# chorowski-lab/pytorch-asr

Hardware: AMD Instinct MI355X
Metric: CTC train-step frames/sec (higher is better)
Workload: dtype bf16; 1 GPU; WSJ mono-char CTC (egs/wsj/yamls/ctc.yaml shapes), DeepSpeech2 conv+4xBiLSTM-320 encoder + FSTDecoder, fwd+bwd+GradientClipping(clip 480000, skip 4.8e+06 = recipe x global_batch/16)+PolyakDecay+Adam, synthetic 40-dim x 1-channel x 1000-frame fbank; batch_per_gpu=768, global_batch=768, frames=1000, classes=49, parallelism=dp1, batch_norm=per-replica statistics, optimizer_steps=139, step_boundary=device: att_speech.fused_step (clip / skip decision + Adam, no read-back)

## Files before the change

include/asr_amd.h:

```cpp
#ifndef ASR_AMD_H
#define ASR_AMD_H

#include <stdint.h>

#ifdef __cplusplus
extern "C" {
#endif

enum {
    ASR_OK = 0,
    ASR_EINVAL = 1,
    ASR_EUNSUPPORTED = 2,
    ASR_ELAUNCH = 3
};

int asr_abi_version(void);

const char *asr_strerror(int code);

int64_t asr_lattice_fwbw_workspace_bytes(int T, int B, int C, int N);

int asr_lattice_fwbw_f32(const float *lp, int T, int B, int C,
                         const int32_t *lens,
                         const int32_t *src_in, const int32_t *il_in,
                         const float *w_in, const float *term,
                         const int32_t *dst_out, const int32_t *il_out,
                         const float *w_out,
                         int N, int Kin, int Kout, int Bg, float neg_inf,
                         float *out_logZ, float *out_grad,
                         float *out_logZ_bwd,
                         void *workspace, int64_t workspace_bytes,
                         void *stream);

int asr_lattice_fwbw_band_supported(int T, int B, int C, int N, int Kin, int Kout, int Bg);
int asr_lattice_fwbw_band_f32(const float *lp, int T, int B, int C,
                              const int32_t *lens,
                              const int32_t *src_in, const int32_t *il_in,
                              const float *w_in, const float *term,
                              const int32_t *dst_out, const int32_t *il_out,
                              const float *w_out,
                              int N, int Kin, int Kout, int Bg, float neg_inf, float grad_sign,
                              float *out_logZ, float *out_grad,
                              float *out_logZ_bwd,
                              void *workspace, int64_t workspace_bytes,
                              uint32_t *redo_count,
                              const int32_t *ctc_labels, const int32_t *ctc_label_lens, int ctc_lmax,
                              void *stream);

int64_t asr_lattice_viterbi_workspace_bytes(int T, int B, int N);

int asr_lattice_forward_f32(const float *lp, int T, int B, int C,
                            const int32_t *lens,
                            const int32_t *src_in, const int32_t *il_in,
                            const float *w_in, const float *term,
                            int N, int K, int Bg, float neg_inf, int viterbi,
                            float *out_score, int32_t *out_best_il,
                            void *workspace, int64_t workspace_bytes,
                            void *stream);

int asr_log_softmax_fwd_f32(const float *x, int64_t rows, int group,
                            float *y, void *stream);

int asr_log_softmax_bwd_f32(const float *y, const float *dy, int64_t rows,
                            int group, float *dx, void *stream);

int asr_sub_rowmax_f32(const float *x, int T, int B, int C,
                       const int32_t *lens, float *y, float *row_max,
                       float *max_sum, void *stream);

int asr_argmax_rows_f32(const float *x, int64_t rows, int C, int32_t *out_idx,
                        void *stream);

int asr_ctc_graph_build(const int32_t *labels, const int32_t *label_lens, int B, int Lmax,
                        int num_symbols, int context_order, int allow_nonblank_selfloops,
                        int use_contextual_blanks, float nc_weight, int32_t *src_in,
                        int32_t *il_in, float *w_in, float *term, int32_t *dst_out,
                        int32_t *il_out, float *w_out, void *stream);

int64_t asr_lattice_grouped_workspace_bytes(int T, int B, int N, int G);

int asr_lattice_grouped_fwbw_f32(
    const float *lp, int T, int B, int C, const int32_t *lens, int N, int G, int Wg, int Wh,
    const int32_t *g_of, const int32_t *h_of, const int32_t *label, const int32_t *selfx,
    const int32_t *uniq, const int32_t *mem_g, const int32_t *mem_h, const float *term,
    float neg_inf, float *out_logZ, float *out_grad, float *out_logZ_bwd, void *workspace,
    int64_t workspace_bytes, void *stream);
int asr_lattice_grouped_fwbw_acc_f32(
    const float *lp, int T, int B, int C, const int32_t *lens, int N, int G, int Wg, int Wh,
    const int32_t *g_of, const int32_t *h_of, const int32_t *label, const int32_t *selfx,
    const int32_t *uniq, const int32_t *mem_g, const int32_t *mem_h, const float *term,
    float neg_inf, int accumulate, float *out_logZ, float *out_grad, float *out_logZ_bwd,
    void *workspace, int64_t workspace_bytes, void *stream);

int asr_lattice_grouped_forward_f32(
    const float *lp, int T, int B, int C, const int32_t *lens, int N, int G, int Wg, int Wh,
    const int32_t *g_of, const int32_t *h_of, const int32_t *label, const int32_t *selfx,
    const int32_t *uniq, const int32_t *mem_g, const int32_t *mem_h, const float *term,
    float neg_inf, int viterbi, float *out_score, int32_t *out_best_il, void *workspace,
    int64_t workspace_bytes, void *stream);

int64_t asr_lstm_workspace_bytes(int B, int H);

int asr_lstm_bidir_fwd_bf16(const void *gx, int gx_bf16, const void *whh_bf16,
                            const int32_t *lens, int T, int B, int H,
                            float *y, void *y_bf16, void *gates_bf16, float *csave,
                            void *workspace, int64_t workspace_bytes,
                            uint32_t *err_flag, void *stream);

int asr_lstm_wgrad_supported(int H);
int64_t asr_lstm_wgrad_workspace_bytes(int T, int B, int H, int with_input);
int asr_lstm_wgrad_bf16(const void *dgates_bf16, const void *x_bf16, const void *y_bf16,
                        int T, int B, int H, float *dw_ih, float *dw_hh,
                        void *workspace, int64_t workspace_bytes, void *stream);

int asr_lstm_dgrad_supported(int H);
int asr_lstm_dgrad_bf16(const void *dgates_bf16, const void *w_ih_bf16, int T, int B, int H,
                        float *dx, void *stream);

int asr_lstm_fused_supported(int B, int H, int F);
int asr_lstm_bidir_fwd_fused_bf16(const void *x_bf16, const void *wih_bf16,
                                  const void *whh_bf16, const int32_t *lens,
                                  int T, int B, int H, int F, float *y, void *y_bf16,
                                  void *gates_bf16, float *csave, void *workspace,
                                  int64_t workspace_bytes, uint32_t *err_flag, void *stream);

int asr_lstm_bidir_bwd_bf16(const float *dy, int dy_shared, const void *whhT_bf16,
                            const int32_t *lens, int T, int B, int H,
                            const void *gates_bf16, const float *csave,
                            void *dgates_bf16,
                            void *workspace, int64_t workspace_bytes,
                            uint32_t *err_flag, void *stream);

int64_t asr_gru_workspace_bytes(int B, int H);
int asr_gru_supported(int B, int H);

int asr_gru_bidir_fwd_bf16(const void *gx, int gx_bf16, const void *whh_bf16,
                           const int32_t *lens, int T, int B, int H,
                           float *y, void *y_bf16, void *gates_bf16,
                           void *workspace, int64_t workspace_bytes,
                           uint32_t *err_flag, void *stream);

int asr_gru_bidir_bwd_bf16(const float *dy, int dy_shared, const void *whhT_bf16,
                           const int32_t *lens, int T, int B, int H,
                           const void *gates_bf16, const float *y,
                           void *dgx_bf16, void *dhn_bf16,
                           void *workspace, int64_t workspace_bytes,
                           uint32_t *err_flag, void *stream);

int64_t asr_bn_act_workspace_bytes(int C);
int asr_bn_act_fwd_f32(const void *x, int x_bf16, const float *conv_bias, int B, int C, int H, int W,
                       const float *gamma, const float *beta,
                       float *running_mean, float *running_var,
                       int channels_last,
                       int training, float momentum, float eps, float lo, float hi,
                       void *out, int out_bf16, int out_time_major,
                       float *save_mean, float *save_invstd,
                       const double *chan_sums,
                       void *workspace, int64_t workspace_bytes, void *stream);

int asr_bn_act_bwd_f32(const void *x, int x_bf16, const float *conv_bias, int B, int C, int H, int W,
                       const float *gamma, const float *beta,
                       const float *save_mean, const float *save_invstd,
                       int channels_last,
                       int training, float lo, float hi,
                       const void *dy, int dy_bf16, int dy_time_major,
                       void *dx, float *dgamma, float *dbeta, float *dconv_bias,
                       void *workspace, int64_t workspace_bytes, void *stream);

int asr_bn_act_bwd_phase_f32(const void *x, int x_bf16, const float *conv_bias, int B, int C, int H, int W,
                             const float *gamma, const float *beta,
                             const float *save_mean, const float *save_invstd,
                             int channels_last,
                             int training, float lo, float hi,
                             const void *dy, int dy_bf16, int dy_time_major,
                             void *dx, float *dgamma, float *dbeta, float *dconv_bias,
                             void *workspace, int64_t workspace_bytes, int phase, double n_total,
                             void *stream);

int asr_log_softmax_shift_fwd_f32(const float *x, int T, int B, int C, const int32_t *lens,
                                  float *y, float *nls, float *nls_sum, void *stream);
int asr_log_softmax_shift_bwd_f32(const float *y, const float *nls, const float *dy, int64_t rows,
                                  int C, float *dx, void *stream);

int asr_log_softmax_shift_bwd_split_blocks(int64_t rows);
int asr_log_softmax_shift_bwd_split_bf16(const float *y, const float *nls, const float *dy,
                                         int64_t rows, int C, void *hi_bf16, void *lo_bf16, int ld,
                                         float *colsum_partial, void *stream);

int asr_sum_leading_f32(const float *in, int G, int64_t n, float *out, void *stream);

int asr_split_bf16_f32(const float *x, int64_t rows, int64_t cols, int64_t ldx,
                       void *hi_bf16, int64_t ldhi, void *lo_bf16, int64_t ldlo, void *stream);

int64_t asr_conv7x7c32_workspace_bytes(void);
int asr_conv7x7c32_fwd_bf16(const void *x, const float *w, int B, int H, int W, int stride_h,
                            void *y, double *chan_sums, void *workspace, int64_t workspace_bytes,
                            void *stream);
int asr_conv7x7c32_bwd_data_bf16(const void *dy, const float *w, int B, int H, int W,
                                 int stride_h, void *dx, void *workspace,
                                 int64_t workspace_bytes, void *stream);
int asr_conv7x7c32_wgrad_bf16(const void *x, const void *dy, int B, int H, int W, int stride_h,
                              float *dw, void *workspace, int64_t workspace_bytes, void *stream);

int64_t asr_conv1_7x7s2_workspace_bytes(void);
int asr_conv1_7x7s2_fwd(const float *x, const float *w, int B, int T, int F, void *y,
                        double *chan_sums, void *workspace, int64_t workspace_bytes, void *stream);
int asr_conv1_7x7s2_wgrad(const float *x, const void *dy, int B, int T, int F, float *dw,
                          void *workspace, int64_t workspace_bytes, void *stream);

int64_t asr_conv1c_7x7s2_workspace_bytes(int cin);
int asr_conv1c_7x7s2_fwd(const float *x, const float *w, int B, int T, int F, int cin, void *y,
                         double *chan_sums, void *workspace, int64_t workspace_bytes, void *stream);
int asr_conv1c_7x7s2_wgrad(const float *x, const void *dy, int B, int T, int F, int cin,
                           float *dw, void *workspace, int64_t workspace_bytes, void *stream);

int asr_tcn_attention_step_f32(const float *eproj, const float *enc, const int32_t *enc_lens,
                               const float *filt, const float *glob, const float *w_score,
                               float b_score, float temperature,
                               const float *att_prev, const int32_t *parent,
                               int T, int B, int beam, int A, int Kf, int E,
                               float *att_new, float *context, void *stream);

int asr_tcn_attention_step_win_f32(const float *eproj, const float *enc, const int32_t *enc_lens,
                                   const float *filt, const float *glob, const float *w_score,
                                   float b_score, float temperature,
                                   const float *att_prev, const int32_t *parent,
                                   int T, int B, int beam, int A, int Kf, int E,
                                   int win_lo, int win_hi,
                                   float *att_new, float *context, void *stream);

int asr_tcn_attention_scan_fwd_f32(const float *eproj, const float *filt, const float *glob,
                                   const float *a0, const float *w_score, const float *b_score,
                                   float temperature, const int32_t *enc_lens, int T, int B,
                                   int L, int A, int Kf, float *att, void *stream);
int asr_tcn_attention_scan_bwd_f32(const float *eproj, const float *filt, const float *glob,
                                   const float *a0, const float *w_score, float temperature,
                                   const int32_t *enc_lens, const float *att, const float *d_att,
                                   int T, int B, int L, int A, int Kf, float *d_eproj,
                                   float *d_filt, float *d_glob, float *d_a0, float *d_wb,
                                   void *stream);

int asr_att_gru_scan_fwd_f32(const float *eproj, const float *encoded, const int32_t *enc_lens,
                             const float *gx_emb, const float *w_ic, const float *w_hh,
                             const float *b_hh, const float *w_rec, const float *w_score,
                             const float *b_score, const float *h0, int T, int B, int beam,
                             int L, int A, int E, int H, float *att, float *states,
                             float *contexts, float *gates, float *rec, void *stream);
int asr_att_gru_scan_bwd_f32(const float *eproj, const float *encoded, const int32_t *enc_lens,
                             const float *w_icT, const float *w_hhT, const float *w_recT,
                             const float *w_score, const float *h0, const float *att,
                             const float *states, const float *gates, const float *rec,
                             const float *d_att, const float *d_states, int T, int B, int L,
                             int A, int E, int H, float *d_eproj, float *d_gates,
                             float *d_contexts, float *d_rec, float *d_w_score, float *d_h0,
                             void *stream);

int asr_beam_step_f32(const float *logits, const float *scores_in, float *scores_out,
                      const int32_t *est_in, int32_t *est_out, int step, int B, int beam, int C,
                      int Lcap, float len_div, int32_t *finished_count, float *best_score,
                      int32_t *best_len, int32_t *best_tokens, int32_t *new_input,
                      int32_t *parent, int32_t *done_and_scratch, void *stream);

#define ASR_LM_BAG_CAP 32
int asr_beam_lm_supported(int beam, int C, int bag_cap);
int asr_lm_label_costs_f64(const int32_t *ptr, const int32_t *ilabel, const double *arc_w_closed,
                           int nstates, const int32_t *bag_state, const double *bag_cost,
                           const int32_t *bag_n, int bag_cap, const int32_t *mapping,
                           const int32_t *frozen, int B, int beam, int C, double *cost, void *stream);
int asr_lm_bag_advance_f64(const int32_t *ptr, const int32_t *ptr_ne, const int32_t *dst,
                           const int32_t *ilabel, const double *weight, const int32_t *rank,
                           int nstates, int max_rank, const int32_t *mapping,
                           const int32_t *in_state, const double *in_cost, const int32_t *in_n,
                           int32_t *out_state, double *out_cost, int32_t *out_n, int bag_cap,
                           const int32_t *parent, const int32_t *new_input, const int32_t *nsteps,
                           int step, int B, int beam, int32_t *overflow, void *stream);
int asr_beam_lm_step_f32(const float *logits, const float *att, const int32_t *enc_lens,
                         const double *lm_cost, double lm_weight, const float *scores_in,
                         float *scores_out, const int32_t *est_in, int32_t *est_out,
                         const float *cov_in, float *cov_out, float *min_eos, int step, int B,
                         int beam, int C, int T, int Lcap, float len_div, double min_attention_pos,
                         float coverage_tau, float coverage_weight, int32_t *fin_count,
                         int32_t *fin_parity, float *fin_score, int32_t *fin_len, int32_t *fin_beam,
                         int32_t *fin_tokens, float *best_score, int32_t *best_len,
                         int32_t *best_tokens, float *best_elems, int32_t *new_input,
                         int32_t *parent, int32_t *frozen, int32_t *nsteps, void *stream);

int asr_graph_search_supported(int beam, int span, int T, int bag_cap);
int asr_beam_lm_step_graph_f32(const float *logits, const float *att, const int32_t *enc_lens,
                               const double *lm_cost, double lm_weight, const float *scores_in,
                               float *scores_out, const int32_t *est_in, int32_t *est_out,
                               const float *cov_in, float *cov_out, float *min_eos, int step, int B,
                               int beam, int C, int T, int Lcap, float len_div,
                               double min_attention_pos, float coverage_tau, float coverage_weight,
                               int32_t *fin_count, int32_t *fin_parity, float *fin_score,
                               int32_t *fin_len, int32_t *fin_beam, int32_t *fin_tokens,
                               float *best_score, int32_t *best_len, int32_t *best_tokens,
                               float *best_elems, int32_t *new_input, int32_t *parent,
                               int32_t *frozen, int32_t *nsteps, int32_t *fin_mask, float *tot_out,
                               void *stream);
int asr_graph_merge_f32(const float *att, const int32_t *enc_lens, float *scores, float *tot,
                        const int32_t *est_in, const int32_t *est_out, const int32_t *fin_mask,
                        const int32_t *bag_state, const int32_t *bag_n, int bag_cap,
                        const int32_t *nsteps, const float *len_pow, int step, int B, int beam, int T,
                        int Lcap, int span, float merge_threshold, int Ncap, int32_t *node_count,
                        float *node_score, int32_t *node_len, int32_t *node_tokens, float *node_att,
                        int32_t *node_bag_n, int32_t *node_bag_state, int32_t *node_fin,
                        int32_t *node_uplink, void *stream);

int asr_forced_level_f32(const float *logits, const float *att, const float *cov_in, float *cov_out,
                         const int32_t *parent, const int32_t *edge_ptr, const int32_t *edge_label,
                         const int32_t *edge_dst, const double *acoustic_in, double *acoustic_out,
                         const int32_t *enc_lens, int B, int width, int C, int T, int cov_in_rows,
                         int n_edges, int n_out, int n_sent, float coverage_tau,
                         double *sent_acoustic, int32_t *sent_covered, void *stream);

int asr_lattice_fwbw_signed_f32(const float *lp, int T, int B, int C, const int32_t *lens,
                                const int32_t *src_in, const int32_t *il_in, const float *w_in,
                                const float *term, const int32_t *dst_out, const int32_t *il_out,
                                const float *w_out, int N, int Kin, int Kout, int Bg, float neg_inf,
                                float grad_sign, float *out_logZ, float *out_grad,
                                float *out_logZ_bwd, void *workspace, int64_t workspace_bytes,
                                void *stream);
int asr_scale_rows_f32(float *x, int T, int B, int C, const float *scale, void *stream);

typedef struct AsrAdamChunk {
    void *param;
    uint32_t flat_offset;
    uint32_t count;
} AsrAdamChunk;
int asr_adam_chunk_elems(void);
int asr_grad_sumsq_partials_f32(const float *g, int64_t n, float *partials, int nparts, void *stream);
int asr_adam_clip_step_f32(const AsrAdamChunk *chunks, int nchunks, const float *g_flat,
                           float *m_flat, float *v_flat, const float *partials, int nparts,
                           const uint32_t *err_word, float lr, float beta1, float beta2, float eps,
                           float weight_decay, float clip_norm, float skip_norm,
                           const int32_t *step_in, int32_t *step_out, float *stats, void *stream);

int asr_adam_clip_step_ex_f32(const AsrAdamChunk *chunks, int nchunks, const float *g_flat,
                              float *m_flat, float *v_flat, const float *partials, int nparts,
                              const uint32_t *err_word, float lr, float beta1, float beta2, float eps,
                              float weight_decay, float clip_norm, float skip_norm,
                              const int32_t *step_in, int32_t *step_out, const uint32_t *skip_word,
                              float *stats, void *stream);

int asr_nonfinite_flag_f32(const float *x, int n, uint32_t *flag, void *stream);

typedef struct AsrNoiseSegment {
    void *data;
    uint64_t index;
    uint32_t count;
    float sigma;
} AsrNoiseSegment;
#define ASR_NOISE_APPLY 0
#define ASR_NOISE_WRITE 1
int asr_noise_chunk_elems(void);
int asr_gaussian_noise_f32(const AsrNoiseSegment *segs, int nsegs, uint64_t seed, uint32_t tag,
                           uint64_t iteration, int mode, int sign, void *stream);

int asr_edit_distance_max_len(void);
int asr_edit_distance_stats_i32(const int32_t *x, const int32_t *x_off, const int32_t *y,
                                const int32_t *y_off, int n_pairs, int max_x, int max_y,
                                int32_t *out, void *stream);

int asr_lattice_shared_supported(int N, int E, int C);
int64_t asr_lattice_shared_workspace_bytes(int T, int B, int N);
int asr_lattice_shared_fwbw_f32(
    const float *lp, int T, int B, int C, const int32_t *lens, int N, int E,
    const int32_t *in_ptr, const uint32_t *in_arc, const int32_t *out_ptr, const uint32_t *out_arc,
    const float *term, const int32_t *order_in, int n_light_in, int lanes_in,
    const int32_t *order_out, int n_light_out, int lanes_out, float neg_inf, float grad_sign,
    int accumulate, float *out_logZ, float *out_grad, float *out_logZ_bwd, void *workspace,
    int64_t workspace_bytes, void *stream);
int asr_lattice_shared_forward_f32(
    const float *lp, int T, int B, int C, const int32_t *lens, int N, int E,
    const int32_t *in_ptr, const uint32_t *in_arc, const float *term, const int32_t *order_in,
    int n_light_in, int lanes_in, float neg_inf, int viterbi, float *out_score,
    int32_t *out_best_il, void *workspace, int64_t workspace_bytes, void *stream);

int asr_ctc_align_supported(int T, int Lmax, int C);
int64_t asr_ctc_align_workspace_bytes(int T, int B, int Lmax);
int asr_ctc_align_f64(const float *lp, const int32_t *lens, const int32_t *labels,
                      const int32_t *label_lens, int B, int T, int C, int Lmax, int S,
                      int context_order, int allow_nonblank_selfloops, int eval_repeats_in_context,
                      double *out_cost, int32_t *out_frames, int32_t *out_states,
                      int32_t *out_segments, void *workspace, int64_t workspace_bytes, void *stream);

int asr_wfst_decode_supported(int64_t N, int64_t A, int C, int T);
int64_t asr_wfst_decode_workspace_bytes(int64_t N, int B, int64_t list_cap, int64_t log_cap);
int asr_wfst_decode_f32(const float *lp, int64_t frame_stride, const int32_t *lens, int T, int B, int C,
                        int64_t N, int64_t A, const uint32_t *arc_ptr, const int32_t *arc_src,
                        const int32_t *arc_dst, const int32_t *arc_ilabel, const int32_t *arc_olabel,
                        const float *arc_weight, const float *final_cost, const uint32_t *eps_ptr,
                        const uint32_t *eps_arc, int64_t E, const int32_t *eps_rank, int num_ranks,
                        int start, float beam, float acoustic_scale, int allow_partial, int64_t list_cap,
                        int64_t log_cap, int word_cap, int threads, float *out_cost,
                        int32_t *out_reached_final,
                        int32_t *out_alignment, int32_t *out_num_active, int32_t *out_words,
                        int32_t *out_num_words, int32_t *out_overflow, void *workspace,
                        int64_t workspace_bytes, void *stream);

int asr_wfst_lattice_supported(int64_t N, int64_t A, int C, int T);
int64_t asr_wfst_lattice_workspace_bytes(int64_t N, int B, int T, int64_t list_cap, int64_t log_cap);
int asr_wfst_lattice_f32(const float *lp, int64_t frame_stride, const int32_t *lens, int T, int B, int C,
                         int64_t N, int64_t A, const uint32_t *arc_ptr, const int32_t *arc_src,
                         const int32_t *arc_dst, const int32_t *arc_ilabel, const int32_t *arc_olabel,
                         const float *arc_weight, const float *final_cost, const uint32_t *eps_ptr,
                         const uint32_t *eps_arc, int64_t E, const int32_t *eps_rank, int num_ranks,
                         int start, float beam, float lattice_beam, float acoustic_scale,
                         int allow_partial, int64_t list_cap, int64_t log_cap, int64_t node_cap,
                         int64_t arc_cap, int threads, float *out_cost, int32_t *out_reached_final,
                         int32_t *out_num_nodes, int32_t *out_num_arcs, int32_t *node_time,
                         int32_t *node_state, float *node_alpha, float *node_beta,
                         int32_t *lat_src, int32_t *lat_dst, uint32_t *lat_arc, float *lat_lp,
                         int32_t *out_overflow, void *workspace, int64_t workspace_bytes,
                         void *stream);

int asr_lattice_bestpath_supported(int64_t N, int64_t A, int64_t L);
int64_t asr_lattice_bestpath_workspace_bytes(int64_t num_nodes, int num_pairs);
int asr_lattice_bestpath_f64(
    int B, int b_begin, int b_count, int num_pairs, int64_t N, int64_t A, int64_t L, const int64_t *h_node_off,
    const int64_t *h_arc_off, const int64_t *h_level_off, const int64_t *node_off, const int64_t *arc_off,
    const int64_t *level_off, const int32_t *node_time, const int32_t *node_state, const int32_t *node_level,
    const int32_t *lat_src, const int32_t *lat_dst, const int64_t *lat_arc, const float *lat_lp,
    const int32_t *level_ptr, const int32_t *level_node, const int32_t *in_ptr, const int32_t *in_arc,
    const int32_t *out_ptr, const int32_t *num_frames, const int32_t *reached_final, const double *own_scale,
    const double *acoustic_scales, const double *lm_scales, int64_t num_states, int64_t num_graph_arcs,
    const float *arc_weight, const int32_t *arc_olabel, const float *final_cost, int start, int threads,
    double *out_cost, int32_t *out_num_words, int32_t *out_words, int32_t *out_status, void *workspace,
    int64_t workspace_bytes, void *stream);
int asr_lattice_posterior_supported(int64_t N, int64_t A, int64_t L);
int64_t asr_lattice_posterior_workspace_bytes(int64_t num_nodes);
int asr_lattice_posterior_f64(
    int B, int b_begin, int b_count, int64_t N, int64_t A, int64_t L, const int64_t *h_node_off,
    const int64_t *h_arc_off, const int64_t *h_level_off, const int64_t *node_off, const int64_t *arc_off,
    const int64_t *level_off, const int32_t *node_time, const int32_t *node_state, const int32_t *node_level,
    const int32_t *lat_src, const int32_t *lat_dst, const int64_t *lat_arc, const float *lat_lp,
    const int32_t *level_ptr, const int32_t *level_node, const int32_t *in_ptr, const int32_t *in_arc,
    const int32_t *out_ptr, const int32_t *num_frames, const int32_t *reached_final, const double *own_scale,
    double acoustic_scale, double lm_scale, int64_t num_states, int64_t num_graph_arcs, const float *arc_weight,
    const int32_t *arc_olabel, const float *final_cost, int start, int threads, double *out_log_z,
    double *out_arc_log_post, double *out_node_log_post, int32_t *out_status, void *workspace,
    int64_t workspace_bytes, void *stream);

#ifdef __cplusplus
}
#endif
#endif
```

pytorch-asr_amd/att_speech/_native.py:

```python
import ctypes
import warnings
import os

import torch

_HERE = os.path.dirname(os.path.abspath(__file__))
LIB_PATH = os.environ.get(
    'ASR_AMD_LIB', os.path.join(os.path.dirname(_HERE), 'csrc', 'libasr_amd.so'))

ASR_OK, ASR_EINVAL, ASR_EUNSUPPORTED, ASR_ELAUNCH = 0, 1, 2, 3
ABI_VERSION = 24

_lib = None
EVENT_HOOK = None
_WARNED = {}

_vp, _i, _i64, _f = ctypes.c_void_p, ctypes.c_int, ctypes.c_int64, ctypes.c_float

_SIGNATURES = {
    'asr_abi_version': (ctypes.c_int, []),
    'asr_strerror': (ctypes.c_char_p, [_i]),
    'asr_lattice_fwbw_workspace_bytes': (_i64, [_i, _i, _i, _i]),
    'asr_lattice_fwbw_f32': (_i, [_vp, _i, _i, _i, _vp, _vp, _vp, _vp, _vp, _vp,
                                  _vp, _vp, _i, _i, _i, _i, _f, _vp, _vp, _vp,
                                  _vp, _i64, _vp]),
    'asr_lattice_fwbw_signed_f32': (_i, [_vp, _i, _i, _i, _vp, _vp, _vp, _vp, _vp, _vp,
                                         _vp, _vp, _i, _i, _i, _i, _f, _f, _vp, _vp, _vp,
                                         _vp, _i64, _vp]),
    'asr_scale_rows_f32': (_i, [_vp, _i, _i, _i, _vp, _vp]),
    'asr_lattice_fwbw_band_supported': (_i, [_i] * 7),
    'asr_lattice_fwbw_band_f32': (_i, [_vp, _i, _i, _i, _vp, _vp, _vp, _vp, _vp, _vp,
                                       _vp, _vp, _i, _i, _i, _i, _f, _f, _vp, _vp, _vp,
                                       _vp, _i64, _vp, _vp, _vp, _i, _vp]),
    'asr_lattice_viterbi_workspace_bytes': (_i64, [_i, _i, _i]),
    'asr_lattice_forward_f32': (_i, [_vp, _i, _i, _i, _vp, _vp, _vp, _vp, _vp,
                                     _i, _i, _i, _f, _i, _vp, _vp, _vp, _i64,
                                     _vp]),
    'asr_log_softmax_fwd_f32': (_i, [_vp, _i64, _i, _vp, _vp]),
    'asr_log_softmax_bwd_f32': (_i, [_vp, _vp, _i64, _i, _vp, _vp]),
    'asr_sub_rowmax_f32': (_i, [_vp, _i, _i, _i, _vp, _vp, _vp, _vp, _vp]),
    'asr_argmax_rows_f32': (_i, [_vp, _i64, _i, _vp, _vp]),
    'asr_conv7x7c32_workspace_bytes': (_i64, []),
    'asr_conv7x7c32_fwd_bf16': (_i, [_vp, _vp, _i, _i, _i, _i, _vp, _vp, _vp, _i64, _vp]),
    'asr_conv7x7c32_bwd_data_bf16': (_i, [_vp, _vp, _i, _i, _i, _i, _vp, _vp, _i64, _vp]),
    'asr_conv7x7c32_wgrad_bf16': (_i, [_vp, _vp, _i, _i, _i, _i, _vp, _vp, _i64, _vp]),
    'asr_conv1_7x7s2_workspace_bytes': (_i64, []),
    'asr_conv1_7x7s2_fwd': (_i, [_vp, _vp, _i, _i, _i, _vp, _vp, _vp, _i64, _vp]),
    'asr_conv1_7x7s2_wgrad': (_i, [_vp, _vp, _i, _i, _i, _vp, _vp, _i64, _vp]),
    'asr_conv1c_7x7s2_workspace_bytes': (_i64, [_i]),
    'asr_conv1c_7x7s2_fwd': (_i, [_vp, _vp, _i, _i, _i, _i, _vp, _vp, _vp, _i64, _vp]),
    'asr_conv1c_7x7s2_wgrad': (_i, [_vp, _vp, _i, _i, _i, _i, _vp, _vp, _i64, _vp]),
    'asr_log_softmax_shift_fwd_f32': (_i, [_vp, _i, _i, _i, _vp, _vp, _vp, _vp, _vp]),
    'asr_log_softmax_shift_bwd_f32': (_i, [_vp, _vp, _vp, _i64, _i, _vp, _vp]),
    'asr_sum_leading_f32': (_i, [_vp, _i, _i64, _vp, _vp]),
    'asr_adam_chunk_elems': (_i, []),
    'asr_grad_sumsq_partials_f32': (_i, [_vp, _i64, _vp, _i, _vp]),
    'asr_adam_clip_step_f32': (_i, [_vp, _i, _vp, _vp, _vp, _vp, _i, _vp, _f, _f, _f, _f, _f, _f, _f,
                                    _vp, _vp, _vp, _vp]),
    'asr_adam_clip_step_ex_f32': (_i, [_vp, _i, _vp, _vp, _vp, _vp, _i, _vp, _f, _f, _f, _f, _f, _f, _f,
                                       _vp, _vp, _vp, _vp, _vp]),
    'asr_nonfinite_flag_f32': (_i, [_vp, _i, _vp, _vp]),
    'asr_noise_chunk_elems': (_i, []),
    'asr_gaussian_noise_f32': (_i, [_vp, _i, ctypes.c_uint64, ctypes.c_uint32, ctypes.c_uint64, _i, _i, _vp]),
    'asr_edit_distance_max_len': (_i, []),
    'asr_edit_distance_stats_i32': (_i, [_vp, _vp, _vp, _vp, _i, _i, _i, _vp, _vp]),
    'asr_ctc_align_supported': (_i, [_i, _i, _i]),
    'asr_ctc_align_workspace_bytes': (_i64, [_i, _i, _i]),
    'asr_ctc_align_f64': (_i, [_vp, _vp, _vp, _vp, _i, _i, _i, _i, _i, _i, _i, _i,
                               _vp, _vp, _vp, _vp, _vp, _i64, _vp]),
    'asr_wfst_decode_supported': (_i, [_i64, _i64, _i, _i]),
    'asr_wfst_decode_workspace_bytes': (_i64, [_i64, _i, _i64, _i64]),
    'asr_wfst_decode_f32': (_i, [_vp, _i64, _vp, _i, _i, _i, _i64, _i64] + [_vp] * 9 + [_i64, _vp, _i, _i,
                                 _f, _f, _i, _i64, _i64, _i, _i] + [_vp] * 8 + [_i64, _vp]),
    'asr_wfst_lattice_supported': (_i, [_i64, _i64, _i, _i]),
    'asr_wfst_lattice_workspace_bytes': (_i64, [_i64, _i, _i, _i64, _i64]),
    'asr_wfst_lattice_f32': (_i, [_vp, _i64, _vp, _i, _i, _i, _i64, _i64] + [_vp] * 9 + [_i64, _vp, _i, _i,
                                  _f, _f, _f, _i, _i64, _i64, _i64, _i64, _i] + [_vp] * 14 + [_i64, _vp]),
    'asr_lattice_bestpath_supported': (_i, [_i64, _i64, _i64]),
    'asr_lattice_bestpath_workspace_bytes': (_i64, [_i64, _i]),
    'asr_lattice_bestpath_f64': (_i, [_i, _i, _i, _i, _i64, _i64, _i64] + [_vp] * 23 + [_i64, _i64] + [_vp] * 3 +
                                 [_i, _i] + [_vp] * 5 + [_i64, _vp]),
    'asr_lattice_posterior_supported': (_i, [_i64, _i64, _i64]),
    'asr_lattice_posterior_workspace_bytes': (_i64, [_i64]),
    'asr_lattice_posterior_f64': (_i, [_i, _i, _i, _i64, _i64, _i64] + [_vp] * 21 + [ctypes.c_double] * 2 +
                                  [_i64, _i64] + [_vp] * 3 + [_i, _i] + [_vp] * 5 + [_i64, _vp]),
    'asr_split_bf16_f32': (_i, [_vp, _i64, _i64, _i64, _vp, _i64, _vp, _i64, _vp]),
    'asr_log_softmax_shift_bwd_split_blocks': (_i, [_i64]),
    'asr_log_softmax_shift_bwd_split_bf16': (_i, [_vp, _vp, _vp, _i64, _i, _vp, _vp, _i, _vp, _vp]),
    'asr_tcn_attention_step_f32': (_i, [_vp, _vp, _vp, _vp, _vp, _vp, _f, _f, _vp, _vp,
                                        _i, _i, _i, _i, _i, _i, _vp, _vp, _vp]),
    'asr_tcn_attention_step_win_f32': (_i, [_vp, _vp, _vp, _vp, _vp, _vp, _f, _f, _vp, _vp,
                                            _i, _i, _i, _i, _i, _i, _i, _i, _vp, _vp, _vp]),
    'asr_tcn_attention_scan_fwd_f32': (_i, [_vp] * 6 + [_f, _vp, _i, _i, _i, _i, _i, _vp, _vp]),
    'asr_tcn_attention_scan_bwd_f32': (_i, [_vp] * 5 + [_f, _vp, _vp, _vp, _i, _i, _i, _i, _i] +
                                       [_vp] * 6),
    'asr_att_gru_scan_fwd_f32': (_i, [_vp] * 11 + [_i] * 7 + [_vp] * 6),
    'asr_att_gru_scan_bwd_f32': (_i, [_vp] * 14 + [_i] * 6 + [_vp] * 7),
    'asr_beam_step_f32': (_i, [_vp, _vp, _vp, _vp, _vp, _i, _i, _i, _i, _i, _f,
                               _vp, _vp, _vp, _vp, _vp, _vp, _vp, _vp]),
    'asr_beam_lm_supported': (_i, [_i, _i, _i]),
    'asr_lm_label_costs_f64': (_i, [_vp, _vp, _vp, _i, _vp, _vp, _vp, _i, _vp, _vp, _i, _i, _i, _vp, _vp]),
    'asr_lm_bag_advance_f64': (_i, [_vp] * 6 + [_i, _i] + [_vp] * 7 + [_i, _vp, _vp, _vp, _i, _i, _i, _vp, _vp]),
    'asr_beam_lm_step_f32': (_i, [_vp, _vp, _vp, _vp, ctypes.c_double] + [_vp] * 7 + [_i] * 6 +
                             [_f, ctypes.c_double, _f, _f] + [_vp] * 15),
    'asr_graph_search_supported': (_i, [_i, _i, _i, _i]),
    'asr_beam_lm_step_graph_f32': (_i, [_vp, _vp, _vp, _vp, ctypes.c_double] + [_vp] * 7 + [_i] * 6 +
                                   [_f, ctypes.c_double, _f, _f] + [_vp] * 17),
    'asr_graph_merge_f32': (_i, [_vp] * 9 + [_i, _vp, _vp] + [_i] * 6 + [_f, _i] + [_vp] * 10),
    'asr_forced_level_f32': (_i, [_vp] * 11 + [_i] * 8 + [_f, _vp, _vp, _vp]),
    'asr_ctc_graph_build': (_i, [_vp, _vp, _i, _i, _i, _i, _i, _i, _f] + [_vp] * 8),
    'asr_lattice_grouped_workspace_bytes': (_i64, [_i, _i, _i, _i]),
    'asr_lattice_grouped_fwbw_f32': (_i, [_vp, _i, _i, _i, _vp, _i, _i, _i, _i] + [_vp] * 8 +
                                     [_f, _vp, _vp, _vp, _vp, _i64, _vp]),
    'asr_lattice_grouped_fwbw_acc_f32': (_i, [_vp, _i, _i, _i, _vp, _i, _i, _i, _i] + [_vp] * 8 +
                                         [_f, _i, _vp, _vp, _vp, _vp, _i64, _vp]),
    'asr_lattice_grouped_forward_f32': (_i, [_vp, _i, _i, _i, _vp, _i, _i, _i, _i] + [_vp] * 8 +
                                        [_f, _i, _vp, _vp, _vp, _i64, _vp]),
    'asr_lattice_shared_supported': (_i, [_i, _i, _i]),
    'asr_lattice_shared_workspace_bytes': (_i64, [_i, _i, _i]),
    'asr_lattice_shared_fwbw_f32': (_i, [_vp, _i, _i, _i, _vp, _i, _i] + [_vp] * 6 + [_i, _i, _vp, _i, _i,
                                         _f, _f, _i, _vp, _vp, _vp, _vp, _i64, _vp]),
    'asr_lattice_shared_forward_f32': (_i, [_vp, _i, _i, _i, _vp, _i, _i] + [_vp] * 4 +
                                       [_i, _i, _f, _i, _vp, _vp, _vp, _i64, _vp]),
    'asr_lstm_workspace_bytes': (_i64, [_i, _i]),
    'asr_lstm_bidir_fwd_bf16': (_i, [_vp, _i, _vp, _vp, _i, _i, _i, _vp, _vp, _vp, _vp, _vp, _i64, _vp, _vp]),
    'asr_lstm_bidir_bwd_bf16': (_i, [_vp, _i, _vp, _vp, _i, _i, _i, _vp, _vp, _vp, _vp, _i64, _vp, _vp]),
    'asr_lstm_fused_supported': (_i, [_i, _i, _i]),
    'asr_lstm_wgrad_supported': (_i, [_i]),
    'asr_lstm_dgrad_supported': (_i, [_i]),
    'asr_lstm_dgrad_bf16': (_i, [_vp, _vp, _i, _i, _i, _vp, _vp]),
    'asr_lstm_wgrad_workspace_bytes': (_i64, [_i, _i, _i, _i]),
    'asr_lstm_wgrad_bf16': (_i, [_vp, _vp, _vp, _i, _i, _i, _vp, _vp, _vp, _i64, _vp]),
    'asr_lstm_bidir_fwd_fused_bf16': (_i, [_vp, _vp, _vp, _vp, _i, _i, _i, _i, _vp, _vp, _vp, _vp, _vp, _i64, _vp, _vp]),
    'asr_gru_workspace_bytes': (_i64, [_i, _i]),
    'asr_gru_supported': (_i, [_i, _i]),
    'asr_gru_bidir_fwd_bf16': (_i, [_vp, _i, _vp, _vp, _i, _i, _i, _vp, _vp, _vp, _vp, _i64, _vp, _vp]),
    'asr_gru_bidir_bwd_bf16': (_i, [_vp, _i, _vp, _vp, _i, _i, _i, _vp, _vp, _vp, _vp, _vp, _i64, _vp, _vp]),
    'asr_bn_act_workspace_bytes': (_i64, [_i]),
    'asr_bn_act_fwd_f32': (_i, [_vp, _i, _vp, _i, _i, _i, _i, _vp, _vp, _vp, _vp, _i, _i, _f, _f, _f, _f,
                                _vp, _i, _i, _vp, _vp, _vp, _vp, _i64, _vp]),
    'asr_bn_act_bwd_f32': (_i, [_vp, _i, _vp, _i, _i, _i, _i, _vp, _vp, _vp, _vp, _i, _i, _f, _f,
                                _vp, _i, _i, _vp, _vp, _vp, _vp, _vp, _i64, _vp]),
    'asr_bn_act_bwd_phase_f32': (_i, [_vp, _i, _vp, _i, _i, _i, _i, _vp, _vp, _vp, _vp, _i, _i, _f, _f,
                                      _vp, _i, _i, _vp, _vp, _vp, _vp, _vp, _i64, _i, ctypes.c_double, _vp]),
}

_EXPERIMENT_SIGNATURES = {
    'asr_lstm_bidir_bwd_fused_bf16': (_i, [_vp, _i, _vp, _vp, _vp, _i, _i, _i, _vp, _vp, _vp, _vp,
                                           _vp, _i64, _vp, _vp]),
    'asr_lstm_bidir_fwd_fused_sum_bf16': (_i, [_vp, _vp, _vp, _vp, _i, _i, _i, _i, _vp, _vp, _vp, _vp, _vp, _vp, _i64,
                                               _vp, _vp]),
}
_experiments = False


class NativeLibraryError(RuntimeError):
    pass


def lib():
    global _lib, _experiments
    if _lib is None:
        if not os.path.exists(LIB_PATH):
            raise NativeLibraryError(
                "%s is missing: build it with `make -C pytorch-asr_amd/csrc` "
                "(or __graft_entry__.build()); there is no fallback path."
                % LIB_PATH)
        handle = ctypes.CDLL(LIB_PATH)
        for name, (res, args) in _SIGNATURES.items():
            fn = getattr(handle, name)
            fn.restype = res
            fn.argtypes = args
        if handle.asr_abi_version() != ABI_VERSION:
            raise NativeLibraryError("libasr_amd.so ABI %d != expected %d" % (
                handle.asr_abi_version(), ABI_VERSION))
        _experiments = all(hasattr(handle, name) for name in _EXPERIMENT_SIGNATURES)
        if _experiments:
            for name, (res, args) in _EXPERIMENT_SIGNATURES.items():
                fn = getattr(handle, name)
                fn.restype = res
                fn.argtypes = args
        _lib = handle
    return _lib


def experiments_built():
    lib()
    return _experiments


def _need_experiments(what):
    if not experiments_built():
        raise NotImplementedError(
            '%s is an experiment (include/asr_amd_experiments.h): rebuild with '
            '`make -C pytorch-asr_amd/csrc clean all EXPERIMENTS=1`' % what)


def check(code, what):
    if code == ASR_OK:
        return
    msg = "%s: %s" % (what, lib().asr_strerror(code).decode())
    if code == ASR_EINVAL:
        raise AssertionError(msg)
    if code == ASR_EUNSUPPORTED:
        raise NotImplementedError(msg)
    raise RuntimeError(msg)


def _dev(t, dtype, name):
    if not isinstance(t, torch.Tensor) or not t.is_cuda:
        raise NativeLibraryError(
            "%s must be a GPU tensor: the MI355X path has no CPU fallback" % name)
    if t.dtype != dtype:
        raise TypeError("%s must be %s, got %s" % (name, dtype, t.dtype))
    return t if t.is_contiguous() else t.contiguous()


def _p(t):
    return ctypes.c_void_p(t.data_ptr()) if t is not None else None


def _stream():
    return ctypes.c_void_p(torch.cuda.current_stream().cuda_stream)


class Graph(object):
    __slots__ = ('src_in', 'il_in', 'w_in', 'term', 'dst_out', 'il_out',
                 'w_out', 'Bg', 'N', 'Kin', 'Kout', 'band', 'ctc_labels', 'addend')

    def __init__(self, graph_matrices, device):
        self.band = False
        self.ctc_labels = None
        self.addend = None
        if graph_matrices is None:
            return
        gm = list(graph_matrices)
        if len(gm) not in (4, 8):
            raise AssertionError("expected 4 or 8 graph matrices")
        bg = gm[0].size(0)
        if not all(m.size(0) == bg for m in gm):
            raise AssertionError("graph matrices disagree on batch size")

        def to_i(m):
            return m.to(device=device, dtype=torch.int32).contiguous()

        def to_f(m):
            return m.to(device=device, dtype=torch.float32).contiguous()
        self.src_in, self.il_in, self.w_in = to_i(gm[0]), to_i(gm[1]), to_f(gm[2])
        self.term = to_f(gm[3]).reshape(bg, -1)
        self.Bg, self.N, self.Kin = self.src_in.shape
        if len(gm) == 8:
            self.dst_out, self.il_out, self.w_out = to_i(gm[4]), to_i(gm[5]), to_f(gm[6])
            self.Kout = self.dst_out.shape[2]
            self.band = _host_band_check(gm)
        else:
            self.dst_out = self.il_out = self.w_out = None
            self.Kout = 0


def _host_band_check(gm):
    src, w = gm[0], gm[2]
    if src.is_cuda or w.is_cuda or src.dim() != 3 or src.size(1) > 256:
        return False
    valid = w > -5e19
    d = torch.arange(src.size(1)).view(1, -1, 1) - src.long()
    return bool(((d >= 0) & (d <= 2) & (w <= 0) | ~valid).all())


_BAND_STATE = {'cool': 0, 'pending': None, 'launched': 0, 'seen': (0, 0)}
_BAND_COOLDOWN = 64
_BAND_MAX_BATCH = 1 << 30
_BAND_COUNTER = {}


def _band_counter(device):
    c = _BAND_COUNTER.get(device)
    if c is None:
        c = (torch.zeros(1, dtype=torch.int32, device=device), torch.zeros(1, dtype=torch.int32).pin_memory())
        _BAND_COUNTER[device] = c
        _BAND_STATE.update(pending=None, launched=0, seen=(0, 0))
    return c


def _band_policy_allows():
    st = _BAND_STATE
    pend = st['pending']
    if pend is not None and pend[1].query():
        redone_total, launched_total = int(pend[0].item()), pend[2]
        redone, batch = redone_total - st['seen'][0], launched_total - st['seen'][1]
        st['seen'] = (redone_total, launched_total)
        st['pending'] = None
        if redone * 10 > batch:
            st['cool'] = _BAND_COOLDOWN
    if st['cool'] > 0:
        st['cool'] -= 1
        return False
    return True


def _band_policy_record(device, B):
    st = _BAND_STATE
    st['launched'] += B
    if st['pending'] is not None:
        return
    dev_cnt, host = _band_counter(device)
    host.copy_(dev_cnt, non_blocking=True)
    ev = torch.cuda.Event()
    ev.record()
    st['pending'] = (host, ev, st['launched'])


def scale_rows_(x, scale):
    x = _dev(x, torch.float32, 'x')
    scale = _dev(scale.to(torch.float32), torch.float32, 'scale')
    T, B, C = x.shape
    check(lib().asr_scale_rows_f32(_p(x), T, B, C, _p(scale), _stream()), 'asr_scale_rows_f32')
    return x


def lattice_fwbw(lp, lens, graph, neg_inf=-1e20, want_bwd_total=False, grad_sign=1.0):
    lp = _dev(lp, torch.float32, 'log_probs')
    lens = _dev(lens, torch.int32, 'act_lens')
    T, B, C = lp.shape
    if graph.Bg not in (1, B):
        raise AssertionError("graph batch %d not in (1, %d)" % (graph.Bg, B))
    L = lib()
    logZ = torch.empty(B, dtype=torch.float32, device=lp.device)
    grad = torch.empty_like(lp)
    zb = torch.empty(B, dtype=torch.float32, device=lp.device) if want_bwd_total else None
    if (T + 64) * B * C * 4 >= 2 ** 32 and graph.N <= 512 and not _WARNED.get('fits32'):
        _WARNED['fits32'] = True
        warnings.warn('lattice_fwbw: T*B*C*4 = %.2f GiB >= 4 GiB (e.g. bi-char CTC at B >= ~1100): the '
                      'meet-in-the-middle kernels address with 32-bit offsets, this call runs the '
                      'generic (much slower) kernel; split the batch' % (T * B * C * 4 / 2.0 ** 30))
    nbytes = L.asr_lattice_fwbw_workspace_bytes(T, B, C, graph.N)
    ws = torch.empty(nbytes, dtype=torch.uint8, device=lp.device)
    hook = EVENT_HOOK
    if hook is not None:
        ev0 = torch.cuda.Event(enable_timing=True)
        ev1 = torch.cuda.Event(enable_timing=True)
        ev0.record()
    band_env = os.environ.get('ASR_LATTICE_BAND', '1')
    use_band = (graph.band and band_env != '0' and
                L.asr_lattice_fwbw_band_supported(T, B, C, graph.N, graph.Kin, graph.Kout, graph.Bg))
    if use_band and band_env != '2' and (B > _BAND_MAX_BATCH or not _band_policy_allows()):
        use_band = False
    args = (_p(lp), T, B, C, _p(lens), _p(graph.src_in), _p(graph.il_in),
            _p(graph.w_in), _p(graph.term), _p(graph.dst_out), _p(graph.il_out),
            _p(graph.w_out), graph.N, graph.Kin, graph.Kout, graph.Bg,
            float(neg_inf), _p(logZ), _p(grad), _p(zb), _p(ws), nbytes)
    sargs = args[:17] + (float(grad_sign),) + args[17:]
# ... 624 lines not shown


def tcn_attention_scan_fwd(eproj, filt, glob, a0, w_score, b_score, enc_lens, temperature):
    eproj, a0 = _dev(eproj, torch.float32, 'eproj'), _dev(a0, torch.float32, 'a0')
    filt, glob = _dev(filt, torch.float32, 'filt'), _dev(glob, torch.float32, 'glob')
    w_score = _dev(w_score, torch.float32, 'w_score')
    b_score = _dev(b_score, torch.float32, 'b_score')
    enc_lens = _dev(enc_lens, torch.int32, 'enc_lens')
    T, B, A = eproj.shape
    L = glob.shape[0]
    att = torch.empty((L, B, T), dtype=torch.float32, device=eproj.device)
    check(lib().asr_tcn_attention_scan_fwd_f32(
        _p(eproj), _p(filt), _p(glob), _p(a0), _p(w_score), _p(b_score), float(temperature),
        _p(enc_lens), T, B, L, A, filt.shape[2] // A, _p(att), _stream()),
        'asr_tcn_attention_scan_fwd_f32')
    return att


def tcn_attention_scan_bwd(eproj, filt, glob, a0, w_score, enc_lens, temperature, att, d_att):
    eproj, a0 = _dev(eproj, torch.float32, 'eproj'), _dev(a0, torch.float32, 'a0')
    filt, glob = _dev(filt, torch.float32, 'filt'), _dev(glob, torch.float32, 'glob')
    w_score = _dev(w_score, torch.float32, 'w_score')
    enc_lens = _dev(enc_lens, torch.int32, 'enc_lens')
    att, d_att = _dev(att, torch.float32, 'att'), _dev(d_att, torch.float32, 'd_att')
    T, B, A = eproj.shape
    L = glob.shape[0]
    d_eproj = torch.empty_like(eproj)
    d_filt = torch.empty_like(filt)
    d_glob = torch.empty_like(glob)
    d_a0 = torch.empty_like(a0)
    d_wb = torch.empty((B, A + 1), dtype=torch.float32, device=eproj.device)
    check(lib().asr_tcn_attention_scan_bwd_f32(
        _p(eproj), _p(filt), _p(glob), _p(a0), _p(w_score), float(temperature), _p(enc_lens),
        _p(att), _p(d_att), T, B, L, A, filt.shape[2] // A, _p(d_eproj), _p(d_filt), _p(d_glob),
        _p(d_a0), _p(d_wb), _stream()), 'asr_tcn_attention_scan_bwd_f32')
    return d_eproj, d_filt, d_glob, d_a0, d_wb


ATT_GRU_MAX_FRAMES, ATT_GRU_MAX_HIDDEN, ATT_GRU_MAX_ENCODED = 4096, 320, 512


def att_gru_supported(T, A, E, H):
    return (1 <= T <= ATT_GRU_MAX_FRAMES and 1 <= A <= ATT_GRU_MAX_HIDDEN
            and 1 <= H <= ATT_GRU_MAX_HIDDEN and 1 <= E <= ATT_GRU_MAX_ENCODED
            and A % 4 == 0 and E % 4 == 0 and H % 4 == 0)


def att_gru_scan_fwd(eproj, encoded, enc_lens, gx_emb, w_ic, w_hh, b_hh, w_rec, w_score, b_score,
                     h0, beam=1, save=True):
    f32 = torch.float32
    eproj, encoded = _dev(eproj, f32, 'eproj'), _dev(encoded, f32, 'encoded')
    gx_emb, h0 = _dev(gx_emb, f32, 'gx_emb'), _dev(h0, f32, 'h0')
    w_ic, w_hh, b_hh = _dev(w_ic, f32, 'w_ic'), _dev(w_hh, f32, 'w_hh'), _dev(b_hh, f32, 'b_hh')
    w_rec, w_score = _dev(w_rec, f32, 'w_rec'), _dev(w_score, f32, 'w_score')
    b_score = _dev(b_score, f32, 'b_score')
    enc_lens = _dev(enc_lens, torch.int32, 'enc_lens')
    T, NU, A = eproj.shape
    E = encoded.shape[2]
    L, B, H3 = gx_emb.shape
    H = H3 // 3
    if (encoded.shape[:2] != (T, NU) or B != NU * beam or h0.shape != (B, H) or H3 != 3 * H
            or w_ic.shape != (H3, E) or w_hh.shape != (H3, H) or b_hh.numel() != H3
            or w_rec.shape != (A, H) or w_score.numel() != A or enc_lens.numel() != NU):
        raise AssertionError('asr_att_gru_scan_fwd_f32: inconsistent operand shapes')
    new = lambda *shape: torch.empty(shape, dtype=f32, device=eproj.device)
    att, states = new(L, B, T), new(L, B, H)
    ctxs, gates, rec = (new(L, B, E), new(L, B, 4 * H), new(L, B, A)) if save else (None,) * 3
    check(lib().asr_att_gru_scan_fwd_f32(
        _p(eproj), _p(encoded), _p(enc_lens), _p(gx_emb), _p(w_ic), _p(w_hh), _p(b_hh), _p(w_rec),
        _p(w_score), _p(b_score), _p(h0), T, B, beam, L, A, E, H, _p(att), _p(states), _p(ctxs),
        _p(gates), _p(rec), _stream()), 'asr_att_gru_scan_fwd_f32')
    return att, states, ctxs, gates, rec


def att_gru_scan_bwd(eproj, encoded, enc_lens, w_icT, w_hhT, w_recT, w_score, h0, att, states,
                     gates, rec, d_att, d_states):
    f32 = torch.float32
    eproj, encoded = _dev(eproj, f32, 'eproj'), _dev(encoded, f32, 'encoded')
    w_icT, w_hhT = _dev(w_icT, f32, 'w_icT'), _dev(w_hhT, f32, 'w_hhT')
    w_recT, w_score = _dev(w_recT, f32, 'w_recT'), _dev(w_score, f32, 'w_score')
    h0, att, states = _dev(h0, f32, 'h0'), _dev(att, f32, 'att'), _dev(states, f32, 'states')
    gates, rec = _dev(gates, f32, 'gates'), _dev(rec, f32, 'rec')
    d_att = None if d_att is None else _dev(d_att, f32, 'd_att')
    d_states = None if d_states is None else _dev(d_states, f32, 'd_states')
    enc_lens = _dev(enc_lens, torch.int32, 'enc_lens')
    T, B, A = eproj.shape
    E = encoded.shape[2]
    L, _, H = states.shape
    if (encoded.shape[:2] != (T, B) or states.shape[1] != B or att.shape != (L, B, T)
            or gates.shape != (L, B, 4 * H) or rec.shape != (L, B, A) or h0.shape != (B, H)
            or w_icT.shape != (E, 3 * H) or w_hhT.shape != (H, 3 * H) or w_recT.shape != (H, A)
            or (d_att is not None and d_att.shape != att.shape)
            or (d_states is not None and d_states.shape != states.shape)):
        raise AssertionError('asr_att_gru_scan_bwd_f32: inconsistent operand shapes')
    dev = eproj.device
    d_eproj = torch.zeros_like(eproj)
    d_gates = torch.empty_like(gates)
    d_ctx = torch.empty((L, B, E), dtype=f32, device=dev)
    d_rec = torch.empty_like(rec)
    d_v = torch.empty((B, A), dtype=f32, device=dev)
    d_h0 = torch.empty_like(h0)
    check(lib().asr_att_gru_scan_bwd_f32(
        _p(eproj), _p(encoded), _p(enc_lens), _p(w_icT), _p(w_hhT), _p(w_recT), _p(w_score),
        _p(h0), _p(att), _p(states), _p(gates), _p(rec), _p(d_att), _p(d_states), T, B, L, A, E, H,
        _p(d_eproj), _p(d_gates), _p(d_ctx), _p(d_rec), _p(d_v), _p(d_h0), _stream()),
        'asr_att_gru_scan_bwd_f32')
    return d_eproj, d_gates, d_ctx, d_rec, d_v, d_h0


LM_BAG_CAP = 32


def beam_lm_supported(beam, C, bag_cap=LM_BAG_CAP):
    return bool(lib().asr_beam_lm_supported(beam, C, bag_cap))


def lm_label_costs(lm, bag_state, bag_cost, bag_n, mapping, frozen, B, beam, C, cost, bag_cap=LM_BAG_CAP):
    check(lib().asr_lm_label_costs_f64(
        _p(lm['ptr']), _p(lm['ilabel']), _p(lm['w_closed']), lm['nstates'], _p(bag_state), _p(bag_cost),
        _p(bag_n), bag_cap, _p(mapping), _p(frozen), B, beam, C, _p(cost), _stream()),
        'asr_lm_label_costs_f64')
    return cost


def lm_bag_advance(lm, mapping, bags_in, bags_out, parent, new_input, nsteps, step, B, beam, overflow,
                   bag_cap=LM_BAG_CAP):
    check(lib().asr_lm_bag_advance_f64(
        _p(lm['ptr']), _p(lm['ptr_ne']), _p(lm['dst']), _p(lm['ilabel']), _p(lm['weight']), _p(lm['rank']),
        lm['nstates'], lm['max_rank'], _p(mapping), _p(bags_in[0]), _p(bags_in[1]), _p(bags_in[2]),
        _p(bags_out[0]), _p(bags_out[1]), _p(bags_out[2]), bag_cap, _p(parent), _p(new_input),
        _p(nsteps), step, B, beam, _p(overflow), _stream()), 'asr_lm_bag_advance_f64')


def beam_lm_step(logits, att, lens, lm_cost, lm_weight, scores_in, scores_out, est_in, est_out, cov_in,
                 cov_out, min_eos, step, B, beam, len_div, min_attention_pos, coverage_tau,
                 coverage_weight, state, fin_mask=None, tot_out=None):
    C, T = logits.shape[-1], att.shape[-1]
    graph = fin_mask is not None or tot_out is not None
    name = 'asr_beam_lm_step_graph_f32' if graph else 'asr_beam_lm_step_f32'
    extra = (_p(fin_mask), _p(tot_out)) if graph else ()
    check(getattr(lib(), name)(
        _p(logits), _p(att), _p(lens), _p(lm_cost), float(lm_weight), _p(scores_in), _p(scores_out),
        _p(est_in), _p(est_out), _p(cov_in), _p(cov_out), _p(min_eos), step, B, beam, C, T,
        est_in.shape[1], len_div, float(min_attention_pos), coverage_tau, coverage_weight,
        _p(state['fin_count']), _p(state['fin_parity']), _p(state['fin_score']), _p(state['fin_len']),
        _p(state['fin_beam']), _p(state['fin_tokens']), _p(state['best_score']), _p(state['best_len']),
        _p(state['best_tokens']), _p(state['best_elems']), _p(state['new_input']), _p(state['parent']),
        _p(state['frozen']), _p(state['nsteps']), *(extra + (_stream(),))), name)


beam_lm_step_graph = beam_lm_step


def graph_search_supported(beam, span, T, bag_cap=LM_BAG_CAP):
    return bool(lib().asr_graph_search_supported(beam, span, T, bag_cap))


NODE_KEYS = ('node_count', 'node_score', 'node_len', 'node_tokens', 'node_att', 'node_bag_n',
             'node_bag_state', 'node_fin', 'node_uplink')


def graph_merge(att, lens, scores, tot, est_in, est_out, fin_mask, bags, nsteps, len_pow, step, B, beam,
                span, merge_threshold, store, bag_cap=LM_BAG_CAP):
    T, Lcap, Ncap = att.shape[-1], est_in.shape[1], store['node_score'].shape[1]
    check(lib().asr_graph_merge_f32(
        _p(att), _p(lens), _p(scores), _p(tot), _p(est_in), _p(est_out), _p(fin_mask),
        _p(bags[0]) if bags is not None else None, _p(bags[2]) if bags is not None else None, bag_cap,
        _p(nsteps), _p(len_pow), step, B, beam, T, Lcap, int(span), float(merge_threshold), Ncap,
        *([_p(store[k]) for k in NODE_KEYS] + [_stream()])), 'asr_graph_merge_f32')


def forced_level(logits, att, cov_in, cov_out, parent, edge_ptr, edge_label, edge_dst, acoustic_in,
                 acoustic_out, lens, B, width, coverage_tau, sent_acoustic, sent_covered):
    slots = B * width
    C, T = logits.shape[-1], att.shape[-1]
    assert logits.shape[0] == slots and att.shape[0] == slots and cov_out.shape[0] >= slots
    assert cov_in.shape[-1] == T and cov_out.shape[-1] == T and parent.numel() >= slots
    assert edge_ptr.numel() >= slots + 1 and acoustic_in.numel() >= slots
    assert edge_dst.numel() == edge_label.numel() and sent_covered.numel() == sent_acoustic.numel()
    check(lib().asr_forced_level_f32(
        _p(_dev(logits, torch.float32, 'logits')), _p(_dev(att, torch.float32, 'att')),
        _p(_dev(cov_in, torch.float32, 'cov_in')), _p(_dev(cov_out, torch.float32, 'cov_out')),
        _p(_dev(parent, torch.int32, 'parent')), _p(_dev(edge_ptr, torch.int32, 'edge_ptr')),
        _p(_dev(edge_label, torch.int32, 'edge_label')), _p(_dev(edge_dst, torch.int32, 'edge_dst')),
        _p(_dev(acoustic_in, torch.float64, 'acoustic_in')),
        _p(_dev(acoustic_out, torch.float64, 'acoustic_out')), _p(_dev(lens, torch.int32, 'lens')),
        B, width, C, T, cov_in.shape[0], edge_label.numel(), acoustic_out.numel(),
        sent_acoustic.numel(), float(coverage_tau), _p(_dev(sent_acoustic, torch.float64, 'sent_acoustic')),
        _p(_dev(sent_covered, torch.int32, 'sent_covered')), _stream()), 'asr_forced_level_f32')


def beam_step(logits, scores_in, scores_out, est_in, est_out, step, B, beam, len_div, state):
    C = logits.shape[-1]
    check(lib().asr_beam_step_f32(
        _p(logits), _p(scores_in), _p(scores_out), _p(est_in), _p(est_out), int(step), B, beam, C,
        est_in.shape[1], float(len_div), _p(state['finished_count']), _p(state['best_score']),
        _p(state['best_len']), _p(state['best_tokens']), _p(state['new_input']),
        _p(state['parent']), _p(state['done']), _stream()), 'asr_beam_step_f32')


def _nhwc_bf16(t, what):
    if not t.is_cuda:
        raise NativeLibraryError("%s must live on the MI355X" % what)
    if t.dtype != torch.bfloat16:
        t = t.to(torch.bfloat16)
    t = t.contiguous(memory_format=torch.channels_last)
    return (t,) + tuple(t.shape)


def conv7x7c32_fwd(x, weight, stride_h, want_sums=False):
    x, B, C, H, W = _nhwc_bf16(x, 'x')
    weight = _dev(weight, torch.float32, 'weight')
    Ho, Wo = (H - 7) // stride_h + 1, W - 6
    y = torch.empty((B, 32, Ho, Wo), dtype=torch.bfloat16, device=x.device,
                    memory_format=torch.channels_last)
    L = lib()
    nbytes = L.asr_conv7x7c32_workspace_bytes()
    ws = torch.empty(nbytes, dtype=torch.uint8, device=x.device)
    sums = torch.empty((2, 32), dtype=torch.float64, device=x.device) if want_sums else None
    check(L.asr_conv7x7c32_fwd_bf16(_p(x), _p(weight), B, H, W, int(stride_h), _p(y), _p(sums),
                                    _p(ws), nbytes, _stream()), 'asr_conv7x7c32_fwd_bf16')
    return (y, sums) if want_sums else y


def conv7x7c32_bwd_data(dy, weight, H, W, stride_h):
    dy, B, C, Ho, Wo = _nhwc_bf16(dy, 'dy')
    weight = _dev(weight, torch.float32, 'weight')
    assert Ho == (H - 7) // stride_h + 1 and Wo == W - 6
    dx = torch.empty((B, 32, H, W), dtype=torch.bfloat16, device=dy.device,
                     memory_format=torch.channels_last)
    L = lib()
    nbytes = L.asr_conv7x7c32_workspace_bytes()
    ws = torch.empty(nbytes, dtype=torch.uint8, device=dy.device)
    check(L.asr_conv7x7c32_bwd_data_bf16(_p(dy), _p(weight), B, H, W, int(stride_h), _p(dx),
                                         _p(ws), nbytes, _stream()), 'asr_conv7x7c32_bwd_data_bf16')
    return dx


def conv7x7c32_wgrad(x, dy, stride_h):
    x, B, C, H, W = _nhwc_bf16(x, 'x')
    dy = _nhwc_bf16(dy, 'dy')[0]
    dw = torch.empty((32, 32, 7, 7), dtype=torch.float32, device=x.device)
    L = lib()
    nbytes = L.asr_conv7x7c32_workspace_bytes()
    ws = torch.empty(nbytes, dtype=torch.uint8, device=x.device)
    check(L.asr_conv7x7c32_wgrad_bf16(_p(x), _p(dy), B, H, W, int(stride_h), _p(dw), _p(ws),
                                      nbytes, _stream()), 'asr_conv7x7c32_wgrad_bf16')
    return dw


def conv1_supported(F, cin):
    Fo = (F - 7) // 2 + 1
    return F >= 7 and ((cin == 1 and Fo <= 64) or (cin == 3 and Fo <= 48 and Fo % 2 == 0))


def conv1_fwd(x, weight, want_sums=False):
    x = _dev(x, torch.float32, 'x')
    weight = _dev(weight, torch.float32, 'weight')
    cin = x.shape[3] if x.dim() == 4 else 1
    B, T, F = x.shape[:3]
    if tuple(weight.shape) != (32, cin, 7, 7):
        raise ValueError('conv1_fwd: weight must be [32, %d, 7, 7]' % cin)
    y = torch.empty((B, 32, T + 6, (F - 7) // 2 + 1), dtype=torch.bfloat16, device=x.device,
                    memory_format=torch.channels_last)
    L = lib()
    sums = torch.empty((2, 32), dtype=torch.float64, device=x.device) if want_sums else None
    if cin == 1:
        nbytes = L.asr_conv1_7x7s2_workspace_bytes()
        ws = torch.empty(nbytes, dtype=torch.uint8, device=x.device)
        check(L.asr_conv1_7x7s2_fwd(_p(x), _p(weight), B, T, F, _p(y), _p(sums), _p(ws), nbytes,
                                    _stream()), 'asr_conv1_7x7s2_fwd')
    else:
        nbytes = L.asr_conv1c_7x7s2_workspace_bytes(cin)
        if nbytes < 0:
            raise NotImplementedError('conv1_fwd: %d input channels' % cin)
        ws = torch.empty(nbytes, dtype=torch.uint8, device=x.device)
        check(L.asr_conv1c_7x7s2_fwd(_p(x), _p(weight), B, T, F, cin, _p(y), _p(sums), _p(ws), nbytes,
                                     _stream()), 'asr_conv1c_7x7s2_fwd')
    return (y, sums) if want_sums else y


def conv1_wgrad(x, dy):
    x = _dev(x, torch.float32, 'x')
    dy = _nhwc_bf16(dy, 'dy')[0]
    cin = x.shape[3] if x.dim() == 4 else 1
    B, T, F = x.shape[:3]
    dw = torch.empty((32, cin, 7, 7), dtype=torch.float32, device=x.device)
    L = lib()
    if cin == 1:
        nbytes = L.asr_conv1_7x7s2_workspace_bytes()
        ws = torch.empty(nbytes, dtype=torch.uint8, device=x.device)
        check(L.asr_conv1_7x7s2_wgrad(_p(x), _p(dy), B, T, F, _p(dw), _p(ws), nbytes, _stream()),
              'asr_conv1_7x7s2_wgrad')
    else:
        nbytes = L.asr_conv1c_7x7s2_workspace_bytes(cin)
        if nbytes < 0:
            raise NotImplementedError('conv1_wgrad: %d input channels' % cin)
        ws = torch.empty(nbytes, dtype=torch.uint8, device=x.device)
        check(L.asr_conv1c_7x7s2_wgrad(_p(x), _p(dy), B, T, F, cin, _p(dw), _p(ws), nbytes, _stream()),
              'asr_conv1c_7x7s2_wgrad')
    return dw


def split_bf16(x, hi=None, lo=None):
    x = _dev(x, torch.float32, 'x')
    if hi is None:
        hi = torch.empty(x.shape, dtype=torch.bfloat16, device=x.device)
        lo = torch.empty(x.shape, dtype=torch.bfloat16, device=x.device)
        rows, cols, ldx, ldh, ldl = 1, x.numel(), x.numel(), x.numel(), x.numel()
    else:
        if x.dim() != 2 or hi.shape != x.shape or lo.shape != x.shape or x.stride(1) != 1 \
                or hi.stride(1) != 1 or lo.stride(1) != 1 or hi.dtype != torch.bfloat16 or lo.dtype != torch.bfloat16:
            raise ValueError('split_bf16: x, hi, lo must be [rows, cols] with a dense last dimension')
        rows, cols = x.shape
        ldx, ldh, ldl = x.stride(0), hi.stride(0), lo.stride(0)
    check(lib().asr_split_bf16_f32(_p(x), rows, cols, ldx, _p(hi), ldh, _p(lo), ldl, _stream()),
          'asr_split_bf16_f32')
    return hi, lo


def sum_leading(t):
    if not t.is_cuda or t.dtype != torch.float32 or (t[0].numel() & 3):
        return t.sum(0)
    t = t.contiguous()
    if t.data_ptr() & 15:
        return t.sum(0)
    out = torch.empty(t.shape[1:], dtype=torch.float32, device=t.device)
    check(lib().asr_sum_leading_f32(_p(t), t.shape[0], t[0].numel(), _p(out), _stream()),
          'asr_sum_leading_f32')
    return out


def log_softmax_shift_fwd(x, lens):
    x = _dev(x, torch.float32, 'logits')
    lens = _dev(lens, torch.int32, 'lens')
    T, B, C = x.shape
    y = torch.empty_like(x)
    nls = torch.empty((T, B), dtype=torch.float32, device=x.device)
    nls_sum = torch.empty(B, dtype=torch.float32, device=x.device)
    check(lib().asr_log_softmax_shift_fwd_f32(_p(x), T, B, C, _p(lens), _p(y), _p(nls), _p(nls_sum),
                                              _stream()), 'asr_log_softmax_shift_fwd_f32')
    return y, nls, nls_sum


def log_softmax_shift_bwd_split(y, nls, dy, ld):
    y, dy = _dev(y, torch.float32, 'y'), _dev(dy, torch.float32, 'dy')
    C = y.shape[-1]
    rows = y.numel() // C
    L = lib()
    hi = torch.empty((rows, ld), dtype=torch.bfloat16, device=y.device)
    lo = torch.empty((rows, ld), dtype=torch.bfloat16, device=y.device)
    part = torch.empty((L.asr_log_softmax_shift_bwd_split_blocks(rows), ld), dtype=torch.float32, device=y.device)
    check(L.asr_log_softmax_shift_bwd_split_bf16(_p(y), _p(nls), _p(dy), rows, C, _p(hi), _p(lo), int(ld),
                                                 _p(part), _stream()), 'asr_log_softmax_shift_bwd_split_bf16')
    nb = part.shape[0]
    if nb % 32 == 0 and nb > 32:
        part = sum_leading(part.view(32, (nb // 32) * ld)).view(nb // 32, ld)
    return hi, lo, sum_leading(part)[:C]


def log_softmax_shift_bwd(y, nls, dy):
    y, dy = _dev(y, torch.float32, 'y'), _dev(dy, torch.float32, 'dy')
    C = y.shape[-1]
    dx = torch.empty_like(y)
    check(lib().asr_log_softmax_shift_bwd_f32(_p(y), _p(nls), _p(dy), y.numel() // C, C, _p(dx),
                                              _stream()), 'asr_log_softmax_shift_bwd_f32')
    return dx


def edit_distance_max_len():
    return int(lib().asr_edit_distance_max_len())


def edit_distance_stats(x, x_off, y, y_off, max_x, max_y):
    x, x_off = _dev(x, torch.int32, 'x'), _dev(x_off, torch.int32, 'x_off')
    y, y_off = _dev(y, torch.int32, 'y'), _dev(y_off, torch.int32, 'y_off')
    n = x_off.numel() - 1
    if n < 0 or y_off.numel() != n + 1:
        raise AssertionError('edit_distance_stats: x_off and y_off must both hold n + 1 offsets')
    out = torch.empty((n, 4), dtype=torch.int32, device=x.device)
    check(lib().asr_edit_distance_stats_i32(_p(x), _p(x_off), _p(y), _p(y_off), n, int(max_x),
                                            int(max_y), _p(out), _stream()),
          'asr_edit_distance_stats_i32')
    return out


def ctc_align_supported(T, Lmax, C):
    return bool(lib().asr_ctc_align_supported(int(T), int(Lmax), int(C)))


def ctc_align(lp, lens, labels, label_lens, num_symbols, context_order=1,
              allow_nonblank_selfloops=True, eval_repeats_in_context=False):
    lp = _dev(lp, torch.float32, 'log_probs')
    lens, label_lens = _dev(lens, torch.int32, 'lens'), _dev(label_lens, torch.int32, 'label_lens')
    labels = _dev(labels, torch.int32, 'labels')
    T, B, C = lp.shape
    Lmax = labels.shape[1] if labels.dim() == 2 else -1
    if Lmax < 0 or labels.shape[0] != B or lens.numel() != B or label_lens.numel() != B:
        raise AssertionError('ctc_align: lens [B], labels [B, Lmax] and label_lens [B] must match lp [T, B, C]')
    L = lib()
    dev = lp.device
    cost = torch.empty(B, dtype=torch.float64, device=dev)
    frames = torch.empty((B, T), dtype=torch.int32, device=dev)
    states = torch.empty((B, T), dtype=torch.int32, device=dev)
    segments = torch.empty((B, Lmax, 2), dtype=torch.int32, device=dev)
    nbytes = int(L.asr_ctc_align_workspace_bytes(T, B, Lmax))
    ws = torch.empty(nbytes, dtype=torch.uint8, device=dev) if nbytes else None
    check(L.asr_ctc_align_f64(_p(lp), _p(lens), _p(labels), _p(label_lens), B, T, C, Lmax,
                              int(num_symbols), int(context_order), int(bool(allow_nonblank_selfloops)),
                              int(bool(eval_repeats_in_context)), _p(cost), _p(frames), _p(states),
                              _p(segments), _p(ws), nbytes, _stream()), 'asr_ctc_align_f64')
    return cost, frames, states, segments
```

pytorch-asr_amd/att_speech/modules/encoders/deep_speech_2.py:

```python
import warnings
from collections import OrderedDict

import torch
from torch import nn

from att_speech.modules.encoders.base_encoder import BaseEncoder
from att_speech.modules.encoders.encoder_utils import (
    BatchRNN, Normalization, SequentialWithOptionalAttributes)


class DeepSpeech2(BaseEncoder):
    def __init__(self, sample_batch, conv_normalization='batch_norm',
                 conv_strides=[[2, 2], [2, 1]],
                 conv_kernel_sizes=[[41, 11], [21, 11]],
                 conv_num_features=[32, 32],
                 rnn_hidden_size=768, rnn_nb_layers=5, rnn_projection_size=0,
                 rnn_type=nn.LSTM, rnn_dropout=0.0, rnn_residual=False,
                 rnn_normalization='batch_norm', rnn_subsample=None, **kwargs):
        super(DeepSpeech2, self).__init__(**kwargs)
        import os
        self.conv_bf16 = os.environ.get('ASR_CONV_BF16', '1') != '0'
        self.fused_bn = os.environ.get('ASR_FUSED_BN', '1') != '0'
        self.native_conv = os.environ.get('ASR_NATIVE_CONV', '1') != '0'
        if isinstance(rnn_type, str):
            rnn_type = {'LSTM': nn.LSTM, 'GRU': nn.GRU}[rnn_type.split('.')[-1]]
        self.makeConv(sample_batch, conv_strides, conv_kernel_sizes,
                      conv_num_features, conv_normalization)
        features = sample_batch['features']
        features = features.permute(0, 3, 1, 2)
        with torch.no_grad():
            was_training = self.conv.training
            self.conv.eval()
            after_conv_size = self.conv.forward(features).size()
            self.conv.train(was_training)
        self.rnn_input_size = after_conv_size[1] * after_conv_size[3]
        self.makeRnn(rnn_hidden_size, rnn_nb_layers, rnn_projection_size,
                     rnn_type, rnn_dropout, rnn_residual, rnn_normalization,
                     rnn_subsample)

    def makeConv(self, sample_batch, conv_strides, conv_kernel_sizes,
                 conv_num_features, normalization):
        num_channels = sample_batch['features'].size()[3]
        conv_padding = int(0.5 * (
            conv_kernel_sizes[1][0] - 1 +
            conv_strides[0][0] * (conv_kernel_sizes[0][0] - 1)))
        self.conv_cumative_stride = conv_strides[0][0] * conv_strides[1][0]
        self.conv = nn.Sequential(
            nn.Conv2d(num_channels, conv_num_features[0],
                      kernel_size=tuple(conv_kernel_sizes[0]),
                      stride=tuple(conv_strides[0]), padding=(conv_padding, 0)),
            Normalization(normalization, 2, conv_num_features[0]),
            nn.Hardtanh(0, 20, inplace=True),
            nn.Conv2d(conv_num_features[0], conv_num_features[1],
                      kernel_size=tuple(conv_kernel_sizes[1]),
                      stride=tuple(conv_strides[1])),
            Normalization(normalization, 2, conv_num_features[1]),
            nn.Hardtanh(0, 20, inplace=True))

    def makeRnn(self, rnn_hidden_size, rnn_nb_layers, rnn_projection_size,
                rnn_type, rnn_dropout, rnn_residual, normalization,
                rnn_subsample):
        if rnn_subsample is None:
            rnn_subsample = []
        rnn_dropout = nn.Dropout(p=rnn_dropout) if rnn_dropout > 0.0 else None
        rnns = [('0', BatchRNN(input_size=self.rnn_input_size,
                               hidden_size=rnn_hidden_size, rnn_type=rnn_type,
                               bidirectional=True, packed_data=True,
                               normalization=None,
                               projection_size=rnn_projection_size,
                               subsample=(0 in rnn_subsample)))]
        for i in range(rnn_nb_layers - 1):
            rnn = BatchRNN(input_size=(rnn_hidden_size if rnn_projection_size == 0
                                       else rnn_projection_size),
                           projection_size=rnn_projection_size,
                           hidden_size=rnn_hidden_size, rnn_type=rnn_type,
                           bidirectional=True, packed_data=True,
                           normalization=normalization, residual=rnn_residual,
                           subsample=(i + 1 in rnn_subsample))
            if rnn_dropout:
                rnns.append(('{}_dropout'.format(i + 1), rnn_dropout))
            rnns.append(('{}'.format(i + 1), rnn))
        self.rnns = SequentialWithOptionalAttributes(OrderedDict(rnns))

    def _conv_forward(self, features):
        conv = self.conv
        fused = (features.is_cuda and self.fused_bn and len(conv) == 6
                 and isinstance(conv[0], nn.Conv2d) and isinstance(conv[3], nn.Conv2d)
                 and all(isinstance(conv[i], Normalization)
                         and isinstance(conv[i].batch_norm, nn.BatchNorm2d)
                         and conv[i].batch_norm.affine for i in (1, 4))
                 and all(isinstance(conv[i], nn.Hardtanh) for i in (2, 5)))
        bf16 = features.is_cuda and self.conv_bf16 and len(conv) == 6 \
            and isinstance(conv[3], nn.Conv2d)
        c2 = conv[3] if len(conv) == 6 else None

        def run_conv(c, x, with_bias=True, keep_bf16=False):
            bias = c.bias if with_bias else None
            if not bf16:
                return nn.functional.conv2d(x.float() if x.dtype != torch.float32 else x,
                                            c.weight, bias, c.stride, c.padding,
                                            c.dilation, c.groups)
            y = nn.functional.conv2d(
                x.to(torch.bfloat16), c.weight.to(torch.bfloat16),
                None if bias is None else bias.to(torch.bfloat16),
                c.stride, c.padding, c.dilation, c.groups)
            return y if keep_bf16 else y.float()

        def second_conv(x, with_bias=True):
            return run_conv(c2, x, with_bias)

        if fused:
            from att_speech.modules.encoders.native_bn import bn_hardtanh
            from att_speech.modules.encoders import native_conv
            c1 = conv[0]
            sums1 = sums2 = None
            if bf16 and self.native_conv and native_conv.first_supported(c1, features):
                x, sums1 = native_conv.conv1(features, c1)
            else:
                if bf16 and self.native_conv and not getattr(self, '_warned_conv1', False):
                    self._warned_conv1 = True
                    warnings.warn('DeepSpeech2: the first convolution is not a (1 or 3)->32 7x7 stride-(1,2) '
                                  'shape on gradient-free features csrc/conv.hip is built for; using '
                                  'torch / MIOpen for it')
                x = run_conv(c1, features, with_bias=False, keep_bf16=True)
            x = bn_hardtanh(x, conv[1].batch_norm, conv[2], out_bf16=bf16, conv_bias=c1.bias,
                            chan_sums=sums1)
            if bf16 and self.native_conv and native_conv.supported(c2, x):
                y2, sums2 = native_conv.conv7x7c32(x, c2)
            else:
                if bf16 and self.native_conv and not getattr(self, '_warned_conv', False):
                    self._warned_conv = True
                    warnings.warn('DeepSpeech2: the second convolution is not the 32->32 7x7 '
                                  'stride-(3,1) shape csrc/conv.hip is built for; using torch / MIOpen')
                y2 = run_conv(c2, x, with_bias=False, keep_bf16=True)
            x = bn_hardtanh(y2, conv[4].batch_norm, conv[5], time_major=True, conv_bias=c2.bias,
                            chan_sums=sums2, out_bf16=bf16 and self._rnn_takes_bf16(y2))
            return x.view(x.size(0), x.size(1), -1)
        if bf16:
            x = conv[5](conv[4](second_conv(conv[2](conv[1](conv[0](features))))))
        else:
            x = conv(features)
        x = x.permute(2, 0, 1, 3).contiguous()
        return x.view(x.size(0), x.size(1), -1)

    def _rnn_takes_bf16(self, x):
        import os
        if os.environ.get('ASR_LSTM_BF16_INPUT', '1') == '0':
            return False
        first = next(iter(self.rnns._modules.values()), None)
        return (isinstance(first, BatchRNN) and first._use_native(x) and not first.residual
                and type(first.batch_norm.batch_norm).__name__ == 'Identity')

    def forward(self, features, features_lengths, spkids, ivectors=None,
                characteristic_vectors=None, **kwargs):
        features = features.permute(0, 3, 1, 2)
        features_lengths = torch.as_tensor(features_lengths)
        features_lengths = ((features_lengths + self.conv_cumative_stride - 1)
                            // self.conv_cumative_stride).int()
        if features.is_cuda:
            from att_speech import _native
            _native.attach_device_lens(features_lengths, features.device)
        features = self._conv_forward(features)
        assert features_lengths[0] == features.size()[0]
        return self.rnns(features, features_lengths, spkids)
```

pytorch-asr_amd/att_speech/modules/encoders/native_conv.py:

```python
import torch

from att_speech import _native


def supported(conv, x):
    return (x.is_cuda and isinstance(conv, torch.nn.Conv2d) and conv.in_channels == 32
            and conv.out_channels == 32 and tuple(conv.kernel_size) == (7, 7)
            and tuple(conv.stride) == (3, 1) and tuple(conv.padding) == (0, 0)
            and tuple(conv.dilation) == (1, 1) and conv.groups == 1
            and x.dim() == 4 and x.size(2) >= 7 and 7 <= x.size(3) <= 48)


class Conv7x7C32Function(torch.autograd.Function):
    @staticmethod
    def forward(ctx, x, weight):
        x = x.to(torch.bfloat16).contiguous(memory_format=torch.channels_last)
        ctx.save_for_backward(x, weight)
        y, sums = _native.conv7x7c32_fwd(x, weight.detach(), 3, want_sums=True)
        ctx.mark_non_differentiable(sums)
        return y, sums

    @staticmethod
    def backward(ctx, dy, _dsums):
        x, weight = ctx.saved_tensors
        dx = dw = None
        if ctx.needs_input_grad[0]:
            dx = _native.conv7x7c32_bwd_data(dy, weight.detach(), x.size(2), x.size(3), 3)
        if ctx.needs_input_grad[1]:
            dw = _native.conv7x7c32_wgrad(x, dy, 3)
        return dx, dw


def first_supported(conv, x):
    return (x.is_cuda and isinstance(conv, torch.nn.Conv2d) and conv.in_channels in (1, 3)
            and conv.out_channels == 32 and tuple(conv.kernel_size) == (7, 7)
            and tuple(conv.stride) == (1, 2) and tuple(conv.padding) == (6, 0)
            and tuple(conv.dilation) == (1, 1) and conv.groups == 1
            and x.dim() == 4 and x.size(1) == conv.in_channels
            and _native.conv1_supported(x.size(3), conv.in_channels)
            and not x.requires_grad)


class Conv1Function(torch.autograd.Function):

    @staticmethod
    def forward(ctx, x, weight):
        x = x.float().contiguous()
        ctx.save_for_backward(x, weight)
        y, sums = _native.conv1_fwd(x, weight.detach(), want_sums=True)
        ctx.mark_non_differentiable(sums)
        return y, sums

    @staticmethod
    def backward(ctx, dy, _dsums):
        x, weight = ctx.saved_tensors
        return None, (_native.conv1_wgrad(x, dy) if ctx.needs_input_grad[1] else None)


def conv1(features, conv):
    if features.size(1) == 1:
        return Conv1Function.apply(features[:, 0], conv.weight)
    return Conv1Function.apply(features.permute(0, 2, 3, 1), conv.weight)


def conv7x7c32(x, conv):
    return Conv7x7C32Function.apply(x, conv.weight)
```

pytorch-asr_amd/csrc/bnact.hip:

```cpp
#include "common.h"
#include "../../include/asr_amd.h"

namespace {

using namespace asr;

struct BnParams {
    const float *x;
    int B, C, HW, Wd;
    const float *gamma, *beta;
    const float *mean, *invstd;
    const float *shift;
    float lo, hi;
};

__global__ __launch_bounds__(256) void bn_stats_kernel(const float *x, const float *shift, int C, int HW, double *sums) {
    __shared__ float red[64];
    const int c = blockIdx.x, b = blockIdx.y;
    const float *p = x + ((size_t)b * C + c) * HW;
    const float sh0 = shift ? shift[c] : 0.f;
    float s = 0.f, q = 0.f;
    for (int i = threadIdx.x; i < HW; i += 256) {
        const float v = p[i] + sh0;
        s += v;
// ... 241 lines not shown

template <typename DyT, int TM>
__device__ __forceinline__ F4 load_dy4(const BnParamsN &p, const DyT *dy, int64_t pix, int c0) {
    if (TM) {
        const size_t o = tm_index(p, pix, c0);
        F4 d;
#pragma unroll
        for (int i = 0; i < 4; ++i) d.v[i] = (float)dy[o + (size_t)i * p.W];
        return d;
    }
    return load4(dy + pix * p.C + c0);
}

template <typename XT, typename DyT, int TM>
__global__ __launch_bounds__(256) void bn_act_bwd_reduce_nhwc_kernel(BnParamsN p, const DyT *dy, double *sums) {
    const XT *px = (const XT *)p.x;
    const int C = p.C;
    NHWC_THREAD_SETUP(p.P);
    float m[4], is[4], g[4], be[4], s[4] = {0.f, 0.f, 0.f, 0.f}, q[4] = {0.f, 0.f, 0.f, 0.f};
#pragma unroll
    for (int i = 0; i < 4; ++i) {
        m[i] = p.mean[c0 + i] - (p.shift ? p.shift[c0 + i] : 0.f);
        is[i] = p.invstd[c0 + i]; g[i] = p.gamma[c0 + i]; be[i] = p.beta[c0 + i];
    }
    auto acc = [&](const F4 &v, const F4 &dv) {
#pragma unroll
        for (int i = 0; i < 4; ++i) {
            const float xh = (v.v[i] - m[i]) * is[i];
            const float y = fmaf(xh, g[i], be[i]);
            const float d = (y > p.lo && y < p.hi) ? dv.v[i] : 0.f;
            s[i] += d;
            q[i] += d * xh;
        }
    };
    int64_t pix = p0 + pl;
    for (; pix + PL < p1; pix += 2 * PL) {
        const F4 v0 = load4(px + pix * C + c0), v1 = load4(px + (pix + PL) * C + c0);
        const F4 d0 = load_dy4<DyT, TM>(p, dy, pix, c0), d1 = load_dy4<DyT, TM>(p, dy, pix + PL, c0);
        acc(v0, d0);
        acc(v1, d1);
    }
    for (; pix < p1; pix += PL) acc(load4(px + pix * C + c0), load_dy4<DyT, TM>(p, dy, pix, c0));
    nhwc_block_atomics(s, q, C, sums);
}

template <typename XT, typename DyT, int TM>
__global__ __launch_bounds__(256) void bn_act_bwd_apply_nhwc_kernel(BnParamsN p, const DyT *dy, const double *sums,
                                                                    double n, int training, XT *dx) {
    const XT *px = (const XT *)p.x;
    const int C = p.C;
    NHWC_THREAD_SETUP(p.P);
    float m[4], is[4], g[4], be[4], k1[4], k2[4];
#pragma unroll
    for (int i = 0; i < 4; ++i) {
        m[i] = p.mean[c0 + i] - (p.shift ? p.shift[c0 + i] : 0.f);
        is[i] = p.invstd[c0 + i]; g[i] = p.gamma[c0 + i]; be[i] = p.beta[c0 + i];
        k1[i] = training ? (float)(sums[2 * (c0 + i)] / n) : 0.f;
        k2[i] = training ? (float)(sums[2 * (c0 + i) + 1] / n) : 0.f;
    }
    for (int64_t pix = p0 + pl; pix < p1; pix += PL) {
        const F4 v = load4(px + pix * C + c0);
        const F4 dv = load_dy4<DyT, TM>(p, dy, pix, c0);
        F4 o;
#pragma unroll
        for (int i = 0; i < 4; ++i) {
            const float xh = (v.v[i] - m[i]) * is[i];
            const float y = fmaf(xh, g[i], be[i]);
            const float d = (y > p.lo && y < p.hi) ? dv.v[i] : 0.f;
            o.v[i] = g[i] * is[i] * (d - k1[i] - xh * k2[i]);
        }
        store4(dx + pix * C + c0, o);
    }
}

struct F8 { float v[8]; };
typedef __attribute__((ext_vector_type(8))) __bf16 bf16x8v;
__device__ __forceinline__ F8 load8(const __bf16 *p) {
    const bf16x8v t = *reinterpret_cast<const bf16x8v *>(p);
    F8 r;
#pragma unroll
    for (int i = 0; i < 8; ++i) r.v[i] = (float)t[i];
    return r;
}
__device__ __forceinline__ F8 load8(const float *p) {
    const float4 a = reinterpret_cast<const float4 *>(p)[0], b = reinterpret_cast<const float4 *>(p)[1];
    return F8{{a.x, a.y, a.z, a.w, b.x, b.y, b.z, b.w}};
}
__device__ __forceinline__ void store8(__bf16 *p, const F8 &a) {
    bf16x8v t;
#pragma unroll
    for (int i = 0; i < 8; ++i) t[i] = (__bf16)a.v[i];
    *reinterpret_cast<bf16x8v *>(p) = t;
}
__device__ __forceinline__ void store8(float *p, const F8 &a) {
    reinterpret_cast<float4 *>(p)[0] = make_float4(a.v[0], a.v[1], a.v[2], a.v[3]);
    reinterpret_cast<float4 *>(p)[1] = make_float4(a.v[4], a.v[5], a.v[6], a.v[7]);
}
__device__ __forceinline__ void nhwc_block_atomics8(const float (&s)[8], const float (&q)[8], int C,
                                                    double *sums) {
    __shared__ float rs8[256][9], rq8[256][9];
#pragma unroll
    for (int i = 0; i < 8; ++i) { rs8[threadIdx.x][i] = s[i]; rq8[threadIdx.x][i] = q[i]; }
    __syncthreads();
    const int CG = C / 8;
    if ((int)threadIdx.x < C) {
        const int cg = threadIdx.x >> 3, i = threadIdx.x & 7;
        float a = 0.f, b = 0.f;
        for (int t = cg; t < 256; t += CG) { a += rs8[t][i]; b += rq8[t][i]; }
        atomicAdd(&sums[2 * threadIdx.x], (double)a);
        atomicAdd(&sums[2 * threadIdx.x + 1], (double)b);
    }
}
#define NHWC8_THREAD_SETUP(P_)                                                         \
    const int CG = C / 8, PL = 256 / CG, c0 = 8 * ((int)threadIdx.x % CG),             \
              pl = (int)threadIdx.x / CG;                                              \
    const int64_t pend = (P_), cstep = (int64_t)gridDim.x * 2 * PL

template <typename XT, typename OutT>
__global__ __launch_bounds__(256) void bn_act_fwd_nhwc8_kernel(BnParamsN p, OutT *out) {
    const XT *px = (const XT *)p.x;
    const int C = p.C;
    NHWC8_THREAD_SETUP(p.P);
    float sc[8], sh[8];
#pragma unroll
    for (int i = 0; i < 8; ++i) {
        sc[i] = p.gamma[c0 + i] * p.invstd[c0 + i];
        sh[i] = p.beta[c0 + i] - (p.mean[c0 + i] - (p.shift ? p.shift[c0 + i] : 0.f)) * sc[i];
    }
    auto one = [&](int64_t pix, const F8 &v) {
        F8 y;
#pragma unroll
        for (int i = 0; i < 8; ++i) y.v[i] = fminf(fmaxf(fmaf(v.v[i], sc[i], sh[i]), p.lo), p.hi);
        store8(out + pix * C + c0, y);
    };
    for (int64_t pix = (int64_t)blockIdx.x * 2 * PL + pl; pix < pend; pix += cstep) {
        if (pix + PL < pend) {
            const F8 v0 = load8(px + pix * C + c0), v1 = load8(px + (pix + PL) * C + c0);
            one(pix, v0);
            one(pix + PL, v1);
        } else {
            one(pix, load8(px + pix * C + c0));
        }
    }
}

template <typename XT, typename DyT, int MODE>
__global__ __launch_bounds__(256) void bn_act_bwd_nhwc8_kernel(BnParamsN p, const DyT *dy, double *sums,
                                                               double n, int training, XT *dx) {
    const XT *px = (const XT *)p.x;
    const int C = p.C;
    NHWC8_THREAD_SETUP(p.P);
    float m[8], is[8], g[8], be[8], k1[8], k2[8], s[8], q[8];
#pragma unroll
    for (int i = 0; i < 8; ++i) {
        m[i] = p.mean[c0 + i] - (p.shift ? p.shift[c0 + i] : 0.f);
        is[i] = p.invstd[c0 + i]; g[i] = p.gamma[c0 + i]; be[i] = p.beta[c0 + i];
        k1[i] = MODE == 1 && training ? (float)(sums[2 * (c0 + i)] / n) : 0.f;
        k2[i] = MODE == 1 && training ? (float)(sums[2 * (c0 + i) + 1] / n) : 0.f;
        s[i] = q[i] = 0.f;
    }
    auto one = [&](int64_t pix, const F8 &v, const F8 &dv) {
        F8 o;
#pragma unroll
        for (int i = 0; i < 8; ++i) {
            const float xh = (v.v[i] - m[i]) * is[i];
            const float y = fmaf(xh, g[i], be[i]);
            const float d = (y > p.lo && y < p.hi) ? dv.v[i] : 0.f;
            if (MODE == 0) { s[i] += d; q[i] += d * xh; }
            else o.v[i] = g[i] * is[i] * (d - k1[i] - xh * k2[i]);
        }
        if (MODE == 1) store8(dx + pix * C + c0, o);
    };
    for (int64_t pix = (int64_t)blockIdx.x * 2 * PL + pl; pix < pend; pix += cstep) {
        if (pix + PL < pend) {
            const F8 v0 = load8(px + pix * C + c0), v1 = load8(px + (pix + PL) * C + c0);
            const F8 d0 = load8(dy + pix * C + c0), d1 = load8(dy + (pix + PL) * C + c0);
            one(pix, v0, d0);
            one(pix + PL, v1, d1);
        } else {
            one(pix, load8(px + pix * C + c0), load8(dy + pix * C + c0));
        }
    }
    if (MODE == 0) nhwc_block_atomics8(s, q, C, sums);
}

struct FastDiv {
    unsigned m, d;
    __device__ __forceinline__ explicit FastDiv(int dd) : m((unsigned)((1ull << 32) / (unsigned)dd) + 1u), d((unsigned)dd) {}
    __device__ __forceinline__ int operator()(int x) const { return d == 1u ? x : (int)__umulhi((unsigned)x, m); }
};

template <typename T>
__device__ __forceinline__ void tm_row_to_lds(const T *row, float *tile, int CW, int it) {
    const F4 v = load4(row + 4 * it);
    *reinterpret_cast<float4 *>(tile + 4 * it) = make_float4(v.v[0], v.v[1], v.v[2], v.v[3]);
}

template <typename XT, typename OutT>
__global__ __launch_bounds__(256) void bn_act_fwd_nhwc_tm_kernel(BnParamsN p, OutT *out, int TMR) {
    extern __shared__ __attribute__((aligned(16))) float tile[];
    const XT *px = (const XT *)p.x;
    const int C = p.C, W = p.W, CW = C * W, CG = C / 4, Q = CW / 4;
    const int c0 = 4 * ((int)threadIdx.x % CG);
    float sc[4], sh[4];
#pragma unroll
    for (int i = 0; i < 4; ++i) {
        sc[i] = p.gamma[c0 + i] * p.invstd[c0 + i];
        sh[i] = p.beta[c0 + i] - (p.mean[c0 + i] - (p.shift ? p.shift[c0 + i] : 0.f)) * sc[i];
    }
    const int64_t nrows = p.P / W;
    const FastDiv dCG(CG), dW(W), dQ(Q);
    for (int64_t r0 = (int64_t)blockIdx.x * TMR; r0 < nrows; r0 += (int64_t)gridDim.x * TMR) {
        const int nr = nrows - r0 < TMR ? (int)(nrows - r0) : TMR;
        const int b0 = (int)(r0 / p.H), h0 = (int)(r0 - (int64_t)b0 * p.H);
        for (int it = threadIdx.x; it < nr * W * CG; it += 256) {
            const int j = dCG(it), row = dW(j), w = j - row * W;
            const F4 v = load4(px + (r0 * W + j) * C + c0);
#pragma unroll
            for (int i = 0; i < 4; ++i)
                tile[row * CW + (c0 + i) * W + w] = fminf(fmaxf(fmaf(v.v[i], sc[i], sh[i]), p.lo), p.hi);
        }
        __syncthreads();
        for (int it = threadIdx.x; it < nr * Q; it += 256) {
            const int row = dQ(it), k = it - row * Q;
            int h = h0 + row, b = b0;
            while (h >= p.H) { h -= p.H; ++b; }
            const float4 t = *reinterpret_cast<const float4 *>(tile + row * CW + 4 * k);
            store4(out + ((size_t)h * p.B + b) * CW + 4 * k, F4{{t.x, t.y, t.z, t.w}});
        }
        __syncthreads();
    }
}

template <typename XT, typename DyT, int MODE>
__global__ __launch_bounds__(256) void bn_act_bwd_nhwc_tm_kernel(BnParamsN p, const DyT *dy, double *sums,
                                                                 double n, int training, XT *dx, int TMR) {
    extern __shared__ __attribute__((aligned(16))) float tile[];
    const XT *px = (const XT *)p.x;
    const int C = p.C, W = p.W, CW = C * W, CG = C / 4, Q = CW / 4;
    const int c0 = 4 * ((int)threadIdx.x % CG);
    float m[4], is[4], g[4], be[4], k1[4], k2[4], s[4] = {0.f, 0.f, 0.f, 0.f}, q[4] = {0.f, 0.f, 0.f, 0.f};
#pragma unroll
    for (int i = 0; i < 4; ++i) {
        m[i] = p.mean[c0 + i] - (p.shift ? p.shift[c0 + i] : 0.f);
        is[i] = p.invstd[c0 + i]; g[i] = p.gamma[c0 + i]; be[i] = p.beta[c0 + i];
        k1[i] = MODE == 1 && training ? (float)(sums[2 * (c0 + i)] / n) : 0.f;
        k2[i] = MODE == 1 && training ? (float)(sums[2 * (c0 + i) + 1] / n) : 0.f;
    }
    const int64_t nrows = p.P / W;
    const FastDiv dCG(CG), dW(W), dQ(Q);
    for (int64_t r0 = (int64_t)blockIdx.x * TMR; r0 < nrows; r0 += (int64_t)gridDim.x * TMR) {
        const int nr = nrows - r0 < TMR ? (int)(nrows - r0) : TMR;
        const int b0 = (int)(r0 / p.H), h0 = (int)(r0 - (int64_t)b0 * p.H);
        for (int it = threadIdx.x; it < nr * Q; it += 256) {
            const int row = dQ(it), k = it - row * Q;
            int h = h0 + row, b = b0;
            while (h >= p.H) { h -= p.H; ++b; }
            tm_row_to_lds(dy + ((size_t)h * p.B + b) * CW, tile + row * CW, CW, k);
        }
        __syncthreads();
        for (int it = threadIdx.x; it < nr * W * CG; it += 256) {
            const int j = dCG(it), row = dW(j), w = j - row * W;
            const F4 v = load4(px + (r0 * W + j) * C + c0);
            F4 o;
#pragma unroll
            for (int i = 0; i < 4; ++i) {
                const float xh = (v.v[i] - m[i]) * is[i];
                const float y = fmaf(xh, g[i], be[i]);
                const float d = (y > p.lo && y < p.hi) ? tile[row * CW + (c0 + i) * W + w] : 0.f;
                if (MODE == 0) { s[i] += d; q[i] += d * xh; }
                else o.v[i] = g[i] * is[i] * (d - k1[i] - xh * k2[i]);
            }
            if (MODE == 1) store4(dx + (r0 * W + j) * C + c0, o);
        }
        __syncthreads();
    }
    if (MODE == 0) nhwc_block_atomics(s, q, C, sums);
}

__global__ void bn_param_grads_kernel(const double *sums, int C, const float *gamma,
                                      const float *invstd, int training, float *dgamma,
                                      float *dbeta, float *dshift) {
    const int c = blockIdx.x * blockDim.x + threadIdx.x;
    if (c >= C) return;
    dbeta[c] = (float)sums[2 * c];
    dgamma[c] = (float)sums[2 * c + 1];
    if (dshift) dshift[c] = training ? 0.f : gamma[c] * invstd[c] * (float)sums[2 * c];
}

__global__ void zero_doubles_kernel(double *p, int n) {
    const int i = blockIdx.x * blockDim.x + threadIdx.x;
    if (i < n) p[i] = 0.0;
}

inline int tm_rows(int cw) {
    if (cw <= 0) return 0;
    const int fit = 48 * 1024 / (cw * 4);
    return fit < 8 ? fit : 8;
}

inline bool bad_shape(int B, int C, int H, int W) {
    return B <= 0 || C <= 0 || H <= 0 || W <= 0 || C > 65535 || B > 65535 ||
           (int64_t)H * W > 0x7fffffff;
}

}

extern "C" int64_t asr_bn_act_workspace_bytes(int C) { return C < 0 ? -1 : (int64_t)C * 2 * 8 + 64; }

extern "C" int asr_bn_act_fwd_f32(const void *x, int x_bf16, const float *conv_bias, int B, int C, int H, int W,
                                  const float *gamma, const float *beta,
                                  float *running_mean, float *running_var,
                                  int channels_last,
                                  int training, float momentum, float eps, float lo, float hi,
                                  void *out, int out_bf16, int out_time_major,
                                  float *save_mean, float *save_invstd,
                                  const double *chan_sums,
                                  void *workspace, int64_t workspace_bytes, void *stream) {
    if (bad_shape(B, C, H, W) || !x || !gamma || !beta || !out || !save_mean || !save_invstd)
        return ASR_EINVAL;
    if (!training && (!running_mean || !running_var)) return ASR_EINVAL;
    if (!workspace || workspace_bytes < asr_bn_act_workspace_bytes(C)) return ASR_EINVAL;
    hipStream_t s = (hipStream_t)stream;
    double *sums = (double *)workspace;
    const int HW = H * W;
    const dim3 grid(C, B);
    if (channels_last && (C % 4 != 0 || C > 1024 || 256 % (C / 4) != 0)) return ASR_EUNSUPPORTED;
    if (x_bf16 && !channels_last) return ASR_EUNSUPPORTED;
    const int64_t P = (int64_t)B * HW;
    const int nwg = (int)(P / 64 < 4096 ? (P / 64 > 0 ? P / 64 : 1) : 4096);
    if (training && chan_sums) {
        hipLaunchKernelGGL(bn_finalize_from_sums_kernel, dim3((C + 63) / 64), dim3(64), 0, s, chan_sums,
                           conv_bias, C, (double)B * HW, eps, momentum, save_mean, save_invstd,
                           running_mean, running_var);
    } else if (training) {
        hipLaunchKernelGGL(zero_doubles_kernel, dim3((2 * C + 255) / 256), dim3(256), 0, s, sums, 2 * C);
        if (channels_last)
            if (x_bf16) hipLaunchKernelGGL(bn_stats_nhwc_kernel<__bf16>, dim3(nwg), dim3(256), 0, s, (const __bf16 *)x, conv_bias, P, C, sums);
            else hipLaunchKernelGGL(bn_stats_nhwc_kernel<float>, dim3(nwg), dim3(256), 0, s, (const float *)x, conv_bias, P, C, sums);
        else
            hipLaunchKernelGGL(bn_stats_kernel, grid, dim3(256), 0, s, (const float *)x, conv_bias, C, HW, sums);
        hipLaunchKernelGGL(bn_finalize_kernel, dim3((C + 63) / 64), dim3(64), 0, s, sums, C,
                           (double)B * HW, eps, momentum, save_mean, save_invstd, running_mean,
                           running_var);
    } else {
        hipLaunchKernelGGL(bn_eval_stats_kernel, dim3((C + 63) / 64), dim3(64), 0, s, running_mean,
                           running_var, C, eps, save_mean, save_invstd);
    }
    BnParams p;
    p.x = (const float *)x; p.B = B; p.C = C; p.HW = HW; p.Wd = W; p.gamma = gamma; p.beta = beta;
    p.mean = save_mean; p.invstd = save_invstd; p.shift = conv_bias; p.lo = lo; p.hi = hi;
    if (channels_last) {
        BnParamsN q;
        q.x = x; q.P = P; q.B = B; q.C = C; q.H = H; q.W = W; q.gamma = gamma; q.beta = beta;
        q.mean = save_mean; q.invstd = save_invstd; q.shift = conv_bias; q.lo = lo; q.hi = hi;
        const int cw = C * W, tmr = tm_rows(cw);
        if (out_time_major && cw % 8 == 0 && tmr >= 1) {
            const int64_t rows = (int64_t)B * H;
            const int g2 = (int)((rows + tmr - 1) / tmr < 2048 ? (rows + tmr - 1) / tmr : 2048);
            const size_t lds = (size_t)tmr * cw * 4;
#define ASR_BN_FWDT(XT, OT) \
            hipLaunchKernelGGL((bn_act_fwd_nhwc_tm_kernel<XT, OT>), dim3(g2), dim3(256), lds, s, q, (OT *)out, tmr)
            if (x_bf16) { if (out_bf16) ASR_BN_FWDT(__bf16, __bf16); else ASR_BN_FWDT(__bf16, float); }
            else { if (out_bf16) ASR_BN_FWDT(float, __bf16); else ASR_BN_FWDT(float, float); }
#undef ASR_BN_FWDT
            return hipGetLastError() == hipSuccess ? ASR_OK : ASR_ELAUNCH;
        }
        if (!out_time_major && x_bf16 && C % 8 == 0 && 256 % (C / 8) == 0) {
            if (out_bf16) hipLaunchKernelGGL((bn_act_fwd_nhwc8_kernel<__bf16, __bf16>), dim3(nwg), dim3(256), 0, s, q, (__bf16 *)out);
            else hipLaunchKernelGGL((bn_act_fwd_nhwc8_kernel<__bf16, float>), dim3(nwg), dim3(256), 0, s, q, (float *)out);
            return hipGetLastError() == hipSuccess ? ASR_OK : ASR_ELAUNCH;
        }
#define ASR_BN_FWDN(XT, OT, TMV) \
        hipLaunchKernelGGL((bn_act_fwd_nhwc_kernel<XT, OT, TMV>), dim3(nwg), dim3(256), 0, s, q, (OT *)out)
        if (x_bf16) {
            if (out_bf16) { if (out_time_major) ASR_BN_FWDN(__bf16, __bf16, 1); else ASR_BN_FWDN(__bf16, __bf16, 0); }
            else { if (out_time_major) ASR_BN_FWDN(__bf16, float, 1); else ASR_BN_FWDN(__bf16, float, 0); }
        } else {
            if (out_bf16) { if (out_time_major) ASR_BN_FWDN(float, __bf16, 1); else ASR_BN_FWDN(float, __bf16, 0); }
            else { if (out_time_major) ASR_BN_FWDN(float, float, 1); else ASR_BN_FWDN(float, float, 0); }
        }
#undef ASR_BN_FWDN
        return hipGetLastError() == hipSuccess ? ASR_OK : ASR_ELAUNCH;
    }
    if (out_bf16) {
        if (out_time_major) hipLaunchKernelGGL((bn_act_fwd_kernel<__bf16, 1>), grid, dim3(256), 0, s, p, (__bf16 *)out);
        else hipLaunchKernelGGL((bn_act_fwd_kernel<__bf16, 0>), grid, dim3(256), 0, s, p, (__bf16 *)out);
    } else {
        if (out_time_major) hipLaunchKernelGGL((bn_act_fwd_kernel<float, 1>), grid, dim3(256), 0, s, p, (float *)out);
        else hipLaunchKernelGGL((bn_act_fwd_kernel<float, 0>), grid, dim3(256), 0, s, p, (float *)out);
    }
    return hipGetLastError() == hipSuccess ? ASR_OK : ASR_ELAUNCH;
}

extern "C" int asr_bn_act_bwd_phase_f32(const void *x, int x_bf16, const float *conv_bias, int B, int C, int H, int W,
                                  const float *gamma, const float *beta,
                                  const float *save_mean, const float *save_invstd,
                                  int channels_last,
                                  int training, float lo, float hi,
                                  const void *dy, int dy_bf16, int dy_time_major,
                                  void *dx, float *dgamma, float *dbeta, float *dconv_bias,
                                  void *workspace, int64_t workspace_bytes, int phase,
                                  double n_total, void *stream) {
    if (phase < 0 || phase > 2 || (phase == 2 && !(n_total >= 1.0))) return ASR_EINVAL;
    const bool do_reduce = phase != 2, do_apply = phase != 1;
    if (bad_shape(B, C, H, W) || !x || !gamma || !beta || !save_mean || !save_invstd || !dy ||
        !dx || !dgamma || !dbeta)
        return ASR_EINVAL;
    if (!workspace || workspace_bytes < asr_bn_act_workspace_bytes(C)) return ASR_EINVAL;
    hipStream_t s = (hipStream_t)stream;
    double *sums = (double *)workspace;
    const int HW = H * W;
    const dim3 grid(C, B);
    BnParams p;
    p.x = (const float *)x; p.B = B; p.C = C; p.HW = HW; p.Wd = W; p.gamma = gamma; p.beta = beta;
    p.mean = save_mean; p.invstd = save_invstd; p.shift = conv_bias; p.lo = lo; p.hi = hi;
    const double n = phase == 2 ? n_total : (double)B * HW;
    if (do_reduce)
        hipLaunchKernelGGL(zero_doubles_kernel, dim3((2 * C + 255) / 256), dim3(256), 0, s, sums, 2 * C);
    if (x_bf16 && !channels_last) return ASR_EUNSUPPORTED;
    if (channels_last) {
        if (C % 4 != 0 || C > 1024 || 256 % (C / 4) != 0) return ASR_EUNSUPPORTED;
        BnParamsN q;
        q.x = x; q.P = (int64_t)B * HW; q.B = B; q.C = C; q.H = H; q.W = W; q.gamma = gamma;
        q.beta = beta; q.mean = save_mean; q.invstd = save_invstd; q.shift = conv_bias; q.lo = lo; q.hi = hi;
        const int nwg = (int)(q.P / 64 < 4096 ? (q.P / 64 > 0 ? q.P / 64 : 1) : 4096);
        const int cw = C * W, tmr = tm_rows(cw);
        if (dy_time_major && cw % 8 == 0 && tmr >= 1) {
            const int64_t rows = (int64_t)B * H;
            const int g2 = (int)((rows + tmr - 1) / tmr < 2048 ? (rows + tmr - 1) / tmr : 2048);
            const size_t lds = (size_t)tmr * cw * 4;
#define ASR_BN_BWDT(XT, DT)                                                                          \
            do {                                                                                     \
                if (do_reduce)                                                                       \
                hipLaunchKernelGGL((bn_act_bwd_nhwc_tm_kernel<XT, DT, 0>), dim3(g2), dim3(256), lds, \
                                   s, q, (const DT *)dy, sums, n, training, (XT *)dx, tmr);          \
                if (do_apply)                                                                        \
                hipLaunchKernelGGL((bn_act_bwd_nhwc_tm_kernel<XT, DT, 1>), dim3(g2), dim3(256), lds, \
                                   s, q, (const DT *)dy, sums, n, training, (XT *)dx, tmr);          \
            } while (0)
            if (x_bf16) { if (dy_bf16) ASR_BN_BWDT(__bf16, __bf16); else ASR_BN_BWDT(__bf16, float); }
            else { if (dy_bf16) ASR_BN_BWDT(float, __bf16); else ASR_BN_BWDT(float, float); }
#undef ASR_BN_BWDT
            if (do_reduce) hipLaunchKernelGGL(bn_param_grads_kernel, dim3((C + 63) / 64), dim3(64), 0, s, sums, C, gamma, save_invstd, training, dgamma, dbeta, dconv_bias);
            return hipGetLastError() == hipSuccess ? ASR_OK : ASR_ELAUNCH;
        }
        if (!dy_time_major && x_bf16 && C % 8 == 0 && 256 % (C / 8) == 0) {
#define ASR_BN_BWD8(DT)                                                                            \
            do {                                                                                   \
                if (do_reduce)                                                                     \
                hipLaunchKernelGGL((bn_act_bwd_nhwc8_kernel<__bf16, DT, 0>), dim3(nwg), dim3(256), 0, s, \
                                   q, (const DT *)dy, sums, n, training, (__bf16 *)dx);            \
                if (do_apply)                                                                      \
                hipLaunchKernelGGL((bn_act_bwd_nhwc8_kernel<__bf16, DT, 1>), dim3(nwg), dim3(256), 0, s, \
                                   q, (const DT *)dy, sums, n, training, (__bf16 *)dx);            \
            } while (0)
            if (dy_bf16) ASR_BN_BWD8(__bf16); else ASR_BN_BWD8(float);
#undef ASR_BN_BWD8
            if (do_reduce) hipLaunchKernelGGL(bn_param_grads_kernel, dim3((C + 63) / 64), dim3(64), 0, s, sums, C, gamma, save_invstd, training, dgamma, dbeta, dconv_bias);
            return hipGetLastError() == hipSuccess ? ASR_OK : ASR_ELAUNCH;
        }
#define ASR_BN_BWDN(XT, DT, TMV)                                                                  \
        do {                                                                                      \
            if (do_reduce)                                                                        \
            hipLaunchKernelGGL((bn_act_bwd_reduce_nhwc_kernel<XT, DT, TMV>), dim3(nwg), dim3(256), \
                               0, s, q, (const DT *)dy, sums);                                    \
            if (do_apply)                                                                         \
            hipLaunchKernelGGL((bn_act_bwd_apply_nhwc_kernel<XT, DT, TMV>), dim3(nwg), dim3(256),  \
                               0, s, q, (const DT *)dy, sums, n, training, (XT *)dx);             \
        } while (0)
        if (x_bf16) {
            if (dy_bf16) { if (dy_time_major) ASR_BN_BWDN(__bf16, __bf16, 1); else ASR_BN_BWDN(__bf16, __bf16, 0); }
            else { if (dy_time_major) ASR_BN_BWDN(__bf16, float, 1); else ASR_BN_BWDN(__bf16, float, 0); }
        } else {
            if (dy_bf16) { if (dy_time_major) ASR_BN_BWDN(float, __bf16, 1); else ASR_BN_BWDN(float, __bf16, 0); }
            else { if (dy_time_major) ASR_BN_BWDN(float, float, 1); else ASR_BN_BWDN(float, float, 0); }
        }
#undef ASR_BN_BWDN
        if (do_reduce) hipLaunchKernelGGL(bn_param_grads_kernel, dim3((C + 63) / 64), dim3(64), 0, s, sums, C, gamma, save_invstd, training, dgamma, dbeta, dconv_bias);
        return hipGetLastError() == hipSuccess ? ASR_OK : ASR_ELAUNCH;
    }
#define ASR_BN_BWD(DT, LAY)                                                                       \
    do {                                                                                          \
        if (do_reduce)                                                                            \
        hipLaunchKernelGGL((bn_act_bwd_reduce_kernel<DT, LAY>), grid, dim3(256), 0, s, p,         \
                           (const DT *)dy, sums);                                                 \
        if (do_apply)                                                                             \
        hipLaunchKernelGGL((bn_act_bwd_apply_kernel<DT, LAY>), grid, dim3(256), 0, s, p,          \
                           (const DT *)dy, sums, n, training, (float *)dx);                       \
    } while (0)
    if (dy_bf16) {
        if (dy_time_major) ASR_BN_BWD(__bf16, 1); else ASR_BN_BWD(__bf16, 0);
    } else {
        if (dy_time_major) ASR_BN_BWD(float, 1); else ASR_BN_BWD(float, 0);
    }
#undef ASR_BN_BWD
    if (do_reduce) hipLaunchKernelGGL(bn_param_grads_kernel, dim3((C + 63) / 64), dim3(64), 0, s, sums, C, gamma, save_invstd, training, dgamma, dbeta, dconv_bias);
    return hipGetLastError() == hipSuccess ? ASR_OK : ASR_ELAUNCH;
}

extern "C" int asr_bn_act_bwd_f32(const void *x, int x_bf16, const float *conv_bias, int B, int C, int H, int W,
                                  const float *gamma, const float *beta,
                                  const float *save_mean, const float *save_invstd,
                                  int channels_last,
                                  int training, float lo, float hi,
                                  const void *dy, int dy_bf16, int dy_time_major,
                                  void *dx, float *dgamma, float *dbeta, float *dconv_bias,
                                  void *workspace, int64_t workspace_bytes, void *stream) {
    return asr_bn_act_bwd_phase_f32(x, x_bf16, conv_bias, B, C, H, W, gamma, beta, save_mean, save_invstd,
                                    channels_last, training, lo, hi, dy, dy_bf16, dy_time_major, dx, dgamma,
                                    dbeta, dconv_bias, workspace, workspace_bytes, 0, 0.0, stream);
}
```

pytorch-asr_amd/csrc/common.h:

```cpp
#pragma once
#include <hip/hip_runtime.h>
#include <stdint.h>

#define ASR_WAVE 64

namespace asr {

__device__ __forceinline__ float wave_max(float v) {
#pragma unroll
    for (int o = 32; o > 0; o >>= 1) v = fmaxf(v, __shfl_xor(v, o, ASR_WAVE));
    return v;
}

__device__ __forceinline__ float wave_sum(float v) {
#pragma unroll
    for (int o = 32; o > 0; o >>= 1) v += __shfl_xor(v, o, ASR_WAVE);
    return v;
}

__device__ __forceinline__ float block_max(float v, float *scratch) {
    const int lane = threadIdx.x & 63, w = threadIdx.x >> 6;
    const int nw = (blockDim.x + 63) >> 6;
    v = wave_max(v);
    __syncthreads();
    if (lane == 0) scratch[w] = v;
    __syncthreads();
    float r = scratch[0];
    for (int i = 1; i < nw; ++i) r = fmaxf(r, scratch[i]);
    return r;
}

__device__ __forceinline__ float block_sum(float v, float *scratch) {
    const int lane = threadIdx.x & 63, w = threadIdx.x >> 6;
    const int nw = (blockDim.x + 63) >> 6;
    v = wave_sum(v);
    __syncthreads();
    if (lane == 0) scratch[w] = v;
    __syncthreads();
    float r = scratch[0];
    for (int i = 1; i < nw; ++i) r += scratch[i];
    return r;
}

struct Lse {
    float m, s;
    __device__ __forceinline__ void init() { m = -INFINITY; s = 0.f; }
    __device__ __forceinline__ void add(float v) {
        if (v > m) {
            s = s * __expf(m - v) + 1.f;
            m = v;
        } else {
            s += __expf(v - m);
        }
    }
    __device__ __forceinline__ float value() const { return m + __logf(s); }
};

}
```

pytorch-asr_amd/csrc/conv.hip:

```cpp
#include <type_traits>
#include "common.h"
#include "../../include/asr_amd.h"

namespace {

typedef __attribute__((ext_vector_type(8))) __bf16 bf16x8;
typedef __attribute__((ext_vector_type(16))) float f32x16;
typedef __attribute__((ext_vector_type(4))) unsigned int u32x4;
typedef __attribute__((ext_vector_type(4))) float f32x4;
typedef __attribute__((ext_vector_type(4))) __bf16 bf16x4;

constexpr int CH = 32;
constexpr int KS = 7;
constexpr int PIX = 80;
constexpr int KSTEPS = KS * KS * CH / 16;

typedef __attribute__((ext_vector_type(4))) int rsrc_words;
__device__ __forceinline__ rsrc_words conv_raw_rsrc(const void *base, unsigned bytes) {
    const unsigned long long a = (unsigned long long)base;
    rsrc_words r;
    r.x = __builtin_amdgcn_readfirstlane((int)(unsigned)a);
    r.y = __builtin_amdgcn_readfirstlane((int)((unsigned)(a >> 32) & 0xffffu));
    r.z = __builtin_amdgcn_readfirstlane((int)bytes);
    r.w = 0x00020000;
// ... 361 lines not shown
        if (idx + DG_AD < N) __builtin_amdgcn_sched_group_barrier(0x100, 1, 0);
    }
}

template <int ROLE>
__device__ __forceinline__ void conv_dgrad_wave(const ConvDgradParams &p, char *smem, int lane, int wave) {
    constexpr int NS = ROLE < 2 ? 21 : 28;
    constexpr int FIRST = ROLE == 0 ? 0 : (ROLE == 1 ? 21 : (ROLE == 2 ? 42 : 70));
    constexpr int R = ROLE < 2 ? 0 : ROLE - 1;
    constexpr int HT = DG_NT / 2;
    constexpr int NT = ROLE < 2 ? HT : DG_NT, T0 = ROLE == 1 ? HT : 0;
    constexpr int GIVE0 = ROLE == 0 ? HT : 0;
    constexpr int SLOTS = 14;
    const int W = p.W, Wo = p.Wo, Rq = p.Rq;
    const unsigned img_bytes = (unsigned)(Rq + 2) * (unsigned)p.pitch;
    bf16x8 bf[28];
    {
        const bf16x8 *src = reinterpret_cast<const bf16x8 *>(p.wpack) + (size_t)FIRST * 64 + lane;
#pragma unroll
        for (int s = 0; s < NS; ++s) bf[s] = src[(size_t)s * 64];
    }
    unsigned tab[SLOTS];
    if (ROLE < 2) {
#pragma unroll
        for (int kk = 0; kk < SLOTS; ++kk) {
            const unsigned beta = (unsigned)(SLOTS * ROLE + kk) * 1024u + (unsigned)lane * 16u;
            const unsigned row = beta / (unsigned)p.pitch, rem = beta - row * (unsigned)p.pitch;
            const unsigned col = (rem * 52429u) >> 22, within = rem - col * 80u;
            const int wo = (int)col - 6;
            const bool ok = beta < img_bytes && within < 64u && wo >= 0 && wo < Wo;
            tab[kk] = ok ? (row * (unsigned)Wo + (unsigned)wo) * 64u + within : 0xC0000000u;
        }
    }
    unsigned pixbase[DG_NT];
    const int npix = Rq * W;
#pragma unroll
    for (int i = 0; i < DG_NT; ++i) {
        int m = 32 * i + (lane & 31);
        if (m >= npix) m = npix - 1;
        const int q = m / W, w = m - q * W;
        pixbase[i] = (unsigned)(q * p.pitch + w * PIX + (lane >> 5) * 16);
    }
    const int nq = (p.H + 2) / 3;
    const int tiles = (nq + Rq - 1) / Rq, nitems = tiles * p.B;
    const int nslots = (int)((img_bytes + 1023u) / 1024u);
    constexpr int HALF = HT * 4 * 64 * 16;
    char *epi = smem + nslots * 1024;
    char *part_out = epi + (ROLE == 0 ? 0 : HALF);
    char *part_in = epi + (ROLE == 0 ? HALF : 0);
    char *ocls = ROLE == 0 ? epi + HALF : ROLE == 1 ? epi - T0 * 2048 : epi + 2 * HALF + (R - 1) * DG_PIX * 64;
    const unsigned img_lds = conv_lds_addr(smem);
    const unsigned item_bytes = (unsigned)(p.Ho * Wo * 64);
    auto stage = [&](int it) {
        const int b = it / tiles, q0 = (it - b * tiles) * Rq;
        const rsrc_words yR = conv_raw_rsrc(reinterpret_cast<const char *>(p.dy) + (size_t)b * item_bytes, item_bytes);
        const unsigned base = (unsigned)((q0 - 2) * Wo * 64);
#pragma unroll
        for (int kk = 0; kk < SLOTS; ++kk)
            if (SLOTS * ROLE + kk < nslots)
                conv_dma16(yR, (unsigned)__builtin_amdgcn_readfirstlane((int)(img_lds + (SLOTS * ROLE + kk) * 1024u)),
                           tab[kk] + base, 0u);
    };
    if (ROLE < 2 && (int)blockIdx.x < nitems) stage(blockIdx.x);
    const unsigned wr_base = (unsigned)((lane & 31) * 64 + ((lane >> 5) << 3));
    const unsigned wr_swz = (unsigned)((lane >> 2) & 3);
    const unsigned qmagic = 65536u / (unsigned)W + 1u;
    const int cls_chunks = Rq * W * 4;
    int nst = 0;
    for (int item = blockIdx.x; item < nitems; item += gridDim.x, ++nst) {
        const int b = item / tiles, q0 = (item - b * tiles) * Rq;
        STAMP(0);
        if (ROLE < 2) asm volatile("s_waitcnt vmcnt(0)" ::: "memory");
        __syncthreads();
        f32x16 acc[DG_NT];
        STAMP(1);
        conv_dgrad_part<NS, ROLE == 1 ? 21 : 0>(smem, pixbase, p.pitch, bf, acc);
        STAMP(2);
        if (ROLE < 2) {
#pragma unroll
            for (int i = 0; i < HT; ++i)
#pragma unroll
                for (int g = 0; g < 4; ++g) {
                    const f32x16 &c = acc[GIVE0 + i];
                    *reinterpret_cast<f32x4 *>(part_out + ((i * 4 + g) * 64 + lane) * 16) =
                        f32x4{c[4 * g], c[4 * g + 1], c[4 * g + 2], c[4 * g + 3]};
                }
        }
        STAMP(3);
        __syncthreads();
        STAMP(4);
        if (ROLE < 2 && item + (int)gridDim.x < nitems) stage(item + gridDim.x);
        {
            constexpr int E = NT * 4, RD = ROLE < 2 ? E / 2 : E;
#pragma unroll
            for (int e0 = 0; e0 < E; e0 += RD) {
                f32x4 o[ROLE < 2 ? RD : 1];
                if (ROLE < 2) {
#pragma unroll
                    for (int k = 0; k < RD; ++k)
                        o[k] = *reinterpret_cast<const f32x4 *>(part_in + ((e0 + k) * 64 + lane) * 16);
                    asm volatile("s_waitcnt lgkmcnt(0)" ::: "memory");
                }
#pragma unroll
                for (int k = 0; k < RD; ++k) {
                    const int i = (e0 + k) / 4, g = (e0 + k) % 4;
                    const f32x16 &c = acc[T0 + i];
                    f32x4 v = {c[4 * g], c[4 * g + 1], c[4 * g + 2], c[4 * g + 3]};
                    if (ROLE < 2) v += o[k];
                    bf16x4 o4 = {(__bf16)v[0], (__bf16)v[1], (__bf16)v[2], (__bf16)v[3]};
                    *reinterpret_cast<bf16x4 *>(ocls + (T0 + i) * 2048 + wr_base + (((unsigned)g ^ wr_swz) << 4)) = o4;
                }
            }
        }
        STAMP(5);
        {
            char *xb = reinterpret_cast<char *>(p.dx) + ((size_t)b * p.H + 3 * q0 + R) * W * 64;
            const int qlim = (p.H - R + 2) / 3 - q0;
            int e0 = T0 * 128 + lane;
            asm volatile("" : "+v"(e0));
#pragma unroll
            for (int rd = 0; rd < NT * 2; rd += 6) {
                u32x4 v[6];
#pragma unroll
                for (int it = 0; it < 6; ++it) {
                    const unsigned e = (unsigned)(e0 + 64 * (rd + it)), m = e >> 2;
                    v[it] = *reinterpret_cast<const u32x4 *>(ocls + ((e ^ ((m >> 2) & 3u)) << 4));
                }
#pragma unroll
                for (int it = 0; it < 6; ++it) {
                    const unsigned e = (unsigned)(e0 + 64 * (rd + it)), m = e >> 2, q = (m * qmagic) >> 16;
                    if ((int)e < cls_chunks && (int)q < qlim)
                        *reinterpret_cast<u32x4 *>(xb + (size_t)(e * 16u + q * (unsigned)(2 * W * 64))) = v[it];
                }
            }
        }
        STAMP(6); STAMP(7);
    }
}

__global__ __launch_bounds__(256, 2) void conv7x7c32_dgrad_s3_kernel(ConvDgradParams p) {
    extern __shared__ char smem[];
    const int lane = threadIdx.x & 63;
    const int wave = __builtin_amdgcn_readfirstlane(threadIdx.x >> 6);
    const int role = __builtin_amdgcn_readfirstlane(p.flip && blockIdx.x >= (gridDim.x >> 1) ? 3 - wave : wave);
    if (role == 0) conv_dgrad_wave<0>(p, smem, lane, wave);
    else if (role == 1) conv_dgrad_wave<1>(p, smem, lane, wave);
    else if (role == 2) conv_dgrad_wave<2>(p, smem, lane, wave);
    else conv_dgrad_wave<3>(p, smem, lane, wave);
}


typedef __attribute__((ext_vector_type(4))) short s16x4;
typedef __attribute__((ext_vector_type(8))) short s16x8;
typedef __attribute__((address_space(3))) s16x4 lds_s16x4;

__device__ __forceinline__ bf16x8 tr_frag(const char *addr) {
    const s16x4 lo = __builtin_amdgcn_ds_read_tr16_b64_v4i16((lds_s16x4 *)(addr));
    const s16x4 hi = __builtin_amdgcn_ds_read_tr16_b64_v4i16((lds_s16x4 *)(addr + 4 * PIX));
    s16x8 v;
    v.s0 = lo.x; v.s1 = lo.y; v.s2 = lo.z; v.s3 = lo.w;
    v.s4 = hi.x; v.s5 = hi.y; v.s6 = hi.z; v.s7 = hi.w;
    return __builtin_bit_cast(bf16x8, v);
}

constexpr int WGRAD_WGS = 256;
constexpr int WGRAD_NT = 448;
constexpr int NX_MAX = 8, ND_MAX = 3;

struct ConvWgradParams {
    const __bf16 *x, *dy;
    float *partial;
    int B, H, W, Ho, Wo, KW;
    int rows;
};

__global__ __launch_bounds__(WGRAD_NT) void conv7x7c32_wgrad_s3_kernel(ConvWgradParams p) {
    extern __shared__ char smem[];
    const int tid = threadIdx.x, lane = tid & 63;
    const int wave = __builtin_amdgcn_readfirstlane(tid >> 6);
    const int W = p.W, Wo = p.Wo, KW = p.KW, Wd = 16 * KW, rows = p.rows;
    const int xrows = 3 * (rows - 1) + KS;
    char *ximg = smem;
    char *dimg = smem + (size_t)(xrows * W + 24) * PIX;
    const int kt = wave;
    f32x16 acc[KS];
#pragma unroll
    for (int f = 0; f < KS; ++f)
#pragma unroll
        for (int j = 0; j < 16; ++j) acc[f][j] = 0.f;
    const unsigned lane_off = (unsigned)((8 * (lane >> 5) + ((lane & 15) >> 2)) * PIX +
                                         (16 * ((lane >> 4) & 1) + 4 * (lane & 3)) * 2);
    for (int i = tid; i < 24 * PIX / 4; i += WGRAD_NT)
        reinterpret_cast<unsigned *>(ximg + (size_t)xrows * W * PIX)[i] = 0u;
    const int chunks_per_utt = (p.Ho + rows - 1) / rows;
    const int nchunks = p.B * chunks_per_utt;
    const int nx = xrows * W * 4, nd = rows * Wd * 4;
    u32x4 sx[NX_MAX], sd[ND_MAX];
    const unsigned wmagic = (1u << 20) / (unsigned)W + 1u, dmagic = (1u << 20) / (unsigned)Wd + 1u;
    auto fetch = [&](int c) {
        const int b = c / chunks_per_utt, ho0 = (c - b * chunks_per_utt) * rows;
        const char *xb = reinterpret_cast<const char *>(p.x) + (size_t)b * p.H * W * 64;
        const char *yb = reinterpret_cast<const char *>(p.dy) + (size_t)b * p.Ho * Wo * 64;
#pragma unroll
        for (int k = 0; k < NX_MAX; ++k) {
            const int i = tid + k * WGRAD_NT;
            const int pix = i >> 2, part = i & 3, row = (int)(((unsigned)pix * wmagic) >> 20);
            u32x4 v = {0u, 0u, 0u, 0u};
            if (i < nx && 3 * ho0 + row < p.H)
                v = *reinterpret_cast<const u32x4 *>(xb + ((size_t)(3 * ho0) * W + pix) * 64 + part * 16);
            sx[k] = v;
        }
#pragma unroll
        for (int k = 0; k < ND_MAX; ++k) {
            const int i = tid + k * WGRAD_NT;
            const int pix = i >> 2, part = i & 3, row = (int)(((unsigned)pix * dmagic) >> 20), wo = pix - row * Wd;
            u32x4 v = {0u, 0u, 0u, 0u};
            if (i < nd && ho0 + row < p.Ho && wo < Wo)
                v = *reinterpret_cast<const u32x4 *>(yb + ((size_t)(ho0 + row) * Wo + wo) * 64 + part * 16);
            sd[k] = v;
        }
    };
    auto stage = [&]() {
#pragma unroll
        for (int k = 0; k < NX_MAX; ++k) {
            const int i = tid + k * WGRAD_NT;
            if (i < nx) *reinterpret_cast<u32x4 *>(ximg + (i >> 2) * PIX + (i & 3) * 16) = sx[k];
        }
#pragma unroll
        for (int k = 0; k < ND_MAX; ++k) {
            const int i = tid + k * WGRAD_NT;
            if (i < nd) *reinterpret_cast<u32x4 *>(dimg + (i >> 2) * PIX + (i & 3) * 16) = sd[k];
        }
    };
    int c = blockIdx.x;
    if (c < nchunks) fetch(c);
    __syncthreads();
    if (c < nchunks) stage();
    __syncthreads();
    for (; c < nchunks; c += gridDim.x) {
        const int next = c + gridDim.x;
        if (next < nchunks) fetch(next);
        for (int r = 0; r < rows; ++r) {
            for (int ks = 0; ks < KW; ++ks) {
                const bf16x8 a = tr_frag(dimg + (size_t)(r * Wd + 16 * ks) * PIX + lane_off);
                const char *xr = ximg + (size_t)((3 * r + kt) * W + 16 * ks) * PIX + lane_off;
#pragma unroll
                for (int f = 0; f < KS; ++f) {
                    const bf16x8 bb = tr_frag(xr + f * PIX);
                    acc[f] = __builtin_amdgcn_mfma_f32_32x32x16_bf16(a, bb, acc[f], 0, 0, 0);
                }
            }
        }
        __syncthreads();
        if (next < nchunks) stage();
        __syncthreads();
    }
    float *out = p.partial + (size_t)blockIdx.x * 49 * 1024;
#pragma unroll
    for (int f = 0; f < KS; ++f)
#pragma unroll
        for (int j = 0; j < 16; ++j) out[((kt * KS + f) * 16 + j) * 64 + lane] = acc[f][j];
}

__device__ __forceinline__ float partial_sum(const float *partial, int nparts, int n, float *lds) {
    const int el = threadIdx.x & 63, part = threadIdx.x >> 6, ways = blockDim.x >> 6;
    const int e = blockIdx.x * 64 + el;
    float s = 0.f;
    if (e < n)
        for (int g = part; g < nparts; g += ways) s += partial[(size_t)g * n + e];
    lds[part * 64 + el] = s;
    __syncthreads();
    float t = 0.f;
    for (int w = 0; w < ways; ++w) t += lds[w * 64 + el];
    return t;
}

__global__ __launch_bounds__(1024) void conv_wgrad_reduce_kernel(const float *partial, int nwg, float *dw) {
    __shared__ float lds4[1024];
    const float s = partial_sum(partial, nwg, 49 * 1024, lds4);
    const int e = blockIdx.x * 64 + (threadIdx.x & 63);
    if (threadIdx.x >= 64 || e >= 49 * 1024) return;
    const int tap = e >> 10, j = (e >> 6) & 15, l = e & 63;
    const int co = (j & 3) + 8 * (j >> 2) + 4 * (l >> 5), ci = l & 31;
    dw[(co * CH + ci) * 49 + tap] = s;
}


constexpr int C1_ROWS = 16;

__global__ void conv1_pack_kernel(const float *w, __bf16 *out) {
    const int i = blockIdx.x * blockDim.x + threadIdx.x;
    if (i >= 4 * 64 * 8) return;
    const int j = i & 7, l = (i >> 3) & 63, s = i >> 9;
    const int kt = 2 * s + (l >> 5), kf = j, co = l & 31;
    out[i] = (kt < KS && kf < KS) ? (__bf16)w[(co * KS + kt) * KS + kf] : (__bf16)0.f;
}

struct Conv1Params {
    const float *x;
    const __bf16 *wpack;
    __bf16 *y;
    float *partial;
    int B, T, F, To, Fo;
};

__device__ __forceinline__ void conv1_stage_windows(const Conv1Params &p, int b, int t0, int nrows,
                                                    char *wimg, int tid, int nt) {
    const float *xb = p.x + (size_t)b * p.T * p.F;
    const unsigned fmagic = (1u << 20) / (unsigned)p.Fo + 1u;
    for (int i = tid; i < nrows * p.Fo; i += nt) {
        const unsigned row = ((unsigned)i * fmagic) >> 20, fo = (unsigned)i - row * (unsigned)p.Fo;
        const int t = t0 - 6 + (int)row;
        bf16x8 v = {};
        if (t >= 0 && t < p.T) {
            const float2 *src = reinterpret_cast<const float2 *>(xb + (size_t)t * p.F + 2 * fo);
#pragma unroll
            for (int j = 0; j < 4; ++j) {
                const float2 f2 = src[j];
                v[2 * j] = (__bf16)f2.x;
                v[2 * j + 1] = (__bf16)f2.y;
            }
        }
        *reinterpret_cast<bf16x8 *>(wimg + (size_t)i * 16) = v;
    }
}

__global__ __launch_bounds__(256) void conv1_fwd_kernel(Conv1Params p) {
    extern __shared__ char smem[];
    const int tid = threadIdx.x, lane = tid & 63;
    const int wave = __builtin_amdgcn_readfirstlane(tid >> 6);
    const int b = blockIdx.y, t0 = blockIdx.x * C1_ROWS, Fo = p.Fo;
    const int npix = C1_ROWS * Fo, ntiles = (npix + 31) >> 5;
    char *wimg = smem;
    __bf16 *oimg = reinterpret_cast<__bf16 *>(smem + (size_t)(C1_ROWS + 8) * Fo * 16);
    bf16x8 bf[4];
#pragma unroll
    for (int s = 0; s < 4; ++s) bf[s] = reinterpret_cast<const bf16x8 *>(p.wpack)[s * 64 + lane];
    conv1_stage_windows(p, b, t0, C1_ROWS + 8, wimg, tid, 256);
    __syncthreads();
    const unsigned fmagic = (1u << 20) / (unsigned)Fo + 1u;
    for (int tile = wave; tile < ntiles; tile += 4) {
        int m = 32 * tile + (lane & 31);
        if (m >= npix) m = npix - 1;
        const unsigned r = ((unsigned)m * fmagic) >> 20, fo = (unsigned)m - r * (unsigned)Fo;
        const char *base = wimg + (size_t)((r + (unsigned)(lane >> 5)) * (unsigned)Fo + fo) * 16;
        bf16x8 a[4];
#pragma unroll
        for (int s = 0; s < 4; ++s) a[s] = *reinterpret_cast<const bf16x8 *>(base + (size_t)(2 * s * Fo) * 16);
        f32x16 acc = {};
#pragma unroll
        for (int s = 0; s < 4; ++s) acc = __builtin_amdgcn_mfma_f32_32x32x16_bf16(bf[s], a[s], acc, 0, 0, 0);
#pragma unroll
        for (int g = 0; g < 4; ++g) {
            bf16x4 o4 = {(__bf16)acc[4 * g], (__bf16)acc[4 * g + 1], (__bf16)acc[4 * g + 2], (__bf16)acc[4 * g + 3]};
            *reinterpret_cast<bf16x4 *>(reinterpret_cast<char *>(oimg) + (size_t)(32 * tile + (lane & 31)) * 64 +
                                        16 * g + 8 * (lane >> 5)) = o4;
        }
    }
    __syncthreads();
    const int rows_here = (p.To - t0) < C1_ROWS ? (p.To - t0) : C1_ROWS;
    char *yb = reinterpret_cast<char *>(p.y) + ((size_t)b * p.To + t0) * Fo * 64;
    for (int c = tid; c < rows_here * Fo * 4; c += 256)
        *reinterpret_cast<u32x4 *>(yb + (size_t)c * 16) =
            *reinterpret_cast<const u32x4 *>(reinterpret_cast<const char *>(oimg) + (size_t)c * 16);
    if (p.partial)
        chan_partial_sums(oimg, rows_here * Fo, reinterpret_cast<float *>(oimg + (size_t)ntiles * 32 * CH),
                          p.partial + ((size_t)blockIdx.y * gridDim.x + blockIdx.x) * 64);
}

constexpr int C1_WGS = 1024;
template <int DI, int WPT>
__global__ __launch_bounds__(256) void conv1_wgrad_kernel(Conv1Params p) {
    extern __shared__ char smem[];
    const int tid = threadIdx.x, lane = tid & 63;
    const int wave = __builtin_amdgcn_readfirstlane(tid >> 6);
    const int Fo = p.Fo, npix = C1_ROWS * Fo, nks = npix >> 4;
    const int nwin = (C1_ROWS + 8) * Fo;
    char *wimg = smem;
    char *dimg = smem + (size_t)nwin * 16;
    f32x16 acc[2];
#pragma unroll
    for (int t = 0; t < 2; ++t)
#pragma unroll
        for (int j = 0; j < 16; ++j) acc[t][j] = 0.f;
    const int h = lane >> 5, q = (lane & 15) >> 2, pp = lane & 3, chalf = (lane >> 4) & 1;
    const unsigned a_off = (unsigned)((8 * h + q) * PIX + (16 * chalf + 4 * pp) * 2);
    const int ktl = 2 * chalf + (pp >> 1);
    const unsigned b_lane = (unsigned)(8 * (pp & 1));
    const int chunks_per_utt = (p.To + C1_ROWS - 1) / C1_ROWS;
    const int nchunks = p.B * chunks_per_utt;
    const unsigned fmagic = (1u << 20) / (unsigned)Fo + 1u;
    u32x4 dreg[DI];
    float2 wreg[WPT][4];
    auto fetch = [&](int c) {
        const int b = c / chunks_per_utt, t0 = (c - b * chunks_per_utt) * C1_ROWS;
        const char *yb = reinterpret_cast<const char *>(p.y) + ((size_t)b * p.To + t0) * Fo * 64;
        const int rows_here = (p.To - t0) < C1_ROWS ? (p.To - t0) : C1_ROWS;
#pragma unroll
        for (int k = 0; k < DI; ++k) {
            const int i = tid + 256 * k, pix = i >> 2;
            dreg[k] = pix < rows_here * Fo ? *reinterpret_cast<const u32x4 *>(yb + (size_t)i * 16) : u32x4{0u, 0u, 0u, 0u};
        }
        const float *xb = p.x + (size_t)b * p.T * p.F;
#pragma unroll
        for (int u = 0; u < WPT; ++u) {
            const unsigned i = (unsigned)(tid + 256 * u);
            const unsigned row = (i * fmagic) >> 20, fo = i - row * (unsigned)Fo;
            const int t = t0 - 6 + (int)row;
            const bool ok = (int)i < nwin && t >= 0 && t < p.T;
            const float2 *src = reinterpret_cast<const float2 *>(xb + (size_t)(ok ? t : 0) * p.F + 2 * fo);
#pragma unroll
            for (int j = 0; j < 4; ++j) wreg[u][j] = ok ? src[j] : float2{0.f, 0.f};
        }
    };
    auto stash = [&]() {
#pragma unroll
        for (int k = 0; k < DI; ++k) {
            const int i = tid + 256 * k, pix = i >> 2, part = i & 3;
            if (pix < npix) *reinterpret_cast<u32x4 *>(dimg + pix * PIX + part * 16) = dreg[k];
        }
#pragma unroll
        for (int u = 0; u < WPT; ++u) {
            const int i = tid + 256 * u;
            bf16x8 v;
#pragma unroll
            for (int j = 0; j < 4; ++j) { v[2 * j] = (__bf16)wreg[u][j].x; v[2 * j + 1] = (__bf16)wreg[u][j].y; }
            if (i < nwin) *reinterpret_cast<bf16x8 *>(wimg + (size_t)i * 16) = v;
        }
    };
    if ((int)blockIdx.x < nchunks) fetch(blockIdx.x);
    for (int c = blockIdx.x; c < nchunks; c += gridDim.x) {
        __syncthreads();
        stash();
        __syncthreads();
        if (c + (int)gridDim.x < nchunks) fetch(c + gridDim.x);
        for (int ks = wave; ks < nks; ks += 4) {
            const bf16x8 a = tr_frag(dimg + (size_t)(16 * ks) * PIX + a_off);
            const unsigned p0 = (unsigned)(16 * ks + 8 * h + q), p1 = p0 + 4;
            const unsigned r0 = (p0 * fmagic) >> 20, f0 = p0 - r0 * (unsigned)Fo;
            const unsigned r1 = (p1 * fmagic) >> 20, f1 = p1 - r1 * (unsigned)Fo;
#pragma unroll
            for (int nt = 0; nt < 2; ++nt) {
                const int kt = 4 * nt + ktl;
                const s16x4 lo = __builtin_amdgcn_ds_read_tr16_b64_v4i16(
                    (lds_s16x4 *)(wimg + (size_t)((r0 + kt) * Fo + f0) * 16 + b_lane));
                const s16x4 hi = __builtin_amdgcn_ds_read_tr16_b64_v4i16(
                    (lds_s16x4 *)(wimg + (size_t)((r1 + kt) * Fo + f1) * 16 + b_lane));
                s16x8 v;
                v.s0 = lo.x; v.s1 = lo.y; v.s2 = lo.z; v.s3 = lo.w;
                v.s4 = hi.x; v.s5 = hi.y; v.s6 = hi.z; v.s7 = hi.w;
                acc[nt] = __builtin_amdgcn_mfma_f32_32x32x16_bf16(a, __builtin_bit_cast(bf16x8, v), acc[nt], 0, 0, 0);
            }
        }
    }
    __syncthreads();
    float *red = reinterpret_cast<float *>(smem);
#pragma unroll
    for (int nt = 0; nt < 2; ++nt)
#pragma unroll
        for (int j = 0; j < 16; ++j) red[((wave * 2 + nt) * 16 + j) * 64 + lane] = acc[nt][j];
    __syncthreads();
    float *out = p.partial + (size_t)blockIdx.x * 2 * 1024;
    for (int e = tid; e < 2 * 1024; e += 256)
        out[e] = red[e] + red[2048 + e] + red[4096 + e] + red[6144 + e];
}

__global__ __launch_bounds__(1024) void conv1_wgrad_reduce_kernel(const float *partial, int nparts, float *dw) {
    __shared__ float lds4[1024];
    const float s = partial_sum(partial, nparts, 2 * 1024, lds4);
    const int e = blockIdx.x * 64 + (threadIdx.x & 63);
    if (threadIdx.x >= 64) return;
    const int nt = e >> 10, j = (e >> 6) & 15, l = e & 63;
    const int co = (j & 3) + 8 * (j >> 2) + 4 * (l >> 5), tap = 32 * nt + (l & 31);
    const int kt = tap >> 3, kf = tap & 7;
    if (kt < KS && kf < KS) dw[(co * KS + kt) * KS + kf] = s;
}


template <int CIN>
__global__ void conv1c_pack_kernel(const float *w, __bf16 *out) {
    const int i = blockIdx.x * blockDim.x + threadIdx.x;
    if (i >= CIN * 4 * 64 * 8) return;
    const int j = i & 7, l = (i >> 3) & 63, s = (i >> 9) & 3, ci = i >> 11;
    const int kt = 2 * s + (l >> 5), kf = j, co = l & 31;
    out[i] = (kt < KS && kf < KS) ? (__bf16)w[((co * CIN + ci) * KS + kt) * KS + kf] : (__bf16)0.f;
}

template <int CIN, int RPT>
__device__ __forceinline__ void conv1c_raw_load(const Conv1Params &p, const float *xb, int t0, int nrows,
                                                int tid, float (&r)[RPT]) {
    const int FC = p.F * CIN;
    const unsigned mg = ((1u << 24) + (unsigned)FC - 1u) / (unsigned)FC;
    const float *base = xb + (ptrdiff_t)(t0 - 6) * FC;
#pragma unroll
    for (int k = 0; k < RPT; ++k) {
        const int e = tid + 256 * k;
        const int t = t0 - 6 + (int)(((unsigned)e * mg) >> 24);
        r[k] = (e < nrows * FC && t >= 0 && t < p.T) ? base[e] : 0.f;
    }
}
template <int CIN, int RPT>
__device__ __forceinline__ void conv1c_raw_stash(const Conv1Params &p, int nrows, int FP, int tid,
                                                 const float (&r)[RPT], __bf16 *planes) {
    const int FC = p.F * CIN;
    const unsigned mg = ((1u << 24) + (unsigned)FC - 1u) / (unsigned)FC;
#pragma unroll
    for (int k = 0; k < RPT; ++k) {
        const int e = tid + 256 * k;
        if (e < nrows * FC) {
            const int row = (int)(((unsigned)e * mg) >> 24), rem = e - row * FC, f = rem / CIN, ci = rem - f * CIN;
            planes[(ci * nrows + row) * FP + f] = (__bf16)r[k];
        }
    }
    for (int i = tid; i < CIN * nrows * (FP - p.F); i += 256) {
        const int rp = i / (FP - p.F), f = p.F + (i - rp * (FP - p.F));
        planes[rp * FP + f] = (__bf16)0.f;
    }
}
template <int CIN>
__device__ __forceinline__ void conv1c_build_windows(int nrows, int Fo, int FP, int tid,
                                                     const __bf16 *planes, char *wimg) {
    const unsigned fmagic = (1u << 20) / (unsigned)Fo + 1u;
    for (int i = tid; i < CIN * nrows * Fo; i += 256) {
        const unsigned rp = ((unsigned)i * fmagic) >> 20, fo = (unsigned)i - rp * (unsigned)Fo;
        const unsigned *src = reinterpret_cast<const unsigned *>(planes + (size_t)rp * FP + 2 * fo);
        u32x4 v;
        v.x = src[0]; v.y = src[1]; v.z = src[2]; v.w = src[3];
        *reinterpret_cast<u32x4 *>(wimg + (size_t)i * 16) = v;
    }
}

template <int CIN, int ROWS, int RPT>
__global__ __launch_bounds__(256) void conv1c_fwd_kernel(Conv1Params p) {
    extern __shared__ char smem[];
    const int tid = threadIdx.x, lane = tid & 63;
    const int wave = __builtin_amdgcn_readfirstlane(tid >> 6);
    const int Fo = p.Fo;
    const int npix = ROWS * Fo, ntiles = (npix + 31) >> 5, nwin1 = (ROWS + 8) * Fo;
    const int FP = (2 * (Fo - 1) + 8 + 3) & ~3;
    char *wimg = smem;
    __bf16 *oimg = reinterpret_cast<__bf16 *>(smem + (size_t)CIN * nwin1 * 16);
    __bf16 *planes = oimg;
    const unsigned fmagic = (1u << 20) / (unsigned)Fo + 1u;
    bf16x8 bw[CIN * 4];
#pragma unroll
    for (int k = 0; k < CIN * 4; ++k) bw[k] = reinterpret_cast<const bf16x8 *>(p.wpack)[k * 64 + lane];
    const int chunks_per_utt = (p.To + ROWS - 1) / ROWS;
    const int nchunks = p.B * chunks_per_utt;
    float rreg[RPT];
    auto fetch = [&](int c) {
        const int b = c / chunks_per_utt, t0 = (c - b * chunks_per_utt) * ROWS;
        conv1c_raw_load<CIN, RPT>(p, p.x + (size_t)b * p.T * p.F * CIN, t0, ROWS + 8, tid, rreg);
    };
    if ((int)blockIdx.x < nchunks) fetch(blockIdx.x);
    for (int c = blockIdx.x; c < nchunks; c += gridDim.x) {
        const int b = c / chunks_per_utt, t0 = (c - b * chunks_per_utt) * ROWS;
        __syncthreads();
        conv1c_raw_stash<CIN, RPT>(p, ROWS + 8, FP, tid, rreg, planes);
        __syncthreads();
        if (c + (int)gridDim.x < nchunks) fetch(c + gridDim.x);
        conv1c_build_windows<CIN>(ROWS + 8, Fo, FP, tid, planes, wimg);
        __syncthreads();
        for (int tile = wave; tile < ntiles; tile += 4) {
            int m = 32 * tile + (lane & 31);
            if (m >= npix) m = npix - 1;
            const unsigned r = ((unsigned)m * fmagic) >> 20, fo = (unsigned)m - r * (unsigned)Fo;
            const char *base = wimg + (size_t)((r + (unsigned)(lane >> 5)) * (unsigned)Fo + fo) * 16;
            f32x16 acc = {};
#pragma unroll
            for (int ci = 0; ci < CIN; ++ci)
#pragma unroll
                for (int s4 = 0; s4 < 4; ++s4) {
                    const bf16x8 a = *reinterpret_cast<const bf16x8 *>(base + (size_t)(ci * nwin1 + 2 * s4 * Fo) * 16);
                    acc = __builtin_amdgcn_mfma_f32_32x32x16_bf16(bw[ci * 4 + s4], a, acc, 0, 0, 0);
                }
#pragma unroll
            for (int g = 0; g < 4; ++g) {
                bf16x4 o4 = {(__bf16)acc[4 * g], (__bf16)acc[4 * g + 1], (__bf16)acc[4 * g + 2], (__bf16)acc[4 * g + 3]};
                *reinterpret_cast<bf16x4 *>(reinterpret_cast<char *>(oimg) + (size_t)(32 * tile + (lane & 31)) * 64 +
                                            16 * g + 8 * (lane >> 5)) = o4;
            }
        }
        __syncthreads();
        const int rows_here = (p.To - t0) < ROWS ? (p.To - t0) : ROWS;
        char *yb = reinterpret_cast<char *>(p.y) + ((size_t)b * p.To + t0) * Fo * 64;
        for (int cc = tid; cc < rows_here * Fo * 4; cc += 256)
            *reinterpret_cast<u32x4 *>(yb + (size_t)cc * 16) =
                *reinterpret_cast<const u32x4 *>(reinterpret_cast<const char *>(oimg) + (size_t)cc * 16);
        if (p.partial)
            chan_partial_sums(oimg, rows_here * Fo, reinterpret_cast<float *>(oimg + (size_t)ntiles * 32 * CH),
                              p.partial + (size_t)c * 64);
    }
}

template <int CIN, int ROWS, int DI, int RPT>
__global__ __launch_bounds__(256) void conv1c_wgrad_kernel(Conv1Params p) {
    extern __shared__ char smem[];
    const int tid = threadIdx.x, lane = tid & 63;
    const int wave = __builtin_amdgcn_readfirstlane(tid >> 6);
    const int Fo = p.Fo, npix = ROWS * Fo, nks = npix >> 4;
    const int nwin1 = (ROWS + 8) * Fo;
    const int FP = (2 * (Fo - 1) + 8 + 3) & ~3;
    char *wimg = smem;
    char *dimg = smem + (size_t)CIN * nwin1 * 16;
    __bf16 *planes = reinterpret_cast<__bf16 *>(dimg + (size_t)npix * PIX);
    f32x16 acc[2 * CIN];
#pragma unroll
    for (int t = 0; t < 2 * CIN; ++t)
#pragma unroll
        for (int j = 0; j < 16; ++j) acc[t][j] = 0.f;
    const int h = lane >> 5, q = (lane & 15) >> 2, pp = lane & 3, chalf = (lane >> 4) & 1;
    const unsigned a_off = (unsigned)((8 * h + q) * PIX + (16 * chalf + 4 * pp) * 2);
    const int ktl = 2 * chalf + (pp >> 1);
    const unsigned b_lane = (unsigned)(8 * (pp & 1));
    const int chunks_per_utt = (p.To + ROWS - 1) / ROWS;
    const int nchunks = p.B * chunks_per_utt;
    const unsigned fmagic = (1u << 20) / (unsigned)Fo + 1u;
    u32x4 dreg[DI];
    float rreg[RPT];
    auto fetch = [&](int c) {
        const int b = c / chunks_per_utt, t0 = (c - b * chunks_per_utt) * ROWS;
        const char *yb = reinterpret_cast<const char *>(p.y) + ((size_t)b * p.To + t0) * Fo * 64;
        const int rows_here = (p.To - t0) < ROWS ? (p.To - t0) : ROWS;
#pragma unroll
        for (int k = 0; k < DI; ++k) {
            const int i = tid + 256 * k, pix = i >> 2;
            dreg[k] = pix < rows_here * Fo ? *reinterpret_cast<const u32x4 *>(yb + (size_t)i * 16) : u32x4{0u, 0u, 0u, 0u};
        }
        conv1c_raw_load<CIN, RPT>(p, p.x + (size_t)b * p.T * p.F * CIN, t0, ROWS + 8, tid, rreg);
    };
    auto stash = [&]() {
#pragma unroll
        for (int k = 0; k < DI; ++k) {
            const int i = tid + 256 * k, pix = i >> 2, part = i & 3;
            if (pix < npix) *reinterpret_cast<u32x4 *>(dimg + pix * PIX + part * 16) = dreg[k];
        }
        conv1c_raw_stash<CIN, RPT>(p, ROWS + 8, FP, tid, rreg, planes);
    };
    if ((int)blockIdx.x < nchunks) fetch(blockIdx.x);
    for (int c = blockIdx.x; c < nchunks; c += gridDim.x) {
        __syncthreads();
        stash();
        __syncthreads();
        if (c + (int)gridDim.x < nchunks) fetch(c + gridDim.x);
        conv1c_build_windows<CIN>(ROWS + 8, Fo, FP, tid, planes, wimg);
        __syncthreads();
        for (int ks = wave; ks < nks; ks += 4) {
            const bf16x8 a = tr_frag(dimg + (size_t)(16 * ks) * PIX + a_off);
            const unsigned p0 = (unsigned)(16 * ks + 8 * h + q), p1 = p0 + 4;
            const unsigned r0 = (p0 * fmagic) >> 20, f0 = p0 - r0 * (unsigned)Fo;
            const unsigned r1 = (p1 * fmagic) >> 20, f1 = p1 - r1 * (unsigned)Fo;
#pragma unroll
            for (int nt = 0; nt < 2 * CIN; ++nt) {
                const int kt = 4 * (nt & 1) + ktl;
                const char *plane = wimg + (size_t)(nt >> 1) * nwin1 * 16;
                const s16x4 lo = __builtin_amdgcn_ds_read_tr16_b64_v4i16(
                    (lds_s16x4 *)(plane + (size_t)((r0 + kt) * Fo + f0) * 16 + b_lane));
                const s16x4 hi = __builtin_amdgcn_ds_read_tr16_b64_v4i16(
                    (lds_s16x4 *)(plane + (size_t)((r1 + kt) * Fo + f1) * 16 + b_lane));
                s16x8 v;
                v.s0 = lo.x; v.s1 = lo.y; v.s2 = lo.z; v.s3 = lo.w;
                v.s4 = hi.x; v.s5 = hi.y; v.s6 = hi.z; v.s7 = hi.w;
                acc[nt] = __builtin_amdgcn_mfma_f32_32x32x16_bf16(a, __builtin_bit_cast(bf16x8, v), acc[nt], 0, 0, 0);
            }
        }
    }
    float *red = reinterpret_cast<float *>(smem);
    float *out = p.partial + (size_t)blockIdx.x * 2 * CIN * 1024;
#pragma unroll
    for (int nt = 0; nt < 2 * CIN; ++nt) {
        __syncthreads();
#pragma unroll
        for (int j = 0; j < 16; ++j) red[(wave * 16 + j) * 64 + lane] = acc[nt][j];
        __syncthreads();
        for (int e = tid; e < 1024; e += 256)
            out[nt * 1024 + e] = (red[e] + red[1024 + e]) + (red[2048 + e] + red[3072 + e]);
    }
}

template <int CIN>
__global__ __launch_bounds__(1024) void conv1c_wgrad_reduce_kernel(const float *partial, int nparts, float *dw) {
    __shared__ float lds4[1024];
    const float s = partial_sum(partial, nparts, 2 * CIN * 1024, lds4);
    const int e = blockIdx.x * 64 + (threadIdx.x & 63);
    if (threadIdx.x >= 64) return;
    const int nt = e >> 10, j = (e >> 6) & 15, l = e & 63;
    const int ci = nt >> 1;
    const int co = (j & 3) + 8 * (j >> 2) + 4 * (l >> 5), tap = 32 * (nt & 1) + (l & 31);
    const int kt = tap >> 3, kf = tap & 7;
    if (kt < KS && kf < KS) dw[((co * CIN + ci) * KS + kt) * KS + kf] = s;
}

}


#ifdef CONV_STAMPS
static long long *stamp_buf() {
    static long long *d = nullptr;
    if (!d && getenv("ASR_CONV_STAMPS")) { hipMalloc(&d, 4 * 64 * 8 * 8); }
    if (d) hipMemset(d, 0, 4 * 64 * 8 * 8);
    return d;
}
static hipEvent_t stamp_ev[2];
static void stamp_begin(hipStream_t s) {
    if (!stamp_ev[0]) { hipEventCreate(&stamp_ev[0]); hipEventCreate(&stamp_ev[1]); }
    hipEventRecord(stamp_ev[0], s);
}
static void stamp_dump(const char *name, long long *d, hipStream_t s) {
    if (!d) return;
    hipEventRecord(stamp_ev[1], s);
    hipDeviceSynchronize();
    float ms = 0;
    hipEventElapsedTime(&ms, stamp_ev[0], stamp_ev[1]);
    static long long h[4 * 64 * 8];
    hipMemcpy(h, d, sizeof(h), hipMemcpyDeviceToHost);
    for (int w = 0; w < 4; ++w)
        for (int lo = 2; lo < 30; lo += 14) {
            double avg[9] = {0};
            for (int it = lo; it < lo + 12; ++it) {
                for (int k = 1; k < 8; ++k) avg[k] += (double)(h[(w * 64 + it) * 8 + k] - h[(w * 64 + it) * 8 + k - 1]) / 12;
                avg[8] += (double)(h[(w * 64 + it + 1) * 8] - h[(w * 64 + it) * 8]) / 12;
            }
            fprintf(stderr, "%s wave %d items %d..%d avg:", name, w, lo, lo + 11);
            for (int k = 1; k < 8; ++k) fprintf(stderr, " %6.0f", avg[k]);
            fprintf(stderr, "  | total %.0f\n", avg[8]);
        }
    fprintf(stderr, "%s kernel %.1f us; items 0..30 of block 7 took %lld ticks\n", name, ms * 1e3, h[30 * 8] - h[0]);
}
#endif

extern "C" int64_t asr_conv7x7c32_workspace_bytes(void) {
    return (int64_t)KSTEPS * 64 * 8 * 2 * 2 + (int64_t)WGRAD_WGS * 49 * 1024 * 4 + 256;
}

extern "C" int asr_conv7x7c32_fwd_bf16(const void *x, const float *w, int B, int H, int W,
                                       int stride_h, void *y, double *chan_sums, void *workspace,
                                       int64_t workspace_bytes, void *stream) {
    if (B <= 0 || H < KS || W < KS) return ASR_EINVAL;
    if (!x || !w || !y || !workspace || workspace_bytes < asr_conv7x7c32_workspace_bytes())
        return ASR_EINVAL;
    if (stride_h != 1 && stride_h != 3) return ASR_EUNSUPPORTED;
    const int Ho = (H - KS) / stride_h + 1, Wo = W - KS + 1;
    if (Wo > 48) return ASR_EUNSUPPORTED;
    int R = FWD_PIX / Wo;
    if (R > 16) R = 16;
    const int pitch = pick_row_pitch(W * PIX, Wo, stride_h, R * Wo, 2 * FWD_NT);
    const size_t img = ((size_t)(stride_h * (R - 1) + KS) * pitch + 1023) / 1024 * 1024;
    if ((int64_t)H * W * 64 >= (1ll << 31)) return ASR_EUNSUPPORTED;
    if (img > (size_t)4 * FWD_MAXQ * 1024) return ASR_EUNSUPPORTED;
    const size_t lds = img + img / 8 + 4 * 4096 + 2048;
    if (lds > 80 * 1024) return ASR_EUNSUPPORTED;
    hipStream_t s = (hipStream_t)stream;
    __bf16 *wpack = (__bf16 *)workspace;
    hipLaunchKernelGGL(conv_pack_fwd_kernel, dim3((KSTEPS * 64 * 8 + 255) / 256), dim3(256), 0, s, w, wpack);
    ConvFwdParams p;
    p.x = (const __bf16 *)x; p.wpack = wpack; p.y = (__bf16 *)y;
    p.B = B; p.H = H; p.W = W; p.Ho = Ho; p.Wo = Wo; p.R = R; p.pitch = pitch;
    const int nitems = ((Ho + R - 1) / R) * B;
    int wgs = 2 * conv_cu_count();
    if (wgs <= 0) wgs = 512;
    if (wgs > nitems) wgs = nitems;
    const dim3 grid(wgs);
    p.stats = chan_sums ? (float *)((char *)workspace + (size_t)KSTEPS * 64 * 8 * 2 * 2) : nullptr;
    if (chan_sums && (int64_t)wgs * 4 * 64 * 4 > (int64_t)WGRAD_WGS * 49 * 1024 * 4) return ASR_EUNSUPPORTED;
    void (*kern)(ConvFwdParams) = stride_h == 3 ? conv7x7c32_fwd_kernel<3> : conv7x7c32_fwd_kernel<1>;
    if (lds > 64 * 1024 &&
        hipFuncSetAttribute((const void *)kern, hipFuncAttributeMaxDynamicSharedMemorySize, (int)lds) != hipSuccess)
        return ASR_EUNSUPPORTED;
#ifdef CONV_STAMPS
    p.stamps = stamp_buf();
    stamp_begin(s);
#else
    p.stamps = nullptr;
#endif
    hipLaunchKernelGGL(kern, grid, dim3(256), lds, s, p);
#ifdef CONV_STAMPS
    stamp_dump("fwd", p.stamps, s);
#endif
    if (chan_sums) {
        hipLaunchKernelGGL(zero_chan_sums_kernel, dim3(1), dim3(64), 0, s, chan_sums);
        hipLaunchKernelGGL(chan_sums_reduce_kernel, dim3(64), dim3(1024), 0, s, p.stats, wgs * 4, chan_sums);
    }
    return hipGetLastError() == hipSuccess ? ASR_OK : ASR_ELAUNCH;
}

extern "C" int asr_conv7x7c32_bwd_data_bf16(const void *dy, const float *w, int B, int H, int W,
                                            int stride_h, void *dx, void *workspace,
                                            int64_t workspace_bytes, void *stream) {
    if (B <= 0 || H < KS || W < KS) return ASR_EINVAL;
    if (!dy || !w || !dx || !workspace || workspace_bytes < asr_conv7x7c32_workspace_bytes())
        return ASR_EINVAL;
    if (stride_h != 3) return ASR_EUNSUPPORTED;
    const int Ho = (H - KS) / stride_h + 1, Wo = W - KS + 1;
    if (W > 48) return ASR_EUNSUPPORTED;
    int Rq = DG_PIX / W;
    if (Rq > 16) Rq = 16;
    const int pitch = pick_row_pitch((Wo + 12) * PIX, W, 1, Rq * W, DG_NT);
    const size_t img = ((size_t)(Rq + 2) * pitch + 1023) / 1024 * 1024;
    if ((int64_t)B * Ho * Wo * 64 >= (1ll << 31)) return ASR_EUNSUPPORTED;
    const size_t epi = (size_t)DG_NT * 4 * 64 * 16 + (size_t)2 * DG_PIX * CH * 2;
    const size_t lds = img + epi;
    if (lds > 80 * 1024 || img > 28 * 1024) return ASR_EUNSUPPORTED;
    hipStream_t s = (hipStream_t)stream;
    __bf16 *wpack = (__bf16 *)workspace + (size_t)KSTEPS * 64 * 8;
    hipLaunchKernelGGL(conv_pack_dgrad_kernel, dim3((KSTEPS * 64 * 8 + 255) / 256), dim3(256), 0, s, w, wpack);
    ConvDgradParams p;
    p.dy = (const __bf16 *)dy; p.wpack = wpack; p.dx = (__bf16 *)dx;
    p.B = B; p.H = H; p.W = W; p.Ho = Ho; p.Wo = Wo; p.Rq = Rq; p.pitch = pitch;
    const int nq = (H + 2) / 3;
    const int nitems = ((nq + Rq - 1) / Rq) * B;
    int wgs = 2 * conv_cu_count();
    if (wgs <= 0) wgs = 512;
    p.flip = wgs <= nitems;
    if (wgs > nitems) wgs = nitems;
    const dim3 grid(wgs);
    if (lds > 64 * 1024 &&
        hipFuncSetAttribute((const void *)conv7x7c32_dgrad_s3_kernel,
                            hipFuncAttributeMaxDynamicSharedMemorySize, (int)lds) != hipSuccess)
        return ASR_EUNSUPPORTED;
#ifdef CONV_STAMPS
    p.stamps = stamp_buf();
    stamp_begin(s);
#else
    p.stamps = nullptr;
#endif
    hipLaunchKernelGGL(conv7x7c32_dgrad_s3_kernel, grid, dim3(256), lds, s, p);
#ifdef CONV_STAMPS
    stamp_dump("dgrad", p.stamps, s);
#endif
    return hipGetLastError() == hipSuccess ? ASR_OK : ASR_ELAUNCH;
}

extern "C" int asr_conv7x7c32_wgrad_bf16(const void *x, const void *dy, int B, int H, int W,
                                         int stride_h, float *dw, void *workspace,
                                         int64_t workspace_bytes, void *stream) {
    if (B <= 0 || H < KS || W < KS) return ASR_EINVAL;
    if (!x || !dy || !dw || !workspace || workspace_bytes < asr_conv7x7c32_workspace_bytes())
        return ASR_EINVAL;
    if (stride_h != 3) return ASR_EUNSUPPORTED;
    const int Ho = (H - KS) / stride_h + 1, Wo = W - KS + 1;
    if (Wo > 48) return ASR_EUNSUPPORTED;
    const int KW = (Wo + 15) / 16;
    int rows = 8;
    size_t lds = 0;
    for (; rows >= 1; rows >>= 1) {
        const int xrows = 3 * (rows - 1) + KS;
        lds = (size_t)(xrows * W + 24) * PIX + (size_t)rows * 16 * KW * PIX;
        if (lds <= 72 * 1024 && xrows * W * 4 <= NX_MAX * WGRAD_NT && rows * 16 * KW * 4 <= ND_MAX * WGRAD_NT)
            break;
    }
    if (rows < 1) return ASR_EUNSUPPORTED;
    hipStream_t s = (hipStream_t)stream;
    ConvWgradParams p;
    p.x = (const __bf16 *)x; p.dy = (const __bf16 *)dy;
    p.partial = (float *)((char *)workspace + (size_t)KSTEPS * 64 * 8 * 2 * 2);
    p.B = B; p.H = H; p.W = W; p.Ho = Ho; p.Wo = Wo; p.KW = KW; p.rows = rows;
    const int chunks = B * ((Ho + rows - 1) / rows);
    const int nwg = chunks < WGRAD_WGS ? chunks : WGRAD_WGS;
    if (lds > 64 * 1024 &&
        hipFuncSetAttribute((const void *)conv7x7c32_wgrad_s3_kernel,
                            hipFuncAttributeMaxDynamicSharedMemorySize, (int)lds) != hipSuccess)
        return ASR_EUNSUPPORTED;
    hipLaunchKernelGGL(conv7x7c32_wgrad_s3_kernel, dim3(nwg), dim3(WGRAD_NT), lds, s, p);
    hipLaunchKernelGGL(conv_wgrad_reduce_kernel, dim3(49 * 1024 / 64), dim3(256), 0, s,
                       p.partial, nwg, dw);
    return hipGetLastError() == hipSuccess ? ASR_OK : ASR_ELAUNCH;
}

extern "C" int64_t asr_conv1_7x7s2_workspace_bytes(void) {
    return 4 * 64 * 8 * 2 + (int64_t)(1 << 17) * 64 * 4 + 256;
}

static int conv1_shapes(int B, int T, int F, int *To, int *Fo) {
    if (B <= 0 || T <= 0 || F < KS) return ASR_EINVAL;
    *To = T + 2 * 6 - KS + 1;
    *Fo = (F - KS) / 2 + 1;
    if (*Fo > 64) return ASR_EUNSUPPORTED;
    return ASR_OK;
}

extern "C" int asr_conv1_7x7s2_fwd(const float *x, const float *w, int B, int T, int F, void *y,
                                   double *chan_sums, void *workspace, int64_t workspace_bytes,
                                   void *stream) {
    int To, Fo;
    const int rc = conv1_shapes(B, T, F, &To, &Fo);
    if (rc != ASR_OK) return rc;
    if (!x || !w || !y || !workspace || workspace_bytes < asr_conv1_7x7s2_workspace_bytes())
        return ASR_EINVAL;
    hipStream_t s = (hipStream_t)stream;
    __bf16 *wpack = (__bf16 *)workspace;
    hipLaunchKernelGGL(conv1_pack_kernel, dim3(8), dim3(256), 0, s, w, wpack);
    Conv1Params p;
    p.x = x; p.wpack = wpack; p.y = (__bf16 *)y;
    p.B = B; p.T = T; p.F = F; p.To = To; p.Fo = Fo;
    const dim3 grid((To + C1_ROWS - 1) / C1_ROWS, B);
    p.partial = chan_sums ? (float *)((char *)workspace + 4 * 64 * 8 * 2) : nullptr;
    if (chan_sums && (int64_t)grid.x * grid.y * 64 * 4 > asr_conv1_7x7s2_workspace_bytes() - 4 * 64 * 8 * 2 - 256)
        return ASR_EUNSUPPORTED;
    const int ntiles = (C1_ROWS * Fo + 31) / 32;
    const size_t lds = (size_t)(C1_ROWS + 8) * Fo * 16 + (size_t)ntiles * 32 * CH * 2 + 512 * 4;
    if (lds > 64 * 1024) return ASR_EUNSUPPORTED;
    hipLaunchKernelGGL(conv1_fwd_kernel, grid, dim3(256), lds, s, p);
    if (chan_sums) {
        hipLaunchKernelGGL(zero_chan_sums_kernel, dim3(1), dim3(64), 0, s, chan_sums);
        hipLaunchKernelGGL(chan_sums_reduce_kernel, dim3(64), dim3(1024), 0, s, p.partial, (int)(grid.x * grid.y), chan_sums);
    }
    return hipGetLastError() == hipSuccess ? ASR_OK : ASR_ELAUNCH;
}

extern "C" int asr_conv1_7x7s2_wgrad(const float *x, const void *dy, int B, int T, int F,
                                     float *dw, void *workspace, int64_t workspace_bytes,
                                     void *stream) {
    int To, Fo;
    const int rc = conv1_shapes(B, T, F, &To, &Fo);
    if (rc != ASR_OK) return rc;
    if (!x || !dy || !dw || !workspace || workspace_bytes < asr_conv1_7x7s2_workspace_bytes())
        return ASR_EINVAL;
    hipStream_t s = (hipStream_t)stream;
    Conv1Params p;
    p.x = x; p.wpack = nullptr; p.y = (__bf16 *)const_cast<void *>(dy);
    p.partial = (float *)((char *)workspace + 4 * 64 * 8 * 2);
    p.B = B; p.T = T; p.F = F; p.To = To; p.Fo = Fo;
    size_t lds = (size_t)(C1_ROWS + 8) * Fo * 16 + (size_t)C1_ROWS * Fo * PIX;
    if (lds < 4 * 2 * 1024 * 4) lds = 4 * 2 * 1024 * 4;
    if (lds > 64 * 1024) return ASR_EUNSUPPORTED;
    const int chunks = B * ((To + C1_ROWS - 1) / C1_ROWS);
    const int nwg = chunks < C1_WGS ? chunks : C1_WGS;
    const int di = (C1_ROWS * Fo * 4 + 255) / 256, wpt = ((C1_ROWS + 8) * Fo + 255) / 256;
    void (*kern)(Conv1Params) = di <= 5 && wpt <= 2 ? conv1_wgrad_kernel<5, 2>
                              : (di <= 8 && wpt <= 3 ? conv1_wgrad_kernel<8, 3> : conv1_wgrad_kernel<16, 6>);
    hipLaunchKernelGGL(kern, dim3(nwg), dim3(256), lds, s, p);
    hipLaunchKernelGGL(conv1_wgrad_reduce_kernel, dim3(2 * 1024 / 64), dim3(1024), 0, s, p.partial, nwg, dw);
    return hipGetLastError() == hipSuccess ? ASR_OK : ASR_ELAUNCH;
}


extern "C" int64_t asr_conv1c_7x7s2_workspace_bytes(int cin) {
    if (cin != 3) return -1;
    const int64_t wg = (int64_t)C1_WGS * 2 * cin * 1024 * 4, cs = (int64_t)(1 << 17) * 64 * 4;
    return (int64_t)cin * 4 * 64 * 8 * 2 + (wg > cs ? wg : cs) + 256;
}

extern "C" int asr_conv1c_7x7s2_fwd(const float *x, const float *w, int B, int T, int F, int cin, void *y,
                                    double *chan_sums, void *workspace, int64_t workspace_bytes,
                                    void *stream) {
    int To, Fo;
    const int rc = conv1_shapes(B, T, F, &To, &Fo);
    if (rc != ASR_OK) return rc;
    if (cin != 3 || (Fo & 1)) return ASR_EUNSUPPORTED;
    if (!x || !w || !y || !workspace || workspace_bytes < asr_conv1c_7x7s2_workspace_bytes(cin))
        return ASR_EINVAL;
    if ((int64_t)T * F * cin * 4 * B >= (1ll << 40)) return ASR_EUNSUPPORTED;
    hipStream_t s = (hipStream_t)stream;
    __bf16 *wpack = (__bf16 *)workspace;
    hipLaunchKernelGGL(conv1c_pack_kernel<3>, dim3(3 * 8), dim3(256), 0, s, w, wpack);
    Conv1Params p;
    p.x = x; p.wpack = wpack; p.y = (__bf16 *)y;
    p.B = B; p.T = T; p.F = F; p.To = To; p.Fo = Fo;
    constexpr int ROWS = 8;
    const int64_t nchunks = (int64_t)B * ((To + ROWS - 1) / ROWS);
    if (nchunks >= (1ll << 31)) return ASR_EUNSUPPORTED;
    const dim3 grid((unsigned)(nchunks < 768 ? nchunks : 768));
    p.partial = chan_sums ? (float *)((char *)workspace + 3 * 4 * 64 * 8 * 2) : nullptr;
    if (chan_sums && nchunks * 64 * 4 > (int64_t)(1 << 17) * 64 * 4) return ASR_EUNSUPPORTED;
    const int ntiles = (ROWS * Fo + 31) / 32;
    const int FP = (2 * (Fo - 1) + 8 + 3) & ~3;
    size_t otail = (size_t)ntiles * 32 * CH * 2 + 512 * 4;
    if (otail < (size_t)3 * (ROWS + 8) * FP * 2) otail = (size_t)3 * (ROWS + 8) * FP * 2;
    const size_t lds = (size_t)3 * (ROWS + 8) * Fo * 16 + otail;
    const int rpt = ((ROWS + 8) * F * 3 + 255) / 256;
    if (lds > 64 * 1024 || rpt > 24) return ASR_EUNSUPPORTED;
    if (rpt <= 16) hipLaunchKernelGGL((conv1c_fwd_kernel<3, ROWS, 16>), grid, dim3(256), lds, s, p);
    else hipLaunchKernelGGL((conv1c_fwd_kernel<3, ROWS, 24>), grid, dim3(256), lds, s, p);
    if (chan_sums) {
        hipLaunchKernelGGL(zero_chan_sums_kernel, dim3(1), dim3(64), 0, s, chan_sums);
        hipLaunchKernelGGL(chan_sums_reduce_kernel, dim3(64), dim3(1024), 0, s, p.partial, (int)nchunks, chan_sums);
    }
    return hipGetLastError() == hipSuccess ? ASR_OK : ASR_ELAUNCH;
}

extern "C" int asr_conv1c_7x7s2_wgrad(const float *x, const void *dy, int B, int T, int F, int cin,
                                      float *dw, void *workspace, int64_t workspace_bytes,
                                      void *stream) {
    int To, Fo;
    const int rc = conv1_shapes(B, T, F, &To, &Fo);
    if (rc != ASR_OK) return rc;
    if (cin != 3 || (Fo & 1)) return ASR_EUNSUPPORTED;
    if (!x || !dy || !dw || !workspace || workspace_bytes < asr_conv1c_7x7s2_workspace_bytes(cin))
        return ASR_EINVAL;
    hipStream_t s = (hipStream_t)stream;
    constexpr int ROWS = 8;
    Conv1Params p;
    p.x = x; p.wpack = nullptr; p.y = (__bf16 *)const_cast<void *>(dy);
    p.partial = (float *)((char *)workspace + 3 * 4 * 64 * 8 * 2);
    p.B = B; p.T = T; p.F = F; p.To = To; p.Fo = Fo;
    const int FP = (2 * (Fo - 1) + 8 + 3) & ~3;
    size_t lds = (size_t)3 * (ROWS + 8) * Fo * 16 + (size_t)ROWS * Fo * PIX + (size_t)3 * (ROWS + 8) * FP * 2;
    if (lds < 4 * 1024 * 4) lds = 4 * 1024 * 4;
    if (lds > 64 * 1024) return ASR_EUNSUPPORTED;
    const int chunks = B * ((To + ROWS - 1) / ROWS);
    const int nwg = chunks < C1_WGS ? chunks : C1_WGS;
    const int di = (ROWS * Fo * 4 + 255) / 256, rpt = ((ROWS + 8) * F * 3 + 255) / 256;
    if (di > 8 || rpt > 24) return ASR_EUNSUPPORTED;
    void (*kern)(Conv1Params) = di <= 5 && rpt <= 16 ? conv1c_wgrad_kernel<3, ROWS, 5, 16>
                                                      : conv1c_wgrad_kernel<3, ROWS, 8, 24>;
    hipLaunchKernelGGL(kern, dim3(nwg), dim3(256), lds, s, p);
    hipLaunchKernelGGL(conv1c_wgrad_reduce_kernel<3>, dim3(2 * 3 * 1024 / 64), dim3(1024), 0, s, p.partial, nwg, dw);
    return hipGetLastError() == hipSuccess ? ASR_OK : ASR_ELAUNCH;
}
```

Baseline: 37.32 million frames/s.

## Fuse first conv with batch-norm and hardtanh, recomputing conv output in backward

Adds a fused conv1+BN+hardtanh path. Forward runs the conv twice: first to accumulate channel statistics, then again to apply BN and the activation in the epilogue, so the raw conv output never goes to memory. Backward recomputes the conv to form the BN reduction sums and applies the BN/activation backward inside the wgrad kernel. This removes the separate BN kernels and the memory traffic for the intermediate tensor, at the cost of extra conv recomputation and more kernel launches.

After: 37.41 million frames/s, median of 2. Within noise of the previous version (+0.2%).

```diff
diff --git a/include/asr_amd.h b/include/asr_amd.h
--- a/include/asr_amd.h
+++ b/include/asr_amd.h
@@ -207,6 +207,19 @@
                         double *chan_sums, void *workspace, int64_t workspace_bytes, void *stream);
 int asr_conv1_7x7s2_wgrad(const float *x, const void *dy, int B, int T, int F, float *dw,
                           void *workspace, int64_t workspace_bytes, void *stream);
+
+int asr_conv1_bn_act_fwd(const float *x, const float *w, const float *conv_bias, int B, int T,
+                         int F, const float *gamma, const float *beta, float *running_mean,
+                         float *running_var, int training, float momentum, float eps, float lo,
+                         float hi, void *out, float *save_mean, float *save_invstd,
+                         double *chan_sums, void *workspace, int64_t workspace_bytes, int phase,
+                         void *stream);
+int asr_conv1_bn_act_bwd(const float *x, const float *w, const float *conv_bias, int B, int T,
+                         int F, const float *gamma, const float *beta, const float *save_mean,
+                         const float *save_invstd, int training, float lo, float hi,
+                         const void *dy, float *dw, float *dgamma, float *dbeta,
+                         float *dconv_bias, double *sums, void *workspace,
+                         int64_t workspace_bytes, int phase, double n_total, void *stream);
 
 int64_t asr_conv1c_7x7s2_workspace_bytes(int cin);
 int asr_conv1c_7x7s2_fwd(const float *x, const float *w, int B, int T, int F, int cin, void *y,
diff --git a/pytorch-asr_amd/att_speech/_native.py b/pytorch-asr_amd/att_speech/_native.py
--- a/pytorch-asr_amd/att_speech/_native.py
+++ b/pytorch-asr_amd/att_speech/_native.py
@@ -47,6 +47,10 @@
     'asr_conv1_7x7s2_workspace_bytes': (_i64, []),
     'asr_conv1_7x7s2_fwd': (_i, [_vp, _vp, _i, _i, _i, _vp, _vp, _vp, _i64, _vp]),
     'asr_conv1_7x7s2_wgrad': (_i, [_vp, _vp, _i, _i, _i, _vp, _vp, _i64, _vp]),
+    'asr_conv1_bn_act_fwd': (_i, [_vp, _vp, _vp, _i, _i, _i, _vp, _vp, _vp, _vp, _i, _f, _f, _f, _f, _vp,
+                                  _vp, _vp, _vp, _vp, _i64, _i, _vp]),
+    'asr_conv1_bn_act_bwd': (_i, [_vp, _vp, _vp, _i, _i, _i, _vp, _vp, _vp, _vp, _i, _f, _f, _vp, _vp,
+                                  _vp, _vp, _vp, _vp, _vp, _i64, _i, ctypes.c_double, _vp]),
     'asr_conv1c_7x7s2_workspace_bytes': (_i64, [_i]),
     'asr_conv1c_7x7s2_fwd': (_i, [_vp, _vp, _i, _i, _i, _i, _vp, _vp, _vp, _i64, _vp]),
     'asr_conv1c_7x7s2_wgrad': (_i, [_vp, _vp, _i, _i, _i, _i, _vp, _vp, _i64, _vp]),
@@ -1277,6 +1281,83 @@
     return dw
 
 
+def conv1_bn_supported(F):
+    return F >= 7 and (F - 7) // 2 + 1 <= 36
+
+
+def conv1_bn_act_fwd(x, weight, conv_bias, gamma, beta, running_mean, running_var, training,
+                     momentum, eps, lo, hi, sync=None):
+    x = _dev(x, torch.float32, 'x')
+    weight = _dev(weight, torch.float32, 'weight')
+    gamma = _dev(gamma, torch.float32, 'gamma')
+    beta = _dev(beta, torch.float32, 'beta')
+    if conv_bias is not None:
+        conv_bias = _dev(conv_bias, torch.float32, 'conv_bias')
+    B, T, F = x.shape
+    if tuple(weight.shape) != (32, 1, 7, 7):
+        raise ValueError('conv1_bn_act_fwd: weight must be [32, 1, 7, 7]')
+    To, Fo = T + 6, (F - 7) // 2 + 1
+    out = torch.empty((B, 32, To, Fo), dtype=torch.bfloat16, device=x.device,
+                      memory_format=torch.channels_last)
+    mean = torch.empty(32, dtype=torch.float32, device=x.device)
+    invstd = torch.empty(32, dtype=torch.float32, device=x.device)
+    sums = torch.empty((2, 32), dtype=torch.float64, device=x.device) if training else None
+    L = lib()
+    nbytes = L.asr_conv1_7x7s2_workspace_bytes()
+    ws = torch.empty(nbytes, dtype=torch.uint8, device=x.device)
+
+    def phase(k):
+        check(L.asr_conv1_bn_act_fwd(
+            _p(x), _p(weight), _p(conv_bias), B, T, F, _p(gamma), _p(beta), _p(running_mean),
+            _p(running_var), int(bool(training)), float(momentum), float(eps), float(lo), float(hi),
+            _p(out), _p(mean), _p(invstd), _p(sums), _p(ws), nbytes, k, _stream()),
+            'asr_conv1_bn_act_fwd')
+    if sync is not None and training:
+        phase(1)
+        sync(sums, float(B) * To * Fo)
+        phase(2)
+    else:
+        phase(0)
+    return out, mean, invstd
+
+
+def conv1_bn_act_bwd(x, weight, conv_bias, gamma, beta, mean, invstd, training, lo, hi, dy,
+                     sync=None):
+    x = _dev(x, torch.float32, 'x')
+    weight = _dev(weight, torch.float32, 'weight')
+    gamma = _dev(gamma, torch.float32, 'gamma')
+    beta = _dev(beta, torch.float32, 'beta')
+    dy = _nhwc_bf16(dy, 'dy')[0]
+    B, T, F = x.shape
+    To, Fo = T + 6, (F - 7) // 2 + 1
+    if tuple(dy.shape) != (B, 32, To, Fo):
+        raise ValueError('conv1_bn_act_bwd: dy must be [%d, 32, %d, %d]' % (B, To, Fo))
+    dev = x.device
+    dw = torch.empty((32, 1, 7, 7), dtype=torch.float32, device=dev)
+    dgamma = torch.empty(32, dtype=torch.float32, device=dev)
+    dbeta = torch.empty(32, dtype=torch.float32, device=dev)
+    dcb = None
+    if conv_bias is not None:
+        conv_bias = _dev(conv_bias, torch.float32, 'conv_bias')
+        dcb = torch.empty(32, dtype=torch.float32, device=dev)
+    sums = torch.empty(64, dtype=torch.float64, device=dev)
+    L = lib()
+    nbytes = L.asr_conv1_7x7s2_workspace_bytes()
+    ws = torch.empty(nbytes, dtype=torch.uint8, device=dev)
+
+    def phase(k, n_total):
+        check(L.asr_conv1_bn_act_bwd(
+            _p(x), _p(weight), _p(conv_bias), B, T, F, _p(gamma), _p(beta), _p(mean), _p(invstd),
+            int(bool(training)), float(lo), float(hi), _p(dy), _p(dw), _p(dgamma), _p(dbeta), _p(dcb),
+            _p(sums), _p(ws), nbytes, k, float(n_total), _stream()), 'asr_conv1_bn_act_bwd')
+    if sync is not None and training:
+        phase(1, 0.0)
+        phase(2, sync(sums, float(B) * To * Fo))
+    else:
+        phase(0, 0.0)
+    return dw, dgamma, dbeta, dcb
+
+
 def split_bf16(x, hi=None, lo=None):
     x = _dev(x, torch.float32, 'x')
     if hi is None:
diff --git a/pytorch-asr_amd/att_speech/modules/encoders/deep_speech_2.py b/pytorch-asr_amd/att_speech/modules/encoders/deep_speech_2.py
--- a/pytorch-asr_amd/att_speech/modules/encoders/deep_speech_2.py
+++ b/pytorch-asr_amd/att_speech/modules/encoders/deep_speech_2.py
@@ -114,8 +114,12 @@
             from att_speech.modules.encoders import native_conv
             c1 = conv[0]
             sums1 = sums2 = None
-            if bf16 and self.native_conv and native_conv.first_supported(c1, features):
+            if bf16 and self.native_conv and native_conv.conv1_bn_fused(c1, features):
+                x = native_conv.conv1_bn_hardtanh(features, c1, conv[1].batch_norm, conv[2])
+            elif bf16 and self.native_conv and native_conv.first_supported(c1, features):
                 x, sums1 = native_conv.conv1(features, c1)
+                x = bn_hardtanh(x, conv[1].batch_norm, conv[2], out_bf16=bf16, conv_bias=c1.bias,
+                                chan_sums=sums1)
             else:
                 if bf16 and self.native_conv and not getattr(self, '_warned_conv1', False):
                     self._warned_conv1 = True
@@ -123,8 +127,7 @@
                                   'shape on gradient-free features csrc/conv.hip is built for; using '
                                   'torch / MIOpen for it')
                 x = run_conv(c1, features, with_bias=False, keep_bf16=True)
-            x = bn_hardtanh(x, conv[1].batch_norm, conv[2], out_bf16=bf16, conv_bias=c1.bias,
-                            chan_sums=sums1)
+                x = bn_hardtanh(x, conv[1].batch_norm, conv[2], out_bf16=bf16, conv_bias=c1.bias)
             if bf16 and self.native_conv and native_conv.supported(c2, x):
                 y2, sums2 = native_conv.conv7x7c32(x, c2)
             else:
diff --git a/pytorch-asr_amd/att_speech/modules/encoders/native_conv.py b/pytorch-asr_amd/att_speech/modules/encoders/native_conv.py
--- a/pytorch-asr_amd/att_speech/modules/encoders/native_conv.py
+++ b/pytorch-asr_amd/att_speech/modules/encoders/native_conv.py
@@ -1,3 +1,5 @@
+import os
+
 import torch
 
 from att_speech import _native
@@ -63,5 +65,68 @@
     return Conv1Function.apply(features.permute(0, 2, 3, 1), conv.weight)
 
 
+def conv1_bn_fused(conv, features):
+    return (os.environ.get('ASR_CONV1_FUSED', '1') != '0' and conv.in_channels == 1
+            and first_supported(conv, features) and _native.conv1_bn_supported(features.size(3)))
+
+
+class Conv1BNActFunction(torch.autograd.Function):
+
+    @staticmethod
+    def forward(ctx, x, weight, conv_bias, gamma, beta, running_mean, running_var, training,
+                momentum, eps, lo, hi, sync_fwd):
+        from att_speech.modules.encoders import native_bn
+        x = x.float().contiguous()
+        ctx.sync = bool(training) and native_bn._sync_active()
+        counts = []
+
+        def sync_sums(sums, n_local):
+            n_total = native_bn._allreduce_sums(sums, n_local)
+            sums.mul_(n_local / n_total)
+            counts.append((n_local, n_total))
+
+        out, mean, invstd = _native.conv1_bn_act_fwd(
+            x, weight.detach(), None if conv_bias is None else conv_bias.detach(), gamma.detach(),
+            beta.detach(), running_mean, running_var, training, momentum, eps, lo, hi,
+            sync=sync_sums if sync_fwd else None)
+        if counts and running_var is not None and momentum:
+            nl, nt = counts[0]
+            var = invstd.double().pow(-2) - eps
+            running_var.add_((momentum * var * (nt / (nt - 1.0) - nl / (nl - 1.0))).float())
+        ctx.has_cb = conv_bias is not None
+        ctx.save_for_backward(x, weight, gamma, beta, mean, invstd,
+                              conv_bias if conv_bias is not None else gamma)
+        ctx.cfg = (training, lo, hi)
+        return out
+
+    @staticmethod
+    def backward(ctx, dy):
+        from att_speech.modules.encoders import native_bn
+        x, weight, gamma, beta, mean, invstd, cb = ctx.saved_tensors
+        training, lo, hi = ctx.cfg
+        dw, dgamma, dbeta, dcb = _native.conv1_bn_act_bwd(
+            x, weight.detach(), cb.detach() if ctx.has_cb else None, gamma.detach(), beta.detach(),
+            mean, invstd, training, lo, hi, dy,
+            sync=native_bn._allreduce_sums if ctx.sync else None)
+        return (None, dw, dcb, dgamma, dbeta) + (None,) * 8
+
+
+def conv1_bn_hardtanh(features, conv, bn, act):
+    use_batch_stats = bn.training or bn.running_mean is None
+    momentum = 0.0
+    rm = rv = None
+    if use_batch_stats and bn.training and bn.track_running_stats and bn.running_mean is not None:
+        bn.num_batches_tracked.add_(1)
+        momentum = bn.momentum if bn.momentum is not None else 1.0 / float(bn.num_batches_tracked)
+        rm, rv = bn.running_mean, bn.running_var
+    elif not use_batch_stats:
+        rm, rv = bn.running_mean, bn.running_var
+    from att_speech.modules.encoders import native_bn
+    sync_fwd = use_batch_stats and bn.training and native_bn._sync_active()
+    return Conv1BNActFunction.apply(features[:, 0], conv.weight, conv.bias, bn.weight, bn.bias, rm, rv,
+                                    use_batch_stats, momentum, bn.eps, float(act.min_val),
+                                    float(act.max_val), sync_fwd)
+
+
 def conv7x7c32(x, conv):
     return Conv7x7C32Function.apply(x, conv.weight)
diff --git a/pytorch-asr_amd/csrc/bnact.hip b/pytorch-asr_amd/csrc/bnact.hip
--- a/pytorch-asr_amd/csrc/bnact.hip
+++ b/pytorch-asr_amd/csrc/bnact.hip
@@ -567,6 +567,30 @@
 inline bool bad_shape(int B, int C, int H, int W) {
     return B <= 0 || C <= 0 || H <= 0 || W <= 0 || C > 65535 || B > 65535 ||
            (int64_t)H * W > 0x7fffffff;
+}
+
+}
+
+namespace asr {
+
+void bn_launch_finalize_from_sums(const double *chan_sums, const float *conv_bias, int C, double n,
+                                  float eps, float momentum, float *mean, float *invstd,
+                                  float *running_mean, float *running_var, hipStream_t s) {
+    hipLaunchKernelGGL(bn_finalize_from_sums_kernel, dim3((C + 63) / 64), dim3(64), 0, s, chan_sums,
+                       conv_bias, C, n, eps, momentum, mean, invstd, running_mean, running_var);
+}
+
+void bn_launch_eval_stats(const float *running_mean, const float *running_var, int C, float eps,
+                          float *mean, float *invstd, hipStream_t s) {
+    hipLaunchKernelGGL(bn_eval_stats_kernel, dim3((C + 63) / 64), dim3(64), 0, s, running_mean,
+                       running_var, C, eps, mean, invstd);
+}
+
+void bn_launch_param_grads(const double *sums, int C, const float *gamma, const float *invstd,
+                           int training, float *dgamma, float *dbeta, float *dconv_bias,
+                           hipStream_t s) {
+    hipLaunchKernelGGL(bn_param_grads_kernel, dim3((C + 63) / 64), dim3(64), 0, s, sums, C, gamma,
+                       invstd, training, dgamma, dbeta, dconv_bias);
 }
 
 }
diff --git a/pytorch-asr_amd/csrc/common.h b/pytorch-asr_amd/csrc/common.h
--- a/pytorch-asr_amd/csrc/common.h
+++ b/pytorch-asr_amd/csrc/common.h
@@ -56,4 +56,13 @@
     __device__ __forceinline__ float value() const { return m + __logf(s); }
 };
 
+void bn_launch_finalize_from_sums(const double *chan_sums, const float *conv_bias, int C, double n,
+                                  float eps, float momentum, float *mean, float *invstd,
+                                  float *running_mean, float *running_var, hipStream_t s);
+void bn_launch_eval_stats(const float *running_mean, const float *running_var, int C, float eps,
+                          float *mean, float *invstd, hipStream_t s);
+void bn_launch_param_grads(const double *sums, int C, const float *gamma, const float *invstd,
+                           int training, float *dgamma, float *dbeta, float *dconv_bias,
+                           hipStream_t s);
+
 }
diff --git a/pytorch-asr_amd/csrc/conv.hip b/pytorch-asr_amd/csrc/conv.hip
--- a/pytorch-asr_amd/csrc/conv.hip
+++ b/pytorch-asr_amd/csrc/conv.hip
@@ -687,6 +687,11 @@
     __bf16 *y;
     float *partial;
     int B, T, F, To, Fo;
+    const float *gamma, *beta, *mean, *invstd, *shift;
+    const double *sums;
+    double n;
+    int training;
+    float lo, hi;
 };
 
 __device__ __forceinline__ void conv1_stage_windows(const Conv1Params &p, int b, int t0, int nrows,
@@ -710,7 +715,29 @@
     }
 }
 
-__global__ __launch_bounds__(256) void conv1_fwd_kernel(Conv1Params p) {
+__device__ __forceinline__ f32x16 conv1_tile_at(const char *wimg, const bf16x8 (&bf)[4], int m, int Fo,
+                                                unsigned fmagic, int lane) {
+    const unsigned r = ((unsigned)m * fmagic) >> 20, fo = (unsigned)m - r * (unsigned)Fo;
+    const char *base = wimg + (size_t)((r + (unsigned)(lane >> 5)) * (unsigned)Fo + fo) * 16;
+    bf16x8 a[4];
+#pragma unroll
+    for (int s = 0; s < 4; ++s) a[s] = *reinterpret_cast<const bf16x8 *>(base + (size_t)(2 * s * Fo) * 16);
+    f32x16 acc = {};
+#pragma unroll
+    for (int s = 0; s < 4; ++s) acc = __builtin_amdgcn_mfma_f32_32x32x16_bf16(bf[s], a[s], acc, 0, 0, 0);
+    return acc;
+}
+__device__ __forceinline__ f32x16 conv1_tile(const char *wimg, const bf16x8 (&bf)[4], int tile, int npix,
+                                             int Fo, unsigned fmagic, int lane) {
+    int m = 32 * tile + (lane & 31);
+    if (m >= npix) m = npix - 1;
+    return conv1_tile_at(wimg, bf, m, Fo, fmagic, lane);
+}
+
+enum { C1_STORE = 0, C1_STATS = 1, C1_BNACT = 2 };
+
+template <int EPI>
+__global__ __launch_bounds__(256, EPI == C1_BNACT ? 4 : 1) void conv1_fwd_kernel(Conv1Params p) {
     extern __shared__ char smem[];
     const int tid = threadIdx.x, lane = tid & 63;
     const int wave = __builtin_amdgcn_readfirstlane(tid >> 6);
@@ -721,41 +748,50 @@
     bf16x8 bf[4];
 #pragma unroll
     for (int s = 0; s < 4; ++s) bf[s] = reinterpret_cast<const bf16x8 *>(p.wpack)[s * 64 + lane];
+    float sc[16], sh[16];
+    if (EPI == C1_BNACT) {
+#pragma unroll
+        for (int i = 0; i < 16; ++i) {
+            const int c = 8 * (i >> 2) + 4 * (lane >> 5) + (i & 3);
+            sc[i] = p.gamma[c] * p.invstd[c];
+            sh[i] = p.beta[c] - (p.mean[c] - (p.shift ? p.shift[c] : 0.f)) * sc[i];
+        }
+    }
     conv1_stage_windows(p, b, t0, C1_ROWS + 8, wimg, tid, 256);
     __syncthreads();
     const unsigned fmagic = (1u << 20) / (unsigned)Fo + 1u;
     for (int tile = wave; tile < ntiles; tile += 4) {
-        int m = 32 * tile + (lane & 31);
-        if (m >= npix) m = npix - 1;
-        const unsigned r = ((unsigned)m * fmagic) >> 20, fo = (unsigned)m - r * (unsigned)Fo;
-        const char *base = wimg + (size_t)((r + (unsigned)(lane >> 5)) * (unsigned)Fo + fo) * 16;
-        bf16x8 a[4];
-#pragma unroll
-        for (int s = 0; s < 4; ++s) a[s] = *reinterpret_cast<const bf16x8 *>(base + (size_t)(2 * s * Fo) * 16);
-        f32x16 acc = {};
-#pragma unroll
-        for (int s = 0; s < 4; ++s) acc = __builtin_amdgcn_mfma_f32_32x32x16_bf16(bf[s], a[s], acc, 0, 0, 0);
+        const f32x16 acc = conv1_tile(wimg, bf, tile, npix, Fo, fmagic, lane);
 #pragma unroll
         for (int g = 0; g < 4; ++g) {
             bf16x4 o4 = {(__bf16)acc[4 * g], (__bf16)acc[4 * g + 1], (__bf16)acc[4 * g + 2], (__bf16)acc[4 * g + 3]};
+            if (EPI == C1_BNACT) {
+#pragma unroll
+                for (int j = 0; j < 4; ++j)
+                    o4[j] = (__bf16)fminf(fmaxf(fmaf((float)o4[j], sc[4 * g + j], sh[4 * g + j]), p.lo), p.hi);
+            }
             *reinterpret_cast<bf16x4 *>(reinterpret_cast<char *>(oimg) + (size_t)(32 * tile + (lane & 31)) * 64 +
                                         16 * g + 8 * (lane >> 5)) = o4;
         }
     }
     __syncthreads();
     const int rows_here = (p.To - t0) < C1_ROWS ? (p.To - t0) : C1_ROWS;
-    char *yb = reinterpret_cast<char *>(p.y) + ((size_t)b * p.To + t0) * Fo * 64;
-    for (int c = tid; c < rows_here * Fo * 4; c += 256)
-        *reinterpret_cast<u32x4 *>(yb + (size_t)c * 16) =
-            *reinterpret_cast<const u32x4 *>(reinterpret_cast<const char *>(oimg) + (size_t)c * 16);
-    if (p.partial)
+    if (EPI != C1_STATS) {
+        char *yb = reinterpret_cast<char *>(p.y) + ((size_t)b * p.To + t0) * Fo * 64;
+        for (int c = tid; c < rows_here * Fo * 4; c += 256)
+            *reinterpret_cast<u32x4 *>(yb + (size_t)c * 16) =
+                *reinterpret_cast<const u32x4 *>(reinterpret_cast<const char *>(oimg) + (size_t)c * 16);
+    }
+    if (EPI != C1_BNACT && p.partial)
         chan_partial_sums(oimg, rows_here * Fo, reinterpret_cast<float *>(oimg + (size_t)ntiles * 32 * CH),
                           p.partial + ((size_t)blockIdx.y * gridDim.x + blockIdx.x) * 64);
 }
 
 constexpr int C1_WGS = 1024;
-template <int DI, int WPT>
-__global__ __launch_bounds__(256) void conv1_wgrad_kernel(Conv1Params p) {
+enum { C1W_PLAIN = 0, C1W_BNAPPLY = 2 };
+
+template <int DI, int WPT, int MODE>
+__global__ __launch_bounds__(256, MODE != C1W_PLAIN && DI <= 5 ? 4 : 1) void conv1_wgrad_kernel(Conv1Params p) {
     extern __shared__ char smem[];
     const int tid = threadIdx.x, lane = tid & 63;
     const int wave = __builtin_amdgcn_readfirstlane(tid >> 6);
@@ -763,6 +799,20 @@
     const int nwin = (C1_ROWS + 8) * Fo;
     char *wimg = smem;
     char *dimg = smem + (size_t)nwin * 16;
+    float *coef = reinterpret_cast<float *>(dimg + (size_t)npix * PIX);
+    char *wpk = reinterpret_cast<char *>(coef + 6 * CH);
+    if (MODE != C1W_PLAIN) {
+        reinterpret_cast<u32x4 *>(wpk)[tid] = reinterpret_cast<const u32x4 *>(p.wpack)[tid];
+        if (tid < CH) {
+            const bool k = MODE == C1W_BNAPPLY && p.training;
+            coef[tid] = p.mean[tid] - (p.shift ? p.shift[tid] : 0.f);
+            coef[CH + tid] = p.invstd[tid];
+            coef[2 * CH + tid] = p.gamma[tid];
+            coef[3 * CH + tid] = p.beta[tid];
+            coef[4 * CH + tid] = k ? (float)(p.sums[2 * tid] / p.n) : 0.f;
+            coef[5 * CH + tid] = k ? (float)(p.sums[2 * tid + 1] / p.n) : 0.f;
+        }
+    }
     f32x16 acc[2];
 #pragma unroll
     for (int t = 0; t < 2; ++t)
@@ -778,6 +828,8 @@
     u32x4 dreg[DI];
     float2 wreg[WPT][4];
     auto fetch = [&](int c) {
+        int tid = threadIdx.x;
+        if (MODE != C1W_PLAIN) asm volatile("" : "+v"(tid));
         const int b = c / chunks_per_utt, t0 = (c - b * chunks_per_utt) * C1_ROWS;
         const char *yb = reinterpret_cast<const char *>(p.y) + ((size_t)b * p.To + t0) * Fo * 64;
         const int rows_here = (p.To - t0) < C1_ROWS ? (p.To - t0) : C1_ROWS;
@@ -818,6 +870,49 @@
         __syncthreads();
         stash();
         __syncthreads();
+        if (MODE != C1W_PLAIN) {
+            const int t0 = (c % chunks_per_utt) * C1_ROWS;
+            const int nlive = ((p.To - t0) < C1_ROWS ? (p.To - t0) : C1_ROWS) * Fo;
+            for (int tile = wave; tile < (npix + 31) >> 5; tile += 4) {
+                bf16x8 bf[4];
+#pragma unroll
+                for (int s = 0; s < 4; ++s) bf[s] = reinterpret_cast<const bf16x8 *>(wpk)[s * 64 + lane];
+                const f32x16 c1 = conv1_tile(wimg, bf, tile, npix, Fo, fmagic, lane);
+                const int m = 32 * tile + (lane & 31);
+                if (m >= nlive) continue;
+                char *dp = dimg + m * PIX + 8 * h;
+#pragma unroll
+                for (int g = 0; g < 8; ++g) {
+                    unsigned co = (unsigned)(8 * (g >> 1) + 4 * h + 2 * (g & 1));
+                    asm volatile("" : "+v"(co));
+                    const float *cf = coef + co;
+                    const float2 cm = *reinterpret_cast<const float2 *>(cf);
+                    const float2 cis = *reinterpret_cast<const float2 *>(cf + CH);
+                    const float2 cg = *reinterpret_cast<const float2 *>(cf + 2 * CH);
+                    const float2 cbe = *reinterpret_cast<const float2 *>(cf + 3 * CH);
+                    const float2 k1 = *reinterpret_cast<const float2 *>(cf + 4 * CH);
+                    const float2 k2 = *reinterpret_cast<const float2 *>(cf + 5 * CH);
+                    typedef __attribute__((ext_vector_type(2))) __bf16 bf16x2;
+                    bf16x2 *dq = reinterpret_cast<bf16x2 *>(dp + 16 * (g >> 1) + 4 * (g & 1));
+                    const bf16x2 d2 = *dq;
+                    bf16x2 o2;
+                    {
+                        const float xh = ((float)(__bf16)c1[2 * g] - cm.x) * cis.x;
+                        const float y = fmaf(xh, cg.x, cbe.x);
+                        const float d = (y > p.lo && y < p.hi) ? (float)d2[0] : 0.f;
+                        o2[0] = (__bf16)(cg.x * cis.x * (d - k1.x - xh * k2.x));
+                    }
+                    {
+                        const float xh = ((float)(__bf16)c1[2 * g + 1] - cm.y) * cis.y;
+                        const float y = fmaf(xh, cg.y, cbe.y);
+                        const float d = (y > p.lo && y < p.hi) ? (float)d2[1] : 0.f;
+                        o2[1] = (__bf16)(cg.y * cis.y * (d - k1.y - xh * k2.y));
+                    }
+                    *dq = o2;
+                }
+            }
+            __syncthreads();
+        }
         if (c + (int)gridDim.x < nchunks) fetch(c + gridDim.x);
         for (int ks = wave; ks < nks; ks += 4) {
             const bf16x8 a = tr_frag(dimg + (size_t)(16 * ks) * PIX + a_off);
@@ -859,6 +954,129 @@
     const int co = (j & 3) + 8 * (j >> 2) + 4 * (l >> 5), tap = 32 * nt + (l & 31);
     const int kt = tap >> 3, kf = tap & 7;
     if (kt < KS && kf < KS) dw[(co * KS + kt) * KS + kf] = s;
+}
+
+__global__ __launch_bounds__(1024) void chan_sums_ordered_kernel(const float *partial, int nparts, double *dpart) {
+    __shared__ double lds[1024];
+    const int el = threadIdx.x & 63, way = threadIdx.x >> 6;
+    double s = 0.0;
+    for (int g = blockIdx.x * 16 + way; g < nparts; g += gridDim.x * 16) s += (double)partial[(size_t)g * 64 + el];
+    lds[way * 64 + el] = s;
+    __syncthreads();
+    if (way == 0) {
+        double t = 0.0;
+        for (int w = 0; w < 16; ++w) t += lds[w * 64 + el];
+        dpart[blockIdx.x * 64 + el] = t;
+    }
+}
+__global__ void chan_sums_ordered_final_kernel(const double *dpart, int nblocks, double *out) {
+    const int el = threadIdx.x;
+    double t = 0.0;
+    for (int j = 0; j < nblocks; ++j) t += dpart[j * 64 + el];
+    out[2 * (el & 31) + (el >> 5)] = t;
+}
+
+constexpr int C1S_PIX = 128;
+constexpr int C1S_NB = 2;
+
+template <int NB>
+__global__ __launch_bounds__(256 * NB) void conv1_bn_sums_kernel(Conv1Params p, int P, int wimg_bytes, int nparent) {
+    extern __shared__ char smem[];
+    const int lane = threadIdx.x & 63;
+    const int wave = __builtin_amdgcn_readfirstlane((int)threadIdx.x >> 6);
+    const int half = __builtin_amdgcn_readfirstlane((int)threadIdx.x >> 8), tid = threadIdx.x & 255;
+    const int pblock = blockIdx.x * NB + half;
+    const int nact = nparent - (int)blockIdx.x * NB < NB ? nparent - (int)blockIdx.x * NB : NB;
+    const int Fo = p.Fo;
+    char *wimg = smem;
+    __bf16 *oimg = reinterpret_cast<__bf16 *>(smem + wimg_bytes);
+    const unsigned fmagic = (1u << 20) / (unsigned)Fo + 1u;
+    bf16x8 bf[4];
+#pragma unroll
+    for (int s = 0; s < 4; ++s) bf[s] = reinterpret_cast<const bf16x8 *>(p.wpack)[s * 64 + lane];
+    const int c0 = 8 * (tid & 3), pl = tid >> 2;
+    float m[8], is[8], g[8], be[8], s[8], q[8];
+#pragma unroll
+    for (int i = 0; i < 8; ++i) {
+        m[i] = p.mean[c0 + i] - (p.shift ? p.shift[c0 + i] : 0.f);
+        is[i] = p.invstd[c0 + i]; g[i] = p.gamma[c0 + i]; be[i] = p.beta[c0 + i];
+        s[i] = q[i] = 0.f;
+    }
+    auto one = [&](const bf16x8 &v, const bf16x8 &dv) {
+#pragma unroll
+        for (int i = 0; i < 8; ++i) {
+            const float xh = ((float)v[i] - m[i]) * is[i];
+            const float y = fmaf(xh, g[i], be[i]);
+            const float d = (y > p.lo && y < p.hi) ? (float)dv[i] : 0.f;
+            s[i] += d;
+            q[i] += d * xh;
+        }
+    };
+    const int nflat = p.B * p.To;
+    const int cstep = nparent * C1S_PIX;
+    for (int base = blockIdx.x * NB * C1S_PIX; base < P; base += cstep) {
+        const int gr0 = base / Fo, off = base - gr0 * Fo;
+        const int npx = P - base < nact * C1S_PIX ? P - base : nact * C1S_PIX;
+        const int nrows = (off + npx - 1) / Fo + 1 + 8;
+        __syncthreads();
+        for (int i = threadIdx.x; i < nrows * Fo; i += 256 * NB) {
+            const unsigned row = ((unsigned)i * fmagic) >> 20, fo = (unsigned)i - row * (unsigned)Fo;
+            const int u = gr0 - 6 + (int)row;
+            bf16x8 v = {};
+            if (u >= 0 && u < nflat) {
+                const int b = u / p.To, t = u - b * p.To;
+                if (t < p.T) {
+                    const float2 *src = reinterpret_cast<const float2 *>(p.x + ((size_t)b * p.T + t) * p.F + 2 * fo);
+#pragma unroll
+                    for (int j = 0; j < 4; ++j) {
+                        const float2 f2 = src[j];
+                        v[2 * j] = (__bf16)f2.x;
+                        v[2 * j + 1] = (__bf16)f2.y;
+                    }
+                }
+            }
+            *reinterpret_cast<bf16x8 *>(wimg + (size_t)i * 16) = v;
+        }
+        const int pix = base + half * C1S_PIX + pl;
+        const bool two = half < nact && pix + 64 < P, single = half < nact && pix < P && !two;
+        const __bf16 *dy = p.y + (size_t)pix * CH + c0;
+        bf16x8 d0 = {}, d1 = {};
+        if (two || single) d0 = *reinterpret_cast<const bf16x8 *>(dy);
+        if (two) d1 = *reinterpret_cast<const bf16x8 *>(dy + 64 * CH);
+        __syncthreads();
+        if (32 * wave < npx) {
+            int ml = 32 * wave + (lane & 31);
+            if (ml >= npx) ml = npx - 1;
+            const f32x16 acc = conv1_tile_at(wimg, bf, off + ml, Fo, fmagic, lane);
+#pragma unroll
+            for (int gq = 0; gq < 4; ++gq) {
+                const bf16x4 o4 = {(__bf16)acc[4 * gq], (__bf16)acc[4 * gq + 1], (__bf16)acc[4 * gq + 2], (__bf16)acc[4 * gq + 3]};
+                *reinterpret_cast<bf16x4 *>(reinterpret_cast<char *>(oimg) + (size_t)(32 * wave + (lane & 31)) * 64 +
+                                            16 * gq + 8 * (lane >> 5)) = o4;
+            }
+        }
+        __syncthreads();
+        const __bf16 *ov = oimg + (half * C1S_PIX + pl) * CH + c0;
+        if (two) {
+            const bf16x8 v0 = *reinterpret_cast<const bf16x8 *>(ov), v1 = *reinterpret_cast<const bf16x8 *>(ov + 64 * CH);
+            one(v0, d0);
+            one(v1, d1);
+        } else if (single) {
+            one(*reinterpret_cast<const bf16x8 *>(ov), d0);
+        }
+    }
+    __syncthreads();
+    float *rs8 = reinterpret_cast<float *>(smem) + half * 2 * 256 * 9, *rq8 = rs8 + 256 * 9;
+#pragma unroll
+    for (int i = 0; i < 8; ++i) { rs8[tid * 9 + i] = s[i]; rq8[tid * 9 + i] = q[i]; }
+    __syncthreads();
+    if (tid < CH && half < nact) {
+        const int cg = tid >> 3, i = tid & 7;
+        float a = 0.f, b = 0.f;
+        for (int t = cg; t < 256; t += 4) { a += rs8[t * 9 + i]; b += rq8[t * 9 + i]; }
+        p.partial[(size_t)pblock * 64 + tid] = a;
+        p.partial[(size_t)pblock * 64 + CH + tid] = b;
+    }
 }
 
 
@@ -1285,12 +1503,29 @@
     const int ntiles = (C1_ROWS * Fo + 31) / 32;
     const size_t lds = (size_t)(C1_ROWS + 8) * Fo * 16 + (size_t)ntiles * 32 * CH * 2 + 512 * 4;
     if (lds > 64 * 1024) return ASR_EUNSUPPORTED;
-    hipLaunchKernelGGL(conv1_fwd_kernel, grid, dim3(256), lds, s, p);
+    hipLaunchKernelGGL(conv1_fwd_kernel<C1_STORE>, grid, dim3(256), lds, s, p);
     if (chan_sums) {
         hipLaunchKernelGGL(zero_chan_sums_kernel, dim3(1), dim3(64), 0, s, chan_sums);
         hipLaunchKernelGGL(chan_sums_reduce_kernel, dim3(64), dim3(1024), 0, s, p.partial, (int)(grid.x * grid.y), chan_sums);
     }
     return hipGetLastError() == hipSuccess ? ASR_OK : ASR_ELAUNCH;
+}
+
+template <int MODE>
+static int conv1_wgrad_launch(const Conv1Params &p, int *nwg, hipStream_t s) {
+    const int Fo = p.Fo;
+    size_t lds = (size_t)(C1_ROWS + 8) * Fo * 16 + (size_t)C1_ROWS * Fo * PIX;
+    if (MODE != C1W_PLAIN) lds += 6 * CH * 4 + 4 * 64 * 16;
+    const size_t fin = 4 * 2 * 1024 * 4;
+    if (lds < fin) lds = fin;
+    if (lds > 64 * 1024) return ASR_EUNSUPPORTED;
+    const int chunks = p.B * ((p.To + C1_ROWS - 1) / C1_ROWS);
+    *nwg = chunks < C1_WGS ? chunks : C1_WGS;
+    const int di = (C1_ROWS * Fo * 4 + 255) / 256, wpt = ((C1_ROWS + 8) * Fo + 255) / 256;
+    void (*kern)(Conv1Params) = di <= 5 && wpt <= 2 ? conv1_wgrad_kernel<5, 2, MODE>
+                              : (di <= 8 && wpt <= 3 ? conv1_wgrad_kernel<8, 3, MODE> : conv1_wgrad_kernel<16, 6, MODE>);
+    hipLaunchKernelGGL(kern, dim3(*nwg), dim3(256), lds, s, p);
+    return ASR_OK;
 }
 
 extern "C" int asr_conv1_7x7s2_wgrad(const float *x, const void *dy, int B, int T, int F,
@@ -1306,16 +1541,104 @@
     p.x = x; p.wpack = nullptr; p.y = (__bf16 *)const_cast<void *>(dy);
     p.partial = (float *)((char *)workspace + 4 * 64 * 8 * 2);
     p.B = B; p.T = T; p.F = F; p.To = To; p.Fo = Fo;
-    size_t lds = (size_t)(C1_ROWS + 8) * Fo * 16 + (size_t)C1_ROWS * Fo * PIX;
-    if (lds < 4 * 2 * 1024 * 4) lds = 4 * 2 * 1024 * 4;
+    int nwg;
+    const int rc2 = conv1_wgrad_launch<C1W_PLAIN>(p, &nwg, s);
+    if (rc2 != ASR_OK) return rc2;
+    hipLaunchKernelGGL(conv1_wgrad_reduce_kernel, dim3(2 * 1024 / 64), dim3(1024), 0, s, p.partial, nwg, dw);
+    return hipGetLastError() == hipSuccess ? ASR_OK : ASR_ELAUNCH;
+}
+
+extern "C" int asr_conv1_bn_act_fwd(const float *x, const float *w, const float *conv_bias, int B, int T,
+                                    int F, const float *gamma, const float *beta, float *running_mean,
+                                    float *running_var, int training, float momentum, float eps,
+                                    float lo, float hi, void *out, float *save_mean, float *save_invstd,
+                                    double *chan_sums, void *workspace, int64_t workspace_bytes,
+                                    int phase, void *stream) {
+    int To, Fo;
+    const int rc = conv1_shapes(B, T, F, &To, &Fo);
+    if (rc != ASR_OK) return rc;
+    if (Fo > 36) return ASR_EUNSUPPORTED;
+    if (phase < 0 || phase > 2 || !x || !w || !gamma || !beta || !save_mean || !save_invstd || !workspace ||
+        workspace_bytes < asr_conv1_7x7s2_workspace_bytes())
+        return ASR_EINVAL;
+    if ((phase != 1 && !out) || (training && !chan_sums) || (!training && (!running_mean || !running_var)))
+        return ASR_EINVAL;
+    hipStream_t s = (hipStream_t)stream;
+    __bf16 *wpack = (__bf16 *)workspace;
+    hipLaunchKernelGGL(conv1_pack_kernel, dim3(8), dim3(256), 0, s, w, wpack);
+    Conv1Params p;
+    p.x = x; p.wpack = wpack; p.y = (__bf16 *)out;
+    p.B = B; p.T = T; p.F = F; p.To = To; p.Fo = Fo;
+    p.gamma = gamma; p.beta = beta; p.mean = save_mean; p.invstd = save_invstd; p.shift = conv_bias;
+    p.sums = nullptr; p.n = 0.0; p.training = training; p.lo = lo; p.hi = hi;
+    const dim3 grid((To + C1_ROWS - 1) / C1_ROWS, B);
+    p.partial = (float *)((char *)workspace + 4 * 64 * 8 * 2);
+    if ((int64_t)grid.x * grid.y * 64 * 4 > asr_conv1_7x7s2_workspace_bytes() - 4 * 64 * 8 * 2 - 256)
+        return ASR_EUNSUPPORTED;
+    const int ntiles = (C1_ROWS * Fo + 31) / 32;
+    const size_t lds = (size_t)(C1_ROWS + 8) * Fo * 16 + (size_t)ntiles * 32 * CH * 2 + 512 * 4;
     if (lds > 64 * 1024) return ASR_EUNSUPPORTED;
-    const int chunks = B * ((To + C1_ROWS - 1) / C1_ROWS);
-    const int nwg = chunks < C1_WGS ? chunks : C1_WGS;
-    const int di = (C1_ROWS * Fo * 4 + 255) / 256, wpt = ((C1_ROWS + 8) * Fo + 255) / 256;
-    void (*kern)(Conv1Params) = di <= 5 && wpt <= 2 ? conv1_wgrad_kernel<5, 2>
-                              : (di <= 8 && wpt <= 3 ? conv1_wgrad_kernel<8, 3> : conv1_wgrad_kernel<16, 6>);
-    hipLaunchKernelGGL(kern, dim3(nwg), dim3(256), lds, s, p);
-    hipLaunchKernelGGL(conv1_wgrad_reduce_kernel, dim3(2 * 1024 / 64), dim3(1024), 0, s, p.partial, nwg, dw);
+    if (training && phase != 2) {
+        hipLaunchKernelGGL(conv1_fwd_kernel<C1_STATS>, grid, dim3(256), lds, s, p);
+        hipLaunchKernelGGL(zero_chan_sums_kernel, dim3(1), dim3(64), 0, s, chan_sums);
+        hipLaunchKernelGGL(chan_sums_reduce_kernel, dim3(64), dim3(1024), 0, s, p.partial, (int)(grid.x * grid.y), chan_sums);
+    }
+    if (phase != 1) {
+        if (training)
+            asr::bn_launch_finalize_from_sums(chan_sums, conv_bias, CH, (double)B * To * Fo, eps, momentum,
+                                              save_mean, save_invstd, running_mean, running_var, s);
+        else
+            asr::bn_launch_eval_stats(running_mean, running_var, CH, eps, save_mean, save_invstd, s);
+        hipLaunchKernelGGL(conv1_fwd_kernel<C1_BNACT>, grid, dim3(256), lds, s, p);
+    }
+    return hipGetLastError() == hipSuccess ? ASR_OK : ASR_ELAUNCH;
+}
+
+extern "C" int asr_conv1_bn_act_bwd(const float *x, const float *w, const float *conv_bias, int B, int T,
+                                    int F, const float *gamma, const float *beta, const float *save_mean,
+                                    const float *save_invstd, int training, float lo, float hi,
+                                    const void *dy, float *dw, float *dgamma, float *dbeta,
+                                    float *dconv_bias, double *sums, void *workspace,
+                                    int64_t workspace_bytes, int phase, double n_total, void *stream) {
+    int To, Fo;
+    const int rc = conv1_shapes(B, T, F, &To, &Fo);
+    if (rc != ASR_OK) return rc;
+    if (Fo > 36) return ASR_EUNSUPPORTED;
+    if (phase < 0 || phase > 2 || (phase == 2 && !(n_total >= 1.0))) return ASR_EINVAL;
+    if (!x || !w || !gamma || !beta || !save_mean || !save_invstd || !dy || !sums || !workspace ||
+        workspace_bytes < asr_conv1_7x7s2_workspace_bytes())
+        return ASR_EINVAL;
+    if ((phase != 2 && (!dgamma || !dbeta)) || (phase != 1 && !dw)) return ASR_EINVAL;
+    hipStream_t s = (hipStream_t)stream;
+    __bf16 *wpack = (__bf16 *)workspace;
+    hipLaunchKernelGGL(conv1_pack_kernel, dim3(8), dim3(256), 0, s, w, wpack);
+    Conv1Params p;
+    p.x = x; p.wpack = wpack; p.y = (__bf16 *)const_cast<void *>(dy);
+    p.partial = (float *)((char *)workspace + 4 * 64 * 8 * 2);
+    p.B = B; p.T = T; p.F = F; p.To = To; p.Fo = Fo;
+    p.gamma = gamma; p.beta = beta; p.mean = save_mean; p.invstd = save_invstd; p.shift = conv_bias;
+    p.sums = sums; p.n = phase == 2 ? n_total : (double)B * To * Fo; p.training = training;
+    p.lo = lo; p.hi = hi;
+    int nwg;
+    if (phase != 2) {
+        const int64_t P64 = (int64_t)B * To * Fo;
+        if (P64 > 0x7fffffff - 4096 * C1S_PIX) return ASR_EUNSUPPORTED;
+        const int P = (int)P64;
+        nwg = P / 64 < 4096 ? (P / 64 > 0 ? P / 64 : 1) : 4096;
+        const int wimg_bytes = ((C1S_NB * C1S_PIX - 1 + Fo - 1) / Fo + 1 + 8) * Fo * 16;
+        size_t lds = (size_t)wimg_bytes + C1S_NB * C1S_PIX * CH * 2;
+        if (lds < C1S_NB * 2 * 256 * 9 * 4) lds = C1S_NB * 2 * 256 * 9 * 4;
+        double *dpart = (double *)((char *)p.partial + (size_t)4096 * 64 * 4);
+        hipLaunchKernelGGL(conv1_bn_sums_kernel<C1S_NB>, dim3((nwg + C1S_NB - 1) / C1S_NB), dim3(256 * C1S_NB), lds, s, p, P, wimg_bytes, nwg);
+        hipLaunchKernelGGL(chan_sums_ordered_kernel, dim3(64), dim3(1024), 0, s, p.partial, nwg, dpart);
+        hipLaunchKernelGGL(chan_sums_ordered_final_kernel, dim3(1), dim3(64), 0, s, dpart, 64, sums);
+        asr::bn_launch_param_grads(sums, CH, gamma, save_invstd, training, dgamma, dbeta, dconv_bias, s);
+    }
+    if (phase != 1) {
+        const int rc2 = conv1_wgrad_launch<C1W_BNAPPLY>(p, &nwg, s);
+        if (rc2 != ASR_OK) return rc2;
+        hipLaunchKernelGGL(conv1_wgrad_reduce_kernel, dim3(2 * 1024 / 64), dim3(1024), 0, s, p.partial, nwg, dw);
+    }
     return hipGetLastError() == hipSuccess ? ASR_OK : ASR_ELAUNCH;
 }
 
```
